# m4drat/wtf

Measured on AMD Instinct MI355X. Metric: execs/sec + emulated instr/s per node (tlv_server, HEVD) at 1/2/4/8 GPUs, higher is better.
Workload: dtype u64

## Files before the change

### wtf_amd/host/gpu_backend.cc

```cpp
#include "gpu_backend.h"
#include "module_instances.h"

#include <algorithm>
#include <chrono>
#include <cstdio>
#include <cstring>

#include "host_pool.h"

#include "blake3_lite.h"

namespace wtfgpu_host {

thread_local uint32_t GpuBackend_t::cur_ = 0;
thread_local uint64_t GpuBackend_t::servicing_bp_ = ~0ull;
thread_local uint64_t GpuBackend_t::servicing_sp_ = ~0ull;
thread_local bool GpuBackend_t::scouting_ = false;

namespace {
constexpr uint64_t kFeedRegion = 16384;
using Clock = std::chrono::steady_clock;
double ms_since(Clock::time_point t0) {
  return std::chrono::duration<double, std::milli>(Clock::now() - t0).count();
}

int gpr_index(Registers_t r) {
  switch (r) {
    case Registers_t::Rax: return WTFGPU_RAX;
    case Registers_t::Rbx: return WTFGPU_RBX;
    case Registers_t::Rcx: return WTFGPU_RCX;
    case Registers_t::Rdx: return WTFGPU_RDX;
    case Registers_t::Rsi: return WTFGPU_RSI;
    case Registers_t::Rdi: return WTFGPU_RDI;
    case Registers_t::Rsp: return WTFGPU_RSP;
    case Registers_t::Rbp: return WTFGPU_RBP;
    case Registers_t::R8: return WTFGPU_R8;
    case Registers_t::R9: return WTFGPU_R9;
    case Registers_t::R10: return WTFGPU_R10;
    case Registers_t::R11: return WTFGPU_R11;
    case Registers_t::R12: return WTFGPU_R12;
    case Registers_t::R13: return WTFGPU_R13;
    case Registers_t::R14: return WTFGPU_R14;
    case Registers_t::R15: return WTFGPU_R15;
    case Registers_t::Rip: return 16;
    case Registers_t::Rflags: return 17;
    default: return -1;
  }
}

}

GpuBackend_t::GpuBackend_t() = default;
GpuBackend_t::~GpuBackend_t() {
  for (Part &P : parts_)
    for (void *p : {(void *)P.pin, (void *)P.ex, (void *)P.nb, (void *)P.dc, (void *)P.sargs, (void *)P.cov_hdr})
      if (p) wtfgpu_host_free(ctx_, p);
  if (wpin_) wtfgpu_host_free(ctx_, wpin_);
  if (ctx_) wtfgpu_destroy(ctx_);
}

bool GpuBackend_t::LoadDump(const std::string &dump_path) { return dump_.Parse(dump_path); }

bool GpuBackend_t::Initialize(const Options_t &Opts, const CpuState_t &CpuState) {
  if (dump_.PageCount() == 0 && !Opts.DumpPath.empty() && !LoadDump(Opts.DumpPath.string())) {
    printf("Failed to parse the dump %s\n", Opts.DumpPath.string().c_str());
    return false;
  }
  if (wtfgpu_create(Opts.GpuDevice, &ctx_) != WTFGPU_OK) {
    printf("wtfgpu_create(%d) failed\n", Opts.GpuDevice);
    return false;
  }
  const auto pages = dump_.Pages();
  std::vector<uint64_t> gpfns(pages.size());
  std::vector<uint8_t> blob(pages.size() * Page::Size);
  for (size_t i = 0; i < pages.size(); i++) {
    gpfns[i] = pages[i].first;
    memcpy(blob.data() + i * Page::Size, pages[i].second, Page::Size);
  }
  if (wtfgpu_load_pool(ctx_, gpfns.data(), blob.data(), gpfns.size())) return false;
  nlanes_ = std::max<uint32_t>(Opts.GpuLanes, 1);
  overlay_pages_ = std::max<uint32_t>(Opts.GpuOverlayPages, 1);
  if (wtfgpu_alloc_lanes(ctx_, nlanes_, overlay_pages_, Opts.GpuCoverageSet)) return false;
  views_.clear();
  views_.resize(nlanes_);
  touched_.assign(nlanes_, 0);
  pf_.assign(nlanes_, PrepFeed{});
  arenas_.resize(HostPool::Get().Threads() + 1);
  if (Opts.Limit) SetLimit(Opts.Limit);
  if (Opts.Edges && wtfgpu_set_edges(ctx_, 1) != WTFGPU_OK) return false;
  if (!Restore(CpuState)) return false;
  return set_code_pages();
}

bool GpuBackend_t::Restore(const CpuState_t &CpuState) {
  initial_ = CpuState;
  initial_regs_ = RegsFromCpuState(CpuState);
  if (wtfgpu_set_initial_state(ctx_, &initial_regs_)) return false;
  if (wtfgpu_restore(ctx_, 0, nlanes_)) return false;
  for (uint32_t l = 0; l < nlanes_; l++) reset_view(l);
  cur_ = 0;
  return true;
}

void GpuBackend_t::reset_view(uint32_t lane) {
  LaneView &v = views_[lane];
  memcpy(v.gpr, initial_regs_.gpr, sizeof(initial_regs_.gpr));
  v.gpr[16] = initial_regs_.rip;
  v.gpr[17] = initial_regs_.rflags;
  v.regs_dirty = false;
  v.cr[0] = initial_regs_.cr2;
  v.cr[1] = initial_regs_.cr3;
  v.cr_known = 3;
  v.cr_dirty = 0;
  v.result.reset();
  v.handler_fault = false;
  v.seed = initial_.Seed;
  v.has_feed = false;
  v.feed.clear();
  v.dirty_known = true;
  v.dirty.clear();
  v.wlog.clear();
  v.wdata.clear();
  v.win_len = 0;
  drop_staged(v);
  touched_[lane] = 0;
}

void GpuBackend_t::Stop(const TestcaseResult_t &Res) { cur().result = Res; }

void GpuBackend_t::SetLimit(const uint64_t Limit) {
  limit_ = Limit;
  if (ctx_) wtfgpu_set_limit(ctx_, Limit);
}

uint64_t GpuBackend_t::GetReg(const Registers_t Reg) {
  const int i = gpr_index(Reg);
  if (i >= 0) return cur().gpr[i];
  if (Reg == Registers_t::Cr2 || Reg == Registers_t::Cr3) {
    const int k = Reg == Registers_t::Cr2 ? 0 : 1;
    LaneView &v = cur();
    if (!(v.cr_known & (1 << k))) {
      std::lock_guard<std::mutex> g(engine_mu_);
      if (wtfgpu_lane_get_cr(ctx_, cur_, k ? 3 : 2, &v.cr[k]) != WTFGPU_OK) std::abort();
      v.cr_known |= uint8_t(1 << k);
    }
    return v.cr[k];
  }
  return 0;
}

uint64_t GpuBackend_t::SetReg(const Registers_t Reg, const uint64_t Value) {
  const int i = gpr_index(Reg);
  if (i >= 0) {
    cur().gpr[i] = Value;
    cur().regs_dirty = true;
  } else if (Reg == Registers_t::Cr2 || Reg == Registers_t::Cr3) {
    const int k = Reg == Registers_t::Cr2 ? 0 : 1;
    cur().cr[k] = Value;
    cur().cr_known |= uint8_t(1 << k);
    cur().cr_dirty |= uint8_t(1 << k);
  }
  return Value;
}

uint64_t GpuBackend_t::Rdrand() { return wtf_rdrand(cur().seed); }

void GpuBackend_t::PrintRunStats() {
  PrintTestcaseRunStats(last_run_, aggregate_.size());
  printf("  Breakpoint services: %llu in %llu rounds\n", (unsigned long long)stats_.breakpoint_hits,
         (unsigned long long)stats_.rounds);
  printf("       Kernel time ms: %.2f\n", stats_.kernel_ms);
}

bool GpuBackend_t::SetBreakpoint(const Gva_t Gva, const BreakpointHandler_t Handler) {
  if (ModuleInstances *I = ModuleInstances::Registering()) {
    I->AddHandler(Gva.U64(), Handler);
    if (I->RegisteringIndex() > 0) return breakpoints_.count(Gva.U64()) != 0;
  }
  if (breakpoints_.count(Gva.U64())) {
    printf("/!\\ There is already a breakpoint at %#llx\n", (unsigned long long)Gva.U64());
    return false;
  }
  breakpoints_.emplace(Gva.U64(), Handler);
  std::vector<uint64_t> v;
  for (auto &kv : breakpoints_) v.push_back(kv.first);
  return wtfgpu_set_breakpoints(ctx_, v.data(), (uint32_t)v.size()) == WTFGPU_OK;
}

bool GpuBackend_t::SetBreakpoint(const Gva_t Gva, const BreakpointHandler_t Handler,
                                 const BreakpointAction_t &Action) {
  if (!SetBreakpoint(Gva, Handler)) return false;
  if (ModuleInstances::Registering() && ModuleInstances::Registering()->RegisteringIndex() > 0) return true;
  const char *Env = getenv("WTFGPU_DEVICE_BP_ACTIONS");
  if (Action.Kind == BreakpointAction_t::Kind_t::Host || (Env && Env[0] == '0')) return true;
  wtfgpu_bp_action_t A;
  memset(&A, 0, sizeof(A));
  A.gva = Gva.U64();
  if (Action.Kind == BreakpointAction_t::Kind_t::SimulateReturn) {
    A.kind = WTFGPU_BPACT_RETURN;
    A.value = Action.Return;
    if (Action.StringReg >= 0) {
      const int g = gpr_index((Registers_t)Action.StringReg);
      if (g < 0) return false;
      A.gprs[0] = (uint64_t)g + 1;
      A.gprs[1] = Action.StringMax;
    }
  } else if (Action.Kind == BreakpointAction_t::Kind_t::Feed) {
    A.kind = WTFGPU_BPACT_FEED;
    A.value = Action.Return;
    A.gprs[0] = (uint64_t)gpr_index((Registers_t)Action.Gprs[0]);
    A.gprs[1] = (uint64_t)gpr_index((Registers_t)Action.Gprs[1]);
    feed_action_ = true;
  } else if (Action.Kind == BreakpointAction_t::Kind_t::StopOk) {
    A.kind = WTFGPU_BPACT_STOP_OK;
  } else if (Action.Kind == BreakpointAction_t::Kind_t::Rdrand) {
    A.kind = WTFGPU_BPACT_RDRAND;
    A.gprs[0] = (uint64_t)gpr_index((Registers_t)Action.Gprs[0]);
  } else if (Action.Kind == BreakpointAction_t::Kind_t::StopWithArgs) {
    if (!Action.ArgsResult || Action.Return > 6) return false;
    A.kind = WTFGPU_BPACT_STOP_ARGS;
    A.value = Action.Return;
    args_results_[Gva.U64()] = Action.ArgsResult;
  } else {
    A.kind = WTFGPU_BPACT_SET_GPRS;
    memcpy(A.gprs, Action.Gprs, sizeof(A.gprs));
  }
  bp_actions_.push_back(A);
  return wtfgpu_set_breakpoint_actions(ctx_, bp_actions_.data(), (uint32_t)bp_actions_.size()) == WTFGPU_OK;
}

bool GpuBackend_t::SetFeed(const uint8_t *Data, const uint64_t Size) {
  if (!feed_action_ || Size > kFeedRegion) return false;
  LaneView &v = cur();
  v.has_feed = true;
  v.feed.assign(Data, Data + Size);
  return true;
}

bool GpuBackend_t::DeclareInsert(const InsertAction_t &Action) {
  if (ModuleInstances::Registering() && ModuleInstances::Registering()->RegisteringIndex() > 0) return insert_action_;
  const char *Env = getenv("WTFGPU_DEVICE_BP_ACTIONS");
  if (Env && Env[0] == '0') return false;
  const int h = gpr_index(Action.HeadReg), p = gpr_index(Action.PtrReg), l = gpr_index(Action.LenReg);
  if (h < 0 || p < 0 || l < 0 || Action.LenArg > 64) return false;
  const wtfgpu_insert_t I = {(uint32_t)h, (uint32_t)p, (uint32_t)l, Action.LenArg};
  if (wtfgpu_set_insert(ctx_, &I) != WTFGPU_OK) return false;
  insert_action_ = true;
  return true;
}

bool GpuBackend_t::SetInsert(const uint8_t *Data, const uint64_t Size) {
  if (!insert_action_ || Size + 4 > kFeedRegion) return false;
  LaneView &v = cur();
  v.has_feed = true;
  v.feed.resize(Size + 4);
  const uint32_t n = (uint32_t)Size;
  memcpy(v.feed.data(), &n, 4);
  if (Size) memcpy(v.feed.data() + 4, Data, Size);
  return true;
}

int GpuBackend_t::upload_feed(uint32_t n) {
  if (!(feed_action_ || insert_action_) || n == 0) return WTFGPU_OK;
  std::vector<uint64_t> off(n + 1);
  std::vector<uint8_t> has(n);
  uint64_t total = 0;
  for (uint32_t l = 0; l < n; l++) total += view(l).feed.size();
  std::vector<uint8_t> bytes;
  bytes.reserve(total);
  for (uint32_t l = 0; l < n; l++) {
    off[l] = bytes.size();
    has[l] = view(l).has_feed;
    bytes.insert(bytes.end(), view(l).feed.begin(), view(l).feed.end());
  }
  off[n] = bytes.size();
  return wtfgpu_set_feed(ctx_, 0, n, off.data(), has.data(), bytes.data(), bytes.size());
}

bool GpuBackend_t::DirtyGpa(const Gpa_t) { return true; }

namespace {
constexpr size_t kArenaBlock = 16u << 20;
const uint8_t kZeroPage[Page::Size] = {};
}

size_t GpuBackend_t::alloc_slots(size_t n, uint8_t **orig, uint8_t **data) const {
  const bool in_loop = HostPool::InLoop();
  std::shared_lock<std::shared_mutex> recycling(recycle_mu_);
  std::unique_lock<std::mutex> spare(spare_mu_, std::defer_lock);
  if (!in_loop) spare.lock();
  Arena &A = arenas_[in_loop ? HostPool::ThreadIndex() : arenas_.size() - 1];
  while (A.cur < A.blocks.size() && A.blocks[A.cur].cap - A.blocks[A.cur].used < n) A.cur++;
  if (A.cur == A.blocks.size()) {
    Block b;
    b.cap = std::max<size_t>(n, kArenaBlock / Page::Size);
    void *p = nullptr;
    int rc;
    {
      std::lock_guard<std::mutex> g(engine_mu_);
      rc = wtfgpu_host_alloc(ctx_, b.cap * Page::Size, &p);
    }
    if (rc != WTFGPU_OK) {
      printf("wtfgpu_host_alloc failed\n");
      std::abort();
    }
    b.orig = (uint8_t *)p;
    b.data.reset(new uint8_t[b.cap * Page::Size]);
    A.blocks.push_back(std::move(b));
  }
  Block &b = A.blocks[A.cur];
  *orig = b.orig + b.used * Page::Size;
  *data = b.data.get() + b.used * Page::Size;
  const size_t first = b.used;
  b.used += n;
  live_staged_ += n;
  return first;
}

void GpuBackend_t::release_slots(size_t n) const { live_staged_ -= n; }

bool GpuBackend_t::parallel_service(const ModuleSlots *slots) const {
  return slots && slots->ThreadSafe() && HostPool::Get().Threads() > 1;
}

uint8_t *GpuBackend_t::stage(uint32_t lane, uint64_t gpfn, const uint8_t *orig, uint8_t *data) const {
  LaneView &v = view(lane);
  v.pages.push_back(Staged{gpfn, data, orig});
  for (LaneView::Logged &w : v.wlog)
    if (w.len && (w.gpa >> 12) == gpfn) {
      memcpy(data + (w.gpa & 0xfff), v.wdata.data() + w.off, w.len);
      w.len = 0;
    }
  return data;
}

bool GpuBackend_t::PhysWriteDirect(const Gpa_t Gpa, const uint8_t *Buffer, const uint64_t Size) {
  const uint32_t lane = cur_;
  if (Staged *p = find_staged(lane, Gpa.U64() >> 12)) {
    memcpy(p->data + (Gpa.U64() & 0xfff), Buffer, Size);
    return true;
  }
  LaneView &v = view(lane);
  if (v.win_len && Gpa.U64() < v.win_gpa + v.win_len && Gpa.U64() + Size > v.win_gpa) {
    const uint64_t lo = std::max(Gpa.U64(), v.win_gpa), hi = std::min(Gpa.U64() + Size, v.win_gpa + v.win_len);
    memcpy(v.win + (lo - v.win_gpa), Buffer + (lo - Gpa.U64()), hi - lo);
  }
  if (!v.wlog.empty()) {
    LaneView::Logged &last = v.wlog.back();
    if (last.len && last.off + last.len == v.wdata.size() && last.gpa + last.len == Gpa.U64() &&
        ((last.gpa ^ Gpa.U64()) >> 12) == 0) {
      last.len += (uint32_t)Size;
      v.wdata.insert(v.wdata.end(), Buffer, Buffer + Size);
      return true;
    }
  }
  v.wlog.push_back(LaneView::Logged{Gpa.U64(), (uint32_t)Size, (uint32_t)v.wdata.size()});
  v.wdata.insert(v.wdata.end(), Buffer, Buffer + Size);
  return true;
}

bool GpuBackend_t::PhysReadDirect(const Gpa_t Gpa, uint8_t *Buffer, const uint64_t Size) const {
  const uint32_t lane = cur_;
  const uint64_t gpfn = Gpa.U64() >> 12;
  if (Staged *p = find_staged(lane, gpfn)) {
    memcpy(Buffer, p->data + (Gpa.U64() & 0xfff), Size);
    return true;
  }
  const LaneView &v = view(lane);
  if (v.win_len && Gpa.U64() >= v.win_gpa && Gpa.U64() + Size <= v.win_gpa + v.win_len) {
    memcpy(Buffer, v.win + (Gpa.U64() - v.win_gpa), Size);
    return true;
  }
  if (!v.dirty_known || in_overlay(v, gpfn)) return false;
  for (const LaneView::Logged &w : v.wlog)
    if (w.len && (w.gpa >> 12) == gpfn) return false;
  const uint8_t *p = dump_.GetPhysicalPage(gpfn << 12);
  memcpy(Buffer, (p ? p : kZeroPage) + (Gpa.U64() & 0xfff), Size);
  return true;
}

uint8_t *GpuBackend_t::stage_copy(uint32_t lane, uint64_t gpfn, const uint8_t *orig) const {
  uint8_t *o, *d;
  alloc_slots(1, &o, &d);
  memcpy(d, orig, Page::Size);
  return stage(lane, gpfn, orig, d);
}

void GpuBackend_t::drop_staged(LaneView &v) const {
  if (v.pages.empty()) return;
  live_staged_ -= v.pages.size();
  v.pages.clear();
  if (!HostPool::InLoop()) recycle_arenas();
}

void GpuBackend_t::recycle_arenas() const {
  if (live_staged_ != 0 || HostPool::InLoop()) return;
  std::unique_lock<std::shared_mutex> recycling(recycle_mu_);
  if (live_staged_ != 0) return;
  std::lock_guard<std::mutex> spare(spare_mu_);
  for (Arena &A : arenas_) {
    for (Block &b : A.blocks) b.used = 0;
    A.cur = 0;
  }
}

GpuBackend_t::Staged *GpuBackend_t::find_staged(uint32_t lane, uint64_t gpfn) const {
  for (Staged &p : view(lane).pages)
    if (p.gpfn == gpfn) return &p;
  return nullptr;
}

bool GpuBackend_t::in_overlay(const LaneView &v, uint64_t gpfn) const {
  return std::find(v.dirty.begin(), v.dirty.end(), (uint32_t)gpfn) != v.dirty.end();
}

uint8_t *GpuBackend_t::lane_page(uint32_t lane, uint64_t gpfn) const {
  if (Staged *p = find_staged(lane, gpfn)) return p->data;
  LaneView &v = view(lane);
  if (!v.dirty_known) {
    std::vector<uint32_t> buf(overlay_pages_ + 1);
    std::lock_guard<std::mutex> g(engine_mu_);
    wtfgpu_read_dirty_list(ctx_, &lane, 1, buf.data());
    v.dirty.assign(buf.begin() + 1, buf.begin() + 1 + std::min<uint32_t>(buf[0], overlay_pages_));
    v.dirty_known = true;
  }
  if (in_overlay(v, gpfn)) {
    const auto t0 = Clock::now();
    uint8_t *o, *d;
    alloc_slots(1, &o, &d);
    const uint64_t gpa = gpfn << 12;
    std::lock_guard<std::mutex> g(engine_mu_);
    wtfgpu_gather_pages(ctx_, &lane, &gpa, 1, o);
    memcpy(d, o, Page::Size);
    stats_.page_fetches++;
    stats_.fetch_ms += ms_since(t0);
    fetch_by_bp_[servicing_bp_]++;
    learn(gpfn);
    return stage(lane, gpfn, o, d);
  }
  if (scouting_) learn(gpfn);
  const uint8_t *p = dump_.GetPhysicalPage(gpfn << 12);
  return stage_copy(lane, gpfn, p ? p : kZeroPage);
}

void GpuBackend_t::learn(uint64_t gpfn) const {
  if (servicing_bp_ == ~0ull) return;
  if (gpfn == servicing_sp_) {
    bp_stack_.insert(servicing_bp_);
    return;
  }
  auto &l = bp_pages_[servicing_bp_];
  if (l.size() < 8 && std::find(l.begin(), l.end(), gpfn) == l.end()) l.push_back(gpfn);
}

const uint8_t *GpuBackend_t::lane_page_ro(uint32_t lane, uint64_t gpfn) const {
  if (Staged *p = find_staged(lane, gpfn)) return p->data;
  const LaneView &v = view(lane);
  if (!v.dirty_known || in_overlay(v, gpfn)) return lane_page(lane, gpfn);
  const uint8_t *p = dump_.GetPhysicalPage(gpfn << 12);
  return p ? p : kZeroPage;
}

namespace {
struct WalkMemo {
  uint64_t vpn = ~0ull, base = 0, mask = 0;
  uint64_t tables[4] = {};
  uint32_t ntables = 0;
};
thread_local WalkMemo t_walk_memo[64];
}

bool GpuBackend_t::VirtTranslate(const Gva_t Gva, Gpa_t &Gpa, const MemoryValidate_t) const {
  const uint64_t va = Gva.U64(), vpn = va >> 12;
  const LaneView &v = view(cur_);
  WalkMemo &m = t_walk_memo[vpn & 63];
  if (m.vpn == vpn && v.dirty_known && (!(v.cr_known & 2) || v.cr[1] == initial_.Cr3)) {
    bool clean = true;
    for (uint32_t k = 0; k < m.ntables && clean; k++)
      clean = !in_overlay(v, m.tables[k]) && !find_staged(cur_, m.tables[k]);
    if (clean) {
      Gpa = Gpa_t(m.base | (va & m.mask));
      return true;
    }
  }
  uint64_t table = initial_.Cr3 & 0x000ffffffffff000ull;
  WalkMemo w;
  bool from_dump = v.dirty_known;
  if ((v.cr_known & 2) && v.cr[1] != initial_.Cr3) {
    table = v.cr[1] & 0x000ffffffffff000ull;
    from_dump = false;
  }
  for (int level = 3; level >= 0; level--) {
    const uint64_t tf = table >> 12;
    w.tables[w.ntables++] = tf;
    from_dump = from_dump && !in_overlay(v, tf) && !find_staged(cur_, tf);
    const uint8_t *pg = lane_page_ro(cur_, tf);
    uint64_t e;
    memcpy(&e, pg + ((va >> (12 + 9 * level)) & 0x1ff) * 8, 8);
    if (!(e & 1)) return false;
    const uint64_t frame = e & 0x000ffffffffff000ull;
    if ((level == 2 || level == 1) && (e & 0x80)) {
      w.mask = level == 2 ? 0x3fffffffull : 0x1fffffull;
      w.base = frame & ~w.mask;
      break;
    }
    if (level == 0) {
      w.mask = 0xfff;
      w.base = frame;
    }
    table = frame;
  }
  Gpa = Gpa_t(w.base | (va & w.mask));
  if (from_dump) {
    w.vpn = vpn;
    m = w;
  }
  return true;
}

uint8_t *GpuBackend_t::PhysTranslate(const Gpa_t Gpa) const {
  return lane_page(cur_, Gpa.U64() >> 12) + (Gpa.U64() & 0xfff);
}

bool GpuBackend_t::PageFaultsMemoryIfNeeded(const Gva_t Gva, const uint64_t Size) {
  for (uint64_t a = Gva.U64() & ~0xfffull; a < Gva.U64() + Size; a += Page::Size) {
    Gpa_t G;
    if (!VirtTranslate(Gva_t(a), G, MemoryValidate_t::ValidateRead)) {
      cur().inject = a;
      return true;
    }
  }
  return false;
}

const std::unordered_set<Gva_t> &GpuBackend_t::LastNewCoverage() const { return last_new_coverage_; }

bool GpuBackend_t::RevokeLastNewCoverage() {
  for (const Gva_t &g : last_new_coverage_) aggregate_.erase(g.U64());
  last_new_coverage_.clear();
  return true;
}

int GpuBackend_t::flush_lanes(const std::vector<uint32_t> &lanes) {
  const auto tp = Clock::now();
  const size_t nl = lanes.size();
  const bool par = nl >= 1024;
  std::vector<uint64_t> rcnt(nl + 1, 0), pcnt(nl + 1, 0), roff(nl + 1, 0), boff(nl + 1, 0);
  std::atomic<bool> any_cr{false};
  HostPool::Get().For(nl, 256, [&](size_t i) {
    const LaneView &v = view(lanes[i]);
    rcnt[i + 1] = v.regs_dirty ? 1 : 0;
    pcnt[i + 1] = v.pages.size();
    uint64_t r = 0, b = 0;
    for (const LaneView::Logged &w : v.wlog)
      if (w.len) {
        r++;
        b += w.len;
      }
    roff[i + 1] = r;
    boff[i + 1] = b;
    if (v.cr_dirty) any_cr.store(true, std::memory_order_relaxed);
  }, par);
  for (size_t i = 0; i < nl; i++) {
    rcnt[i + 1] += rcnt[i];
    pcnt[i + 1] += pcnt[i];
    roff[i + 1] += roff[i];
    boff[i + 1] += boff[i];
  }
  if (any_cr)
    for (uint32_t l : lanes) {
      LaneView &v = view(l);
      for (int k = 0; k < 2; k++)
        if (v.cr_dirty & (1 << k)) {
          std::lock_guard<std::mutex> g(engine_mu_);
          if (wtfgpu_lane_set_cr(ctx_, l, k ? 3 : 2, v.cr[k]) != WTFGPU_OK) return WTFGPU_ERR_INVALID;
        }
      v.cr_dirty = 0;
    }
  std::vector<uint32_t> rl(rcnt[nl]);
  std::vector<uint64_t> regs(rcnt[nl] * 18);
  struct Cand {
    uint32_t lane;
    const Staged *p;
    uint32_t lo, hi;
  };
  std::vector<Cand> cand(pcnt[nl]);
  HostPool::Get().For(nl, 256, [&](size_t i) {
    const uint32_t l = lanes[i];
    LaneView &v = view(l);
    if (v.regs_dirty) {
      rl[rcnt[i]] = l;
      memcpy(&regs[rcnt[i] * 18], v.gpr, 18 * 8);
      v.regs_dirty = false;
    }
    uint64_t k = pcnt[i];
    for (const Staged &p : v.pages) cand[k++] = Cand{l, &p, 0, 0};
  }, par);
  HostPool::Get().For(cand.size(), 64, [&](size_t i) {
    const uint8_t *d = cand[i].p->data, *o = cand[i].p->orig;
    if (!memcmp(d, o, Page::Size)) return;
    size_t lo = 0, hi = Page::Size;
    while (lo + 8 <= hi && !memcmp(d + lo, o + lo, 8)) lo += 8;
    while (lo < hi && d[lo] == o[lo]) lo++;
    while (hi >= lo + 8 && !memcmp(d + hi - 8, o + hi - 8, 8)) hi -= 8;
    while (hi > lo && d[hi - 1] == o[hi - 1]) hi--;
    cand[i].lo = (uint32_t)lo;
    cand[i].hi = (uint32_t)hi;
  });
  uint64_t cbytes = 0, crecs = 0;
  for (const Cand &c : cand)
    if (c.lo != c.hi) {
      crecs++;
      cbytes += c.hi - c.lo;
    }
  std::vector<wtfgpu_write_t> writes(roff[nl] + crecs);
  const uint64_t total = boff[nl] + cbytes;
  if (total > wpin_cap_) {
    if (wpin_) wtfgpu_host_free(ctx_, wpin_);
    wpin_ = nullptr;
    wpin_cap_ = std::max<uint64_t>(total * 2, 1 << 20);
    void *p = nullptr;
    if (wtfgpu_host_alloc(ctx_, wpin_cap_, &p)) return WTFGPU_ERR_OOM;
    wpin_ = (uint8_t *)p;
  }
  HostPool::Get().For(nl, 256, [&](size_t i) {
    const uint32_t l = lanes[i];
    LaneView &v = view(l);
    uint64_t r = roff[i], b = boff[i];
    for (const LaneView::Logged &w : v.wlog) {
      if (!w.len) continue;
      writes[r++] = wtfgpu_write_t{l, w.len, w.gpa, b};
      memcpy(wpin_ + b, v.wdata.data() + w.off, w.len);
      b += w.len;
      v.dirty_known = false;
    }
    v.wlog.clear();
    v.wdata.clear();
  }, par);
  {
    uint64_t r = roff[nl], b = boff[nl];
    for (const Cand &c : cand) {
      if (c.lo == c.hi) continue;
      wtfgpu_write_t w{};
      w.lane = c.lane;
      w.len = c.hi - c.lo;
      w.gva = (c.p->gpfn << 12) | c.lo;
      w.data_off = b;
      memcpy(wpin_ + b, c.p->data + c.lo, w.len);
      b += w.len;
      writes[r++] = w;
      view(c.lane).dirty_known = false;
    }
  }
  stats_.staged_pages += cand.size();
  if (!cand.empty())
    for (uint32_t l : lanes) drop_staged(view(l));
  int rc = WTFGPU_OK;
  const auto tr = Clock::now();
  stats_.up_prep_ms += std::chrono::duration<double, std::milli>(tr - tp).count();
  if (!rl.empty()) rc = wtfgpu_write_gprs_list(ctx_, rl.data(), (uint32_t)rl.size(), regs.data());
  const auto ta = Clock::now();
  stats_.up_regs_ms += std::chrono::duration<double, std::milli>(ta - tr).count();
  if (!rc && !writes.empty())
    rc = wtfgpu_apply_phys_writes(ctx_, writes.data(), (uint32_t)writes.size(), wpin_, total, nullptr);
  stats_.up_apply_ms += ms_since(ta);
  return rc;
}

bool GpuBackend_t::classify(const std::vector<uint32_t> &pending, uint32_t first, const wtfgpu_exit_t *ex,
                            std::vector<uint8_t> &done, std::vector<LaneResult> *out, std::vector<uint32_t> &hits,
                            const uint64_t *stop_args) {
  std::vector<uint8_t> hit(pending.size(), 0);
  HostPool::Get().For(pending.size(), 1024, [&](size_t pi) {
    const uint32_t l = pending[pi];
    if (done[l - first]) return;
    const wtfgpu_exit_t &e = ex[l - first];
    LaneView &v = views_[l];
    const auto mark = [&]() -> LaneView & {
      touched_[l] = 1;
      return v;
    };
    switch (e.status) {
      case WTFGPU_EXIT_BREAKPOINT: hit[pi] = 1; return;
      case WTFGPU_RUNNING: return;
      case WTFGPU_EXIT_TIMEOUT: mark().result = Timedout_t(); break;
      case WTFGPU_EXIT_INT3:
      case WTFGPU_EXIT_HLT: mark().result = Crash_t(); break;
      case WTFGPU_EXIT_CR3: mark().result = Cr3Change_t(); break;
      case WTFGPU_EXIT_FAULT: mark().result = FaultToResult(e.vector, e.error, e.rip, e.addr, e.opcode); break;
      case WTFGPU_EXIT_STOPPED: break;
      case WTFGPU_EXIT_STOP_OK:
        if (touched_[l]) v.result = Ok_t();
        break;
      case WTFGPU_EXIT_STOP_ARGS: hit[pi] = 2; return;
      case WTFGPU_EXIT_FEED_FAULT: mark().handler_fault = true; break;
      default:
        if (out) (*out)[l].error = true;
        if (!v.result) mark().result = Crash_t();
        if (e.status == WTFGPU_EXIT_UNIMPLEMENTED) {
          stats_.err_unimpl++;
          stats_.unimpl_ops.add(e.opcode);
          stats_.last_unimpl_op = e.opcode;
          stats_.last_unimpl_rip = e.rip;
        } else if (e.status == WTFGPU_EXIT_OVERLAY_FULL) {
          stats_.err_overlay++;
        } else {
          stats_.err_other++;
        }
        break;
    }
    done[l - first] = 1;
  }, pending.size() >= 2048);
  std::vector<uint32_t> named;
  for (size_t pi = 0; pi < pending.size(); pi++) {
    if (hit[pi] == 1) hits.push_back(pending[pi]);
    if (hit[pi] == 2) named.push_back(pending[pi]);
  }
  if (named.empty()) return true;
  std::vector<uint64_t> args(named.size() * 6);
  bool ok = true;
  if (stop_args) {
    HostPool::Get().For(named.size(), 2048, [&](size_t k) {
      memcpy(&args[k * 6], stop_args + (uint64_t)(named[k] - first) * 6, 48);
    }, named.size() >= 8192);
  } else {
    ok = wtfgpu_read_stop_args(ctx_, named.data(), (uint32_t)named.size(), args.data()) == WTFGPU_OK;
  }
  std::atomic<uint64_t> bad{0};
  HostPool::Get().For(named.size(), 512, [&](size_t k) {
    const uint32_t l = named[k];
    LaneView &v = view(l);
    const auto it = args_results_.find(ex[l - first].rip);
    if (ok && it != args_results_.end()) {
      v.result = it->second(&args[k * 6]);
    } else {
      if (out) (*out)[l].error = true;
      if (!v.result) v.result = Crash_t();
      bad++;
    }
    done[l - first] = 1;
  }, named.size() >= 2048);
  stats_.err_other += bad;
  return true;
}

bool GpuBackend_t::fill_results(const std::vector<uint32_t> &lanes, uint32_t first,
                                const wtfgpu_exit_t *ex, const std::vector<uint8_t> &done,
                                std::vector<LaneResult> *out, std::vector<uint32_t> *finished) {
  const auto tg = Clock::now();
  std::vector<uint32_t> fin;
  for (uint32_t l : lanes)
    if (done[l - first]) fin.push_back(l);
  if (finished) finished->insert(finished->end(), fin.begin(), fin.end());
  if (!out) return true;
  std::vector<uint64_t> regs;
  uint32_t lo = 0, hi = 0;
  std::vector<uint64_t> nb;
  std::vector<uint32_t> dc, ec;
  if (want_gprs_) {
    regs.resize(fin.size() * 18);
    if (!fin.empty() && wtfgpu_read_gprs_list(ctx_, fin.data(), (uint32_t)fin.size(), regs.data())) return false;
    if (!fin.empty()) {
      lo = *std::min_element(fin.begin(), fin.end());
      hi = *std::max_element(fin.begin(), fin.end()) + 1;
      nb.resize(hi - lo);
      dc.resize(hi - lo);
      ec.resize(2 * (hi - lo));
      if (wtfgpu_read_bytes(ctx_, lo, hi - lo, nb.data()) || wtfgpu_read_dirty_counts(ctx_, lo, hi - lo, dc.data()) ||
          wtfgpu_read_edge_counts(ctx_, lo, hi - lo, ec.data()))
        return false;
    }
  }
  HostPool::Get().For(fin.size(), 1024, [&](size_t i) {
    LaneResult &r = (*out)[fin[i]];
    const LaneView &v = views_[fin[i]];
    const bool t = touched_[fin[i]] != 0;
    r.result = t && v.result ? std::move(*v.result) : TestcaseResult_t(Ok_t());
    if (t && v.handler_fault) {
      r.result = Crash_t();
      r.error = true;
      r.handler_fault = true;
      stats_.err_handler++;
    }
    if (want_gprs_) {
      memcpy(r.gprs, &regs[i * 18], 18 * 8);
      r.rip = r.gprs[16];
      const uint32_t k = fin[i] - lo;
      r.bytes = nb[k];
      r.dirty = std::min(dc[k], overlay_pages_);
      r.edges = ec[2 * k];
      r.edges_new = ec[2 * k + 1];
    } else {
      r.rip = ex[fin[i] - first].rip;
    }
    r.icount = ex[fin[i] - first].icount;
    r.exit_status = ex[fin[i] - first].status;
  }, fin.size() >= 2048);
  stats_.regs_ms += ms_since(tg);
  return true;
}

bool GpuBackend_t::stop_prestopped(const std::vector<uint32_t> &lanes) {
  std::vector<uint8_t> has(lanes.size());
  HostPool::Get().For(lanes.size(), 1024, [&](size_t i) { has[i] = touched_[lanes[i]] && views_[lanes[i]].result.has_value(); },
                      lanes.size() >= 4096);
  std::vector<uint32_t> pre;
  for (size_t i = 0; i < lanes.size(); i++)
    if (has[i]) pre.push_back(lanes[i]);
  return pre.empty() || wtfgpu_stop(ctx_, pre.data(), (uint32_t)pre.size(), WTFGPU_EXIT_STOPPED) == WTFGPU_OK;
}

bool GpuBackend_t::run_lanes(const std::vector<uint32_t> &lanes, std::vector<LaneResult> *out, ModuleSlots *slots,
                             bool per_lane_state) {
  if (lanes.empty()) return true;
  const uint32_t first = lanes.front() & ~63u, count = lanes.back() + 1 - first;
  std::vector<wtfgpu_exit_t> ex(count);
  std::vector<uint8_t> done(count, 0);
  std::vector<uint32_t> pending = lanes;
  if (!stop_prestopped(lanes)) return false;
  for (;;) {
    wtfgpu_run_stats_t rs{};
    const auto tk = Clock::now();
    if (wtfgpu_run(ctx_, first, count, ~0ull, &rs)) return false;
    const auto te = Clock::now();
    stats_.run_ms += std::chrono::duration<double, std::milli>(te - tk).count();
    account_run(rs);
    if (wtfgpu_read_exits(ctx_, first, count, ex.data())) return false;
    std::vector<uint32_t> hits;
    if (!classify(pending, first, ex.data(), done, out, hits)) return false;
    stats_.exits_ms += ms_since(te);
    if (hits.empty()) break;
    if (!service_hits(hits, first, done, slots, per_lane_state)) return false;
    pending.clear();
    for (uint32_t l : hits)
      if (!done[l - first]) pending.push_back(l);
  }
  return fill_results(lanes, first, ex.data(), done, out, nullptr);
}

void GpuBackend_t::account_run(const wtfgpu_run_stats_t &rs) {
  stats_.kernel_launches += rs.kernel_launches;
  stats_.kernel_ms += rs.kernel_ms;
  stats_.retired += rs.lane_retired;
  stats_.group_steps += rs.group_steps;
  stats_.rounds++;
}

bool GpuBackend_t::service_hits(const std::vector<uint32_t> &hits, uint32_t first, std::vector<uint8_t> &done,
                                ModuleSlots *slots, bool per_lane_state) {
  const auto t0 = Clock::now();
  {
    std::vector<uint64_t> regs(hits.size() * 18);
    if (wtfgpu_read_gprs_list(ctx_, hits.data(), (uint32_t)hits.size(), regs.data())) return false;
    std::vector<uint64_t> seeds(hits.size());
    if (wtfgpu_lane_seeds(ctx_, hits.data(), (uint32_t)hits.size(), seeds.data(), 0)) return false;
    const uint32_t stride = overlay_pages_ + 1;
    std::vector<uint32_t> dl(hits.size() * stride);
    if (wtfgpu_read_dirty_list(ctx_, hits.data(), (uint32_t)hits.size(), dl.data())) return false;
    const auto t1 = Clock::now();
    stats_.bulk_ms += std::chrono::duration<double, std::milli>(t1 - t0).count();
    std::vector<uint64_t> sp_gpfn(hits.size(), ~0ull), sp_gpa(hits.size(), ~0ull);
    HostPool::Get().For(hits.size(), 256, [&](size_t i) {
      LaneView &v = view(hits[i]);
      memcpy(v.gpr, &regs[i * 18], 18 * 8);
      v.seed = seeds[i];
      v.regs_dirty = false;
      v.cr_known = 0;
      v.win_len = 0;
      drop_staged(v);
      const uint32_t cnt = std::min(dl[i * stride], overlay_pages_);
      v.dirty.assign(dl.begin() + i * stride + 1, dl.begin() + i * stride + 1 + cnt);
      v.dirty_known = true;
      const uint64_t rip = v.gpr[16];
      if (!bp_seen_.count(rip) || bp_stack_.count(rip)) {
        cur_ = hits[i];
        Gpa_t sp;
        if (VirtTranslate(Gva_t(v.gpr[WTFGPU_RSP]), sp, MemoryValidate_t::ValidateRead)) {
          sp_gpa[i] = sp.U64();
          sp_gpfn[i] = sp.U64() >> 12;
        }
      }
    });
    recycle_arenas();
    std::vector<uint8_t> action(hits.size());
    auto service = [&](size_t h) {
      const uint32_t l = hits[h];
      LaneView &v = view(l);
      cur_ = l;
      const uint64_t rip0 = v.gpr[16];
      servicing_sp_ = sp_gpfn[h];
      BreakpointHandler_t handler = nullptr;
      if (slots && slots->Instances()) {
        handler = slots->Instances()->HandlerOf(l, rip0);
      } else {
        const auto it = breakpoints_.find(rip0);
        if (it != breakpoints_.end()) handler = it->second;
      }
      if (per_lane_state && slots) slots->SwapIn(l);
      servicing_bp_ = rip0;
      v.inject = ~0ull;
      try {
        if (handler) handler(this);
      } catch (const HandlerFault_t &) {
        v.handler_fault = true;
        v.result = Crash_t();
      }
      servicing_bp_ = ~0ull;
      if (per_lane_state && slots) slots->SwapOut(l);
      action[h] = v.result ? 0 : (v.gpr[16] == rip0 ? 2 : 1);
    };
    Backend_t *saved = g_Backend;
    g_Backend = this;
    std::vector<uint8_t> scouted(hits.size(), 0);
    for (size_t i = 0; i < hits.size(); i++) {
      if (!bp_seen_.insert(view(hits[i]).gpr[16]).second) continue;
      scouting_ = true;
      service(i);
      scouting_ = false;
      scouted[i] = 1;
    }
    std::vector<uint32_t> pf_lanes, win_lanes;
    std::vector<uint64_t> pf_gpas, win_gpas;
    std::vector<uint8_t> use_win(hits.size(), 0);
    HostPool::Get().For(hits.size(), 256, [&](size_t i) {
      if (scouted[i] || sp_gpfn[i] == ~0ull) return;
      const LaneView &v = view(hits[i]);
      if (bp_stack_.count(v.gpr[16]) && in_overlay(v, sp_gpfn[i]))
        use_win[i] = (sp_gpa[i] & 0xfff) + LaneView::kWin <= Page::Size ? 1 : 2;
    });
    for (size_t i = 0; i < hits.size(); i++) {
      if (scouted[i]) continue;
      const LaneView &v = view(hits[i]);
      auto want = [&](uint64_t gpfn) {
        if (!in_overlay(v, gpfn)) return;
        for (size_t k = pf_gpas.size(); k-- > 0 && pf_lanes[k] == hits[i];)
          if (pf_gpas[k] == gpfn << 12) return;
        pf_lanes.push_back(hits[i]);
        pf_gpas.push_back(gpfn << 12);
      };
      if (use_win[i] == 1) {
        win_lanes.push_back(hits[i]);
        win_gpas.push_back(sp_gpa[i]);
      } else if (use_win[i] == 2) {
        want(sp_gpfn[i]);
      }
      if (!bp_pages_.empty()) {
        auto lp = bp_pages_.find(v.gpr[16]);
        if (lp != bp_pages_.end())
          for (uint64_t g : lp->second) want(g);
      }
    }
    if (!win_lanes.empty()) {
      const size_t nw = win_lanes.size();
      std::vector<uint8_t> buf(nw * LaneView::kWin);
      if (wtfgpu_gather_bytes(ctx_, win_lanes.data(), win_gpas.data(), (uint32_t)nw, LaneView::kWin, buf.data()))
        return false;
      HostPool::Get().For(nw, 256, [&](size_t i) {
        LaneView &v = view(win_lanes[i]);
        v.win_gpa = win_gpas[i];
        v.win_len = LaneView::kWin;
        memcpy(v.win, buf.data() + i * LaneView::kWin, LaneView::kWin);
      });
      stats_.stack_windows += nw;
    }
    if (!pf_lanes.empty()) {
      const size_t np = pf_lanes.size();
      uint8_t *o, *d;
      alloc_slots(np, &o, &d);
      if (wtfgpu_gather_pages(ctx_, pf_lanes.data(), pf_gpas.data(), (uint32_t)np, o)) {
        release_slots(np);
        return false;
      }
      HostPool::Get().For(np, 256, [&](size_t i) { memcpy(d + i * Page::Size, o + i * Page::Size, Page::Size); });
      for (size_t i = 0; i < np; i++)
        stage(pf_lanes[i], pf_gpas[i] >> 12, o + i * Page::Size, d + i * Page::Size);
      stats_.prefetched_pages += np;
    }
    const auto t2 = Clock::now();
    stats_.prefetch_ms += std::chrono::duration<double, std::milli>(t2 - t1).count();
    if (per_lane_state && parallel_service(slots)) {
      HostPool::Get().For(hits.size(), 64, [&](size_t h) {
        g_Backend = this;
        if (!scouted[h]) service(h);
      });
    } else {
      for (size_t h = 0; h < hits.size(); h++)
        if (!scouted[h]) service(h);
    }
    g_Backend = saved;
    stats_.breakpoint_hits += hits.size();
    const auto t3 = Clock::now();
    stats_.handler_ms += std::chrono::duration<double, std::milli>(t3 - t2).count();
    if (flush_lanes(hits)) return false;
    for (size_t i = 0; i < hits.size(); i++) seeds[i] = view(hits[i]).seed;
    if (wtfgpu_lane_seeds(ctx_, hits.data(), (uint32_t)hits.size(), seeds.data(), 1)) return false;
    {
      std::vector<uint32_t> il;
      std::vector<uint64_t> ia;
      std::vector<size_t> ih;
      for (size_t h = 0; h < hits.size(); h++)
        if (action[h] != 0 && view(hits[h]).inject != ~0ull) {
          il.push_back(hits[h]);
          ia.push_back(view(hits[h]).inject);
          ih.push_back(h);
        }
      if (!il.empty()) {
        std::vector<int32_t> ok(il.size());
        if (wtfgpu_inject_fault(ctx_, il.data(), (uint32_t)il.size(), WTFGPU_VEC_PF, ErrorWrite | ErrorUser, ia.data(),
                                ok.data()))
          return false;
        for (size_t k = 0; k < il.size(); k++) {
          if (ok[k]) {
            action[ih[k]] = 1;
          } else {
            view(il[k]).result = Crash_t();
            action[ih[k]] = 0;
          }
        }
      }
    }
    std::vector<uint32_t> resume, stop;
    std::vector<uint8_t> skip;
    for (size_t h = 0; h < hits.size(); h++) {
      if (action[h] == 0) {
        stop.push_back(hits[h]);
        done[hits[h] - first] = 1;
      } else {
        resume.push_back(hits[h]);
        skip.push_back(action[h] == 2);
      }
    }
    if (!stop.empty() && wtfgpu_stop(ctx_, stop.data(), (uint32_t)stop.size(), WTFGPU_EXIT_STOPPED)) return false;
    if (!resume.empty() && wtfgpu_resume(ctx_, resume.data(), (uint32_t)resume.size(), skip.data())) return false;
    stats_.flush_ms += ms_since(t3);
    stats_.service_ms += ms_since(t0);
  }
  return true;
}

void GpuBackend_t::finish_coverage(uint32_t n, std::vector<LaneResult> *out, std::vector<uint32_t> *timedout) {
  uint64_t total = 0;
  uint32_t ovf = 0, dl = 0;
  uint64_t dr = 0;
  wtfgpu_read_coverage(ctx_, 0, n, &dl, &dr, 0, &total, &ovf);
  std::vector<uint32_t> lanes(total);
  std::vector<uint64_t> rips(total);
  if (total) wtfgpu_read_coverage(ctx_, 0, n, lanes.data(), rips.data(), total, &total, &ovf);
  std::vector<std::vector<uint64_t>> per(n);
  for (uint64_t i = 0; i < total; i++) per[lanes[i]].push_back(rips[i]);
  std::vector<uint64_t> fresh;
  last_new_coverage_.clear();
  for (uint32_t l = 0; l < n; l++) {
    std::sort(per[l].begin(), per[l].end());
    per[l].erase(std::unique(per[l].begin(), per[l].end()), per[l].end());
    if (full_coverage_) {
      if (out) (*out)[l].new_coverage = per[l];
      if (n == 1)
        for (uint64_t rip : per[l]) last_new_coverage_.insert(Gva_t(rip));
      continue;
    }
    const bool revoke = timedout && std::find(timedout->begin(), timedout->end(), l) != timedout->end();
    for (uint64_t rip : per[l]) {
      if (aggregate_.count(rip)) continue;
      if (out) (*out)[l].new_coverage.push_back(rip);
      if (revoke) continue;
      aggregate_.insert(rip);
      fresh.push_back(rip);
      if (n == 1) last_new_coverage_.insert(Gva_t(rip));
    }
  }
  if (full_coverage_) {
    wtfgpu_reset_coverage(ctx_);
    return;
  }
  commit_fresh(fresh);
}

std::optional<TestcaseResult_t> GpuBackend_t::Run(const uint8_t *, const uint64_t) {
  const auto t0 = Clock::now();
  cur_ = 0;
  if (flush_lanes({0}) || upload_feed(1)) return std::nullopt;
  std::vector<LaneResult> out(1);
  if (!run_lanes({0}, &out, nullptr, false)) return std::nullopt;
  LaneView &v = view(0);
  if (wtfgpu_read_gprs_list(ctx_, &cur_, 1, v.gpr)) return std::nullopt;
  v.regs_dirty = false;
  v.cr_known = 0;
  last_icount_ = out[0].icount;
  last_error_ = out[0].error;
  {
    uint64_t nbytes = 0;
    uint32_t dcount = 0, ecount[2] = {0, 0};
    wtfgpu_read_bytes(ctx_, 0, 1, &nbytes);
    wtfgpu_read_dirty_counts(ctx_, 0, 1, &dcount);
    wtfgpu_read_edge_counts(ctx_, 0, 1, ecount);
    last_run_ = out[0];
    last_run_.bytes = nbytes;
    last_run_.dirty = std::min(dcount, overlay_pages_);
    last_run_.edges = ecount[0];
    last_run_.edges_new = ecount[1];
  }
  finish_coverage(1, nullptr, nullptr);
  stats_.total_ms += ms_since(t0);
  cur_ = 0;
  return out[0].result;
}

bool GpuBackend_t::LaneTrace(uint32_t Lane, std::vector<uint64_t> &Rips, bool &Truncated) {
  uint64_t N = 0;
  Rips.clear();
  if (wtfgpu_read_trace(ctx_, Lane, nullptr, 0, &N) != WTFGPU_OK) return false;
  Truncated = N > trace_cap_;
  Rips.resize(std::min<uint64_t>(N, trace_cap_));
  return wtfgpu_read_trace(ctx_, Lane, Rips.data(), Rips.size(), &N) == WTFGPU_OK;
}

bool GpuBackend_t::LaneTenet(uint32_t Lane, std::vector<uint8_t> &Bytes, bool &Truncated) {
  uint64_t N = 0;
  Bytes.clear();
  if (wtfgpu_read_tenet(ctx_, Lane, nullptr, 0, &N) != WTFGPU_OK) return false;
  Truncated = N > tenet_cap_;
  Bytes.resize(std::min<uint64_t>(N, tenet_cap_));
  return wtfgpu_read_tenet(ctx_, Lane, Bytes.data(), Bytes.size(), &N) == WTFGPU_OK;
}

bool GpuBackend_t::RunBatch(const Target_t &Target, const std::vector<std::pair<const uint8_t *, size_t>> &Testcases,
                            std::vector<LaneResult> &Out, ModuleSlots *Slots) {
  const auto t0 = Clock::now();
  const uint32_t n = (uint32_t)Testcases.size();
  if (n == 0 || n > nlanes_) return false;
  Out.assign(n, LaneResult{});
  if (wtfgpu_restore(ctx_, 0, n)) return false;
  for (uint32_t l = 0; l < n; l++) reset_view(l);
  const auto tm = Clock::now();
  stats_.restore_ms += std::chrono::duration<double, std::milli>(tm - t0).count();
  std::vector<uint32_t> lanes(n);
  for (uint32_t l = 0; l < n; l++) lanes[l] = l;
  std::vector<uint8_t> insert_ok;
  insert_lanes(Target, lanes, Testcases, Slots, insert_ok);
  for (uint32_t l = 0; l < n; l++)
    if (!insert_ok[l]) view(l).result = Crash_t("insert-testcase-failed");
  const auto tu = Clock::now();
  stats_.module_ms += std::chrono::duration<double, std::milli>(tu - tm).count();
  if (flush_lanes(lanes) || upload_feed(n)) return false;
  stats_.upload_ms += ms_since(tu);
  stats_.insert_ms += ms_since(t0);
  if (!run_lanes(lanes, &Out, Slots, Slots != nullptr)) return false;
  {
    std::vector<uint64_t> nb(n);
    std::vector<uint32_t> dc(n);
    if (wtfgpu_read_bytes(ctx_, 0, n, nb.data()) == WTFGPU_OK &&
        wtfgpu_read_dirty_counts(ctx_, 0, n, dc.data()) == WTFGPU_OK)
      for (uint32_t l = 0; l < n; l++) stats_.alg_bytes += nb[l] + 2ull * 4096 * dc[l] + Testcases[l].second;
  }
  const auto tc = Clock::now();
  std::vector<uint32_t> timedout;
  for (uint32_t l = 0; l < n; l++)
    if (std::holds_alternative<Timedout_t>(Out[l].result)) timedout.push_back(l);
  finish_coverage(n, &Out, &timedout);
  const auto tr = Clock::now();
  stats_.coverage_ms += std::chrono::duration<double, std::milli>(tr - tc).count();
  target_restore(Target, lanes, Slots);
  stats_.target_restore_ms += ms_since(tr);
  stats_.total_ms += ms_since(t0);
  stats_.batches++;
  stats_.testcases += n;
  return true;
}

void GpuBackend_t::insert_lanes(const Target_t &Target, const std::vector<uint32_t> &lanes,
                                const std::vector<std::pair<const uint8_t *, size_t>> &tcs, ModuleSlots *Slots,
                                std::vector<uint8_t> &ok) {
  Backend_t *saved = g_Backend;
  ok.assign(lanes.size(), 1);
  auto insert = [&](size_t i) {
    const uint32_t l = lanes[i];
    cur_ = l;
    if (Slots) {
      Slots->ResetLane(l);
      Slots->SwapIn(l);
    }
    const Target_t &T = Slots && Slots->Instances() ? Slots->Instances()->TargetOf(l) : Target;
    try {
      ok[i] = T.InsertTestcase(tcs[i].first, tcs[i].second);
    } catch (const HandlerFault_t &) {
      view(l).handler_fault = true;
      ok[i] = 0;
    }
    if (Slots) Slots->SwapOut(l);
  };
  if (parallel_service(Slots)) {
    HostPool::Get().For(lanes.size(), 256, [&](size_t i) {
      g_Backend = this;
      insert(i);
    });
  } else {
    g_Backend = this;
    for (size_t i = 0; i < lanes.size(); i++) insert(i);
  }
  g_Backend = saved;
}

void GpuBackend_t::target_restore(const Target_t &Target, const std::vector<uint32_t> &lanes, ModuleSlots *Slots) {
  Backend_t *saved = g_Backend;
  auto restore = [&](uint32_t l) {
    cur_ = l;
    if (Slots) Slots->SwapIn(l);
    (Slots && Slots->Instances() ? Slots->Instances()->TargetOf(l) : Target).Restore();
    if (Slots) Slots->SwapOut(l);
  };
  if (parallel_service(Slots)) {
    HostPool::Get().For(lanes.size(), 256, [&](size_t i) {
      g_Backend = this;
      restore(lanes[i]);
    });
  } else {
    g_Backend = this;
    for (uint32_t l : lanes) restore(l);
  }
  g_Backend = saved;
  cur_ = 0;
}

void GpuBackend_t::collect_coverage(const std::vector<uint32_t> &lanes, std::vector<LaneResult> &res,
                                    const uint64_t *pf_hdr) {
  const auto t0 = Clock::now();
  uint64_t total = 0;
  uint32_t ovf = 0;
  constexpr uint64_t kPrefetchCap = 1ull << 22;
  bool pf = pf_hdr && pf_hdr[0] <= kPrefetchCap;
  if (pf) {
    total = pf_hdr[0];
    ovf = (uint32_t)pf_hdr[1] & 1;
    if (cov_lanes_.size() < total) {
      cov_lanes_.resize(total);
      cov_rips_.resize(total);
    }
    pf = wtfgpu_prefetched_coverage(ctx_, cov_lanes_.data(), cov_rips_.data(), total) == WTFGPU_OK &&
         wtfgpu_clear_coverage_lanes(ctx_, lanes.data(), (uint32_t)lanes.size()) == WTFGPU_OK;
    if (pf && total) {
      if (cov_want_.size() < nlanes_) cov_want_.assign(nlanes_, 0);
      for (uint32_t l : lanes) cov_want_[l] = 1;
      uint64_t k = 0;
      for (uint64_t i = 0; i < total; i++)
        if (cov_want_[cov_lanes_[i]]) {
          cov_lanes_[k] = cov_lanes_[i];
          cov_rips_[k++] = cov_rips_[i];
        }
      for (uint32_t l : lanes) cov_want_[l] = 0;
      total = k;
    }
  }
  if (!pf) {
    total = 0;
    ovf = 0;
    if (cov_lanes_.size() < (1u << 16)) {
      cov_lanes_.resize(1u << 16);
      cov_rips_.resize(1u << 16);
    }
    wtfgpu_collect_coverage_lanes(ctx_, lanes.data(), (uint32_t)lanes.size(), cov_lanes_.data(), cov_rips_.data(),
                                  cov_lanes_.size(), &total, &ovf);
    if (total > cov_lanes_.size()) {
      cov_lanes_.resize(total);
      cov_rips_.resize(total);
      wtfgpu_collect_coverage_lanes(ctx_, lanes.data(), (uint32_t)lanes.size(), cov_lanes_.data(), cov_rips_.data(),
                                    cov_lanes_.size(), &total, &ovf);
    }
  }
  const std::vector<uint32_t> &cl = cov_lanes_;
  const std::vector<uint64_t> &cr = cov_rips_;
  const auto t1 = Clock::now();
  stats_.covlog_ms += std::chrono::duration<double, std::milli>(t1 - t0).count();
  stats_.cov_entries += total;
  if (ovf && !cov_ovf_warned_) {
    cov_ovf_warned_ = true;
    fprintf(stderr, "wtfgpu: a lane's new-coverage set filled up (rips lost); raise the set size\n");
  }
  std::vector<std::pair<uint32_t, uint64_t>> &ent = cov_sorted_;
  ent.resize(total);
  for (uint64_t i = 0; i < total; i++) ent[i] = {cl[i], cr[i]};
  std::sort(ent.begin(), ent.end());
  ent.erase(std::unique(ent.begin(), ent.end()), ent.end());
  if (getenv("WTFGPU_COVLOG_TOP")) {
    for (uint64_t i = 0; i < total; i++) covlog_count_[cr[i]]++;
    if (++covlog_calls_ % 64 == 0) {
      std::vector<std::pair<uint64_t, uint64_t>> v(covlog_count_.begin(), covlog_count_.end());
      std::sort(v.begin(), v.end(), [](auto &a, auto &b) { return a.second > b.second; });
      fprintf(stderr, "covlog top:");
      for (size_t i = 0; i < v.size() && i < 24; i++)
        fprintf(stderr, " %llx:%llu%s", (unsigned long long)v[i].first, (unsigned long long)v[i].second,
                aggregate_.count(v[i].first) ? "*" : "");
      fprintf(stderr, " (%zu values)\n", v.size());
    }
  }
  std::vector<uint64_t> fresh;
  last_new_coverage_.clear();
  auto attribute = [&](uint32_t l, size_t at) {
    const bool revoke = std::holds_alternative<Timedout_t>(res[l].result);
    for (; at < ent.size() && ent[at].first == l; at++) {
      const uint64_t rip = ent[at].second;
      if (full_coverage_) {
        res[l].new_coverage.push_back(rip);
        continue;
      }
      if (aggregate_.count(rip)) continue;
      res[l].new_coverage.push_back(rip);
      if (revoke) continue;
      aggregate_.insert(rip);
      fresh.push_back(rip);
    }
    return at;
  };
  if (std::is_sorted(lanes.begin(), lanes.end())) {
    for (size_t at = 0; at < ent.size();) at = attribute(ent[at].first, at);
  } else {
    for (uint32_t l : lanes) {
      const auto it = std::lower_bound(ent.begin(), ent.end(), std::pair<uint32_t, uint64_t>{l, 0});
      if (it != ent.end() && it->first == l) attribute(l, (size_t)(it - ent.begin()));
    }
  }
  commit_fresh(fresh);
  stats_.attrib_ms += ms_since(t1);
}

uint32_t GpuBackend_t::FreeLanes() const {
  if (busy_.empty()) return parts_n() > 1 ? nlanes_ / 2 : nlanes_;
  const Part &P = parts_[next_part_];
  if (P.launched) return P.hi - P.lo;
  return (uint32_t)P.free.size();
}

uint32_t GpuBackend_t::parts_n() const {
  if (!parts_.empty()) return (uint32_t)parts_.size();
  const char *e = getenv("WTFGPU_STREAM_PARTS");
  const uint32_t want = e ? (uint32_t)atoi(e) : 2;
  return (want >= 2 && nlanes_ >= 256 && nlanes_ % 128 == 0) ? 2 : 1;
}

bool GpuBackend_t::StreamStep(const Target_t &Target, const std::vector<StreamTestcase_t> &In, uint64_t Slice,
                              std::vector<StreamResult_t> &Out, ModuleSlots *Slots, size_t *Taken) {
  const auto t0 = Clock::now();
  if (Taken) *Taken = 0;
  if (busy_.empty()) {
    busy_.assign(nlanes_, 0);
    tag_.assign(nlanes_, 0);
    tc_bytes_.assign(nlanes_, 0);
    lres_.assign(nlanes_, LaneResult{});
    lres_stale_.assign(nlanes_, 0);
    const uint32_t n = parts_n();
    parts_.assign(n, Part{});
    for (uint32_t p = 0; p < n; p++) {
      Part &Q = parts_[p];
      Q.lo = (uint32_t)((uint64_t)nlanes_ * p / n);
      Q.hi = (uint32_t)((uint64_t)nlanes_ * (p + 1) / n);
      Q.free.resize(Q.hi - Q.lo);
      for (uint32_t l = Q.lo; l < Q.hi; l++) Q.free[l - Q.lo] = l;
    }
    std::vector<uint32_t> all(nlanes_);
    for (uint32_t l = 0; l < nlanes_; l++) all[l] = l;
    if (wtfgpu_stop(ctx_, all.data(), nlanes_, WTFGPU_EXIT_IDLE)) return false;
  }
  const bool pipelined = parts_.size() > 1;
  const uint32_t pi = next_part_;
  next_part_ = (next_part_ + 1) % (uint32_t)parts_.size();
  Part &P = parts_[pi];
  if (pipelined && wtfgpu_select_queue(ctx_, pi)) return false;
  if (pipelined && P.launched && !harvest_part(P, Target, Out, Slots)) return false;
  const auto ti = Clock::now();
  stats_.harvest_ms += std::chrono::duration<double, std::milli>(ti - t0).count();
  std::vector<uint32_t> fresh;
  std::vector<std::pair<const uint8_t *, size_t>> tcs;
  fresh.reserve(std::min<size_t>(In.size(), P.hi - P.lo));
  tcs.reserve(fresh.capacity());
  {
    const size_t take = std::min(In.size(), P.free.size());
    fresh.assign(P.free.begin(), P.free.begin() + (std::ptrdiff_t)take);
    P.free.erase(P.free.begin(), P.free.begin() + (std::ptrdiff_t)take);
    tcs.resize(take);
    for (size_t i = 0; i < take; i++) tcs[i] = {In[i].data, In[i].size};
  }
  if (Taken) *Taken = fresh.size();
  stats_.fresh_ms += ms_since(ti);
  if (!fresh.empty()) {
    if (wtfgpu_restore_lanes(ctx_, fresh.data(), (uint32_t)fresh.size())) return false;
    stats_.restore_dev_ms += ms_since(ti);
    std::vector<uint8_t> prepared(fresh.size(), 0);
    HostPool::Get().For(fresh.size(), 256, [&](size_t i) {
      const uint32_t l = fresh[i];
      if (touched_[l]) reset_view(l);
      pf_[l] = PrepFeed{};
      busy_[l] = 1;
      tag_[l] = In[i].tag;
      tc_bytes_[l] = In[i].size;
      lres_stale_[l] = 1;
      const StreamTestcase_t &T = In[i];
      switch (T.prep) {
        case PreparedInsert_t::Call: return;
        case PreparedInsert_t::Failed: view(l).result = Crash_t("insert-testcase-failed"); break;
        case PreparedInsert_t::Nothing: break;
        case PreparedInsert_t::Feed:
          if (!feed_action_ || T.prep_size > kFeedRegion) return;
          pf_[l] = PrepFeed{T.prep_data, (uint32_t)T.prep_size, 1, 0};
          break;
        case PreparedInsert_t::Insert:
          if (!insert_action_ || T.size + 4 > kFeedRegion) return;
          pf_[l] = PrepFeed{T.data, (uint32_t)T.size, 1, 1};
          break;
      }
      if (Slots) Slots->ResetLane(l);
      prepared[i] = 1;
    });
    recycle_arenas();
    const auto tm = Clock::now();
    stats_.restore_ms += std::chrono::duration<double, std::milli>(tm - ti).count();
    std::vector<uint32_t> call;
    std::vector<std::pair<const uint8_t *, size_t>> call_tcs;
    for (size_t i = 0; i < fresh.size(); i++)
      if (!prepared[i]) {
        call.push_back(fresh[i]);
        call_tcs.push_back(tcs[i]);
      }
    stats_.prepared += fresh.size() - call.size();
    if (!call.empty()) {
      std::vector<uint8_t> ok;
      insert_lanes(Target, call, call_tcs, Slots, ok);
      for (size_t i = 0; i < call.size(); i++)
        if (!ok[i]) view(call[i]).result = Crash_t("insert-testcase-failed");
    }
    const auto tu = Clock::now();
    stats_.module_ms += std::chrono::duration<double, std::milli>(tu - tm).count();
    if (flush_lanes(call)) return false;
    if (feed_action_ || insert_action_) {
      const auto tf = Clock::now();
      const size_t n = fresh.size();
      std::vector<uint64_t> off(n + 1, 0);
      std::vector<uint8_t> has(n);
      HostPool::Get().For(n, 1024, [&](size_t i) {
        const uint32_t l = fresh[i];
        const PrepFeed &f = pf_[l];
        const bool t = !f.has && touched_[l];
        off[i + 1] = f.has ? f.len + (f.ins ? 4 : 0) : t ? views_[l].feed.size() : 0;
        has[i] = f.has || (t && views_[l].has_feed);
      });
      for (size_t i = 0; i < n; i++) off[i + 1] += off[i];
      if (off[n] > P.pin_cap) {
        if (P.pin) wtfgpu_host_free(ctx_, P.pin);
        P.pin = nullptr;
        P.pin_cap = std::max<uint64_t>(off[n] * 2, 1 << 20);
        void *p = nullptr;
        if (wtfgpu_host_alloc(ctx_, P.pin_cap, &p)) return false;
        P.pin = (uint8_t *)p;
      }
      HostPool::Get().For(n, 256, [&](size_t i) {
        const uint32_t l = fresh[i];
        const PrepFeed &f = pf_[l];
        uint8_t *o = P.pin + off[i];
        if (f.has) {
          if (f.ins) {
            memcpy(o, &f.len, 4);
            o += 4;
          }
          if (f.len) memcpy(o, f.p, f.len);
        } else if (touched_[l] && !views_[l].feed.empty()) {
          memcpy(o, views_[l].feed.data(), views_[l].feed.size());
        }
      });
      if (wtfgpu_set_feed_lanes(ctx_, fresh.data(), (uint32_t)n, off.data(), has.data(), P.pin, off[n]))
        return false;
      stats_.up_feed_ms += ms_since(tf);
    }
    if (!stop_prestopped(fresh)) return false;
    stats_.upload_ms += ms_since(tu);
    stats_.testcases += fresh.size();
  }
  stats_.insert_ms += ms_since(ti);
  const auto to = Clock::now();
  if (!fresh.empty()) {
    std::vector<uint32_t> occ(P.occ.size() + fresh.size());
    std::merge(P.occ.begin(), P.occ.end(), fresh.begin(), fresh.end(), occ.begin());
    P.occ.swap(occ);
  }
  stats_.occ_ms += ms_since(to);
  if (!P.occ.empty()) {
    const auto tk = Clock::now();
    if (wtfgpu_run_async(ctx_, P.lo, P.hi - P.lo, Slice ? Slice : 4096)) return false;
    P.pf = pipelined && prefetch_part(P);
    stats_.run_ms += ms_since(tk);
    P.launched = true;
    if (!pipelined && !harvest_part(P, Target, Out, Slots)) return false;
  }
  stats_.total_ms += ms_since(t0);
  return true;
}

bool GpuBackend_t::prefetch_part(Part &P) {
  const uint32_t count = P.hi - P.lo;
  auto grow = [&](auto *&p, uint64_t bytes) {
    if (p) return true;
    void *q = nullptr;
    if (wtfgpu_host_alloc(ctx_, bytes, &q)) return false;
    p = (std::remove_reference_t<decltype(p)>)q;
    return true;
  };
  if (P.ex_cap < count) {
    if (P.ex) wtfgpu_host_free(ctx_, P.ex);
    P.ex = nullptr;
    P.ex_cap = 0;
    if (!grow(P.ex, (uint64_t)count * sizeof(wtfgpu_exit_t))) return false;
    P.ex_cap = count;
  }
  const bool args = !args_results_.empty();
  if (!grow(P.nb, (uint64_t)count * 8) || !grow(P.dc, (uint64_t)count * 4) || !grow(P.cov_hdr, 16) ||
      (args && !grow(P.sargs, (uint64_t)count * 48)))
    return false;
  if (wtfgpu_prefetch_results(ctx_, P.lo, count, P.ex, P.nb, P.dc, args ? P.sargs : nullptr) != WTFGPU_OK)
    return false;
  P.pf_cov = !full_coverage_ && wtfgpu_prefetch_coverage(ctx_, P.lo, count, P.cov_hdr) == WTFGPU_OK;
  return true;
}

bool GpuBackend_t::harvest_part(Part &P, const Target_t &Target, std::vector<StreamResult_t> &Out,
                                ModuleSlots *Slots) {
  const auto tw = Clock::now();
  wtfgpu_run_stats_t rs{};
  if (wtfgpu_run_wait(ctx_, &rs)) return false;
  const auto te = Clock::now();
  stats_.run_ms += std::chrono::duration<double, std::milli>(te - tw).count();
  account_run(rs);
  P.launched = false;
  const uint32_t first = P.lo, count = P.hi - P.lo;
  HostPool::Get().For(P.occ.size(), 1024, [&](size_t i) {
    const uint32_t l = P.occ[i];
    if (!lres_stale_[l]) return;
    lres_stale_[l] = 0;
    LaneResult &r = lres_[l];
    r.result = Ok_t();
    r.error = false;
    r.handler_fault = false;
    r.exit_status = 0;
    r.icount = 0;
    r.rip = 0;
    r.new_coverage.clear();
  }, P.occ.size() >= 8192);
  const bool pf = P.pf;
  P.pf = false;
  if (!pf) {
    if (P.ex_cap < count) {
      if (P.ex) wtfgpu_host_free(ctx_, P.ex);
      P.ex = nullptr;
      P.ex_cap = 0;
      void *p = nullptr;
      if (wtfgpu_host_alloc(ctx_, (uint64_t)count * sizeof(wtfgpu_exit_t), &p)) return false;
      P.ex = (wtfgpu_exit_t *)p;
      P.ex_cap = count;
    }
    if (wtfgpu_read_exits(ctx_, first, count, P.ex)) return false;
  }
  std::vector<uint8_t> done(count, 0);
  std::vector<uint32_t> hits;
  if (!classify(P.occ, first, P.ex, done, &lres_, hits, pf ? P.sargs : nullptr)) return false;
  stats_.exits_ms += ms_since(te);
  if (!hits.empty() && !service_hits(hits, first, done, Slots, Slots != nullptr)) return false;
  std::vector<uint32_t> finished;
  if (!fill_results(P.occ, first, P.ex, done, &lres_, &finished)) return false;
  if (finished.empty()) return true;
  const auto tc = Clock::now();
  if (pf) {
    uint64_t b = 0;
    for (uint32_t l : finished) b += P.nb[l - first] + 2ull * 4096 * P.dc[l - first] + tc_bytes_[l];
    stats_.alg_bytes += b;
  } else {
    uint32_t lo = finished.front() & ~63u, hi = finished.back() + 1;
    std::vector<uint64_t> nb(hi - lo);
    std::vector<uint32_t> dc(hi - lo);
    if (wtfgpu_read_bytes(ctx_, lo, hi - lo, nb.data()) == WTFGPU_OK &&
        wtfgpu_read_dirty_counts(ctx_, lo, hi - lo, dc.data()) == WTFGPU_OK)
      for (uint32_t l : finished) stats_.alg_bytes += nb[l - lo] + 2ull * 4096 * dc[l - lo] + tc_bytes_[l];
  }
  stats_.bytes_ms += ms_since(tc);
  collect_coverage(finished, lres_, pf && P.pf_cov ? P.cov_hdr : nullptr);
  const auto tr = Clock::now();
  stats_.coverage_ms += std::chrono::duration<double, std::milli>(tr - tc).count();
  target_restore(Target, finished, Slots);
  stats_.target_restore_ms += ms_since(tr);
  const auto tout = Clock::now();
  const size_t base = Out.size();
  Out.resize(base + finished.size());
  for (size_t i = 0; i < finished.size(); i++) {
    const uint32_t l = finished[i];
    Out[base + i] = StreamResult_t{tag_[l], &lres_[l]};
    busy_[l] = 0;
  }
  {
    std::vector<uint32_t> occ(P.occ.size()), fr(P.free.size() + finished.size());
    occ.resize(std::set_difference(P.occ.begin(), P.occ.end(), finished.begin(), finished.end(), occ.begin()) -
               occ.begin());
    std::merge(P.free.begin(), P.free.end(), finished.begin(), finished.end(), fr.begin());
    P.occ.swap(occ);
    P.free.swap(fr);
  }
  stats_.out_ms += ms_since(tout);
  stats_.batches++;
  return true;
}

void GpuBackend_t::ResetCoverage() {
  aggregate_.clear();
  last_new_coverage_.clear();
  wtfgpu_reset_coverage(ctx_);
}

std::string GpuBackend_t::StatsJson() const {
  char b[2048];
  snprintf(b, sizeof(b),
           "{\"kind\":\"gpu\",\"group_steps\":%llu,\"rounds\":%llu,\"breakpoint_hits\":%llu,\"kernel_launches\":%llu,"
           "\"kernel_ms\":%.3f,\"service_ms\":%.3f,\"total_ms\":%.3f,\"page_fetches\":%llu,"
           "\"prefetched_pages\":%llu,\"stack_windows\":%llu,\"staged_pages\":%llu,\"bulk_ms\":%.3f,\"prefetch_ms\":%.3f,"
           "\"handler_ms\":%.3f,\"fetch_ms\":%.3f,\"flush_ms\":%.3f,\"insert_ms\":%.3f,\"coverage_ms\":%.3f,"
           "\"target_restore_ms\":%.3f,\"alg_bytes\":%llu,\"restore_ms\":%.3f,\"module_ms\":%.3f,"
           "\"upload_ms\":%.3f,\"bytes_ms\":%.3f,\"covlog_ms\":%.3f,\"attrib_ms\":%.3f,\"cov_entries\":%llu,"
           "\"run_ms\":%.3f,\"exits_ms\":%.3f,\"regs_ms\":%.3f,\"err_unimpl\":%llu,\"err_overlay\":%llu,"
           "\"err_other\":%llu,\"err_handler\":%llu,\"last_unimpl_op\":%llu,\"last_unimpl_rip\":%llu}",
           (unsigned long long)stats_.group_steps, (unsigned long long)stats_.rounds,
           (unsigned long long)stats_.breakpoint_hits, (unsigned long long)stats_.kernel_launches, stats_.kernel_ms,
           stats_.service_ms, stats_.total_ms, (unsigned long long)stats_.page_fetches,
           (unsigned long long)stats_.prefetched_pages, (unsigned long long)stats_.stack_windows,
           (unsigned long long)stats_.staged_pages, stats_.bulk_ms, stats_.prefetch_ms, stats_.handler_ms,
           stats_.fetch_ms, stats_.flush_ms, stats_.insert_ms, stats_.coverage_ms, stats_.target_restore_ms,
           (unsigned long long)stats_.alg_bytes, stats_.restore_ms, stats_.module_ms, stats_.upload_ms,
           stats_.bytes_ms, stats_.covlog_ms, stats_.attrib_ms, (unsigned long long)stats_.cov_entries,
           stats_.run_ms, stats_.exits_ms, stats_.regs_ms, (unsigned long long)stats_.err_unimpl.load(),
           (unsigned long long)stats_.err_overlay.load(), (unsigned long long)stats_.err_other.load(),
           (unsigned long long)stats_.err_handler.load(), (unsigned long long)stats_.last_unimpl_op.load(), (unsigned long long)stats_.last_unimpl_rip.load());
  std::string r(b);
  r.pop_back();
  snprintf(b, sizeof(b), ",\"up_prep_ms\":%.3f,\"up_regs_ms\":%.3f,\"up_apply_ms\":%.3f,\"up_feed_ms\":%.3f,"
           "\"restore_dev_ms\":%.3f,\"out_ms\":%.3f,\"fresh_ms\":%.3f,\"occ_ms\":%.3f,\"harvest_ms\":%.3f,"
           "\"prepared\":%llu",
           stats_.up_prep_ms, stats_.up_regs_ms, stats_.up_apply_ms, stats_.up_feed_ms, stats_.restore_dev_ms,
           stats_.out_ms, stats_.fresh_ms, stats_.occ_ms, stats_.harvest_ms, (unsigned long long)stats_.prepared);
  r += b;
  r += ",\"unimpl_ops\":" + stats_.unimpl_ops.json();
  r += ",\"unimpl_raw\":" + stats_.unimpl_ops.raw_json();
  b[0] = 0;
  r += b;
  r += ",\"fetch_by_bp\":{";
  bool first = true;
  for (const auto &[bp, n] : fetch_by_bp_) {
    char e[64];
    snprintf(e, sizeof(e), "%s\"%#llx\":%llu", first ? "" : ",", (unsigned long long)bp, (unsigned long long)n);
    r += e;
    first = false;
  }
  return r + "}}";
}

bool GpuBackend_t::set_code_pages() {
  const std::vector<uint64_t> vpns = ExecutablePages(dump_, initial_.Cr3);
  code_vpns_.clear();
  code_vpns_.insert(vpns.begin(), vpns.end());
  if (vpns.empty()) return true;
  return wtfgpu_set_code_pages(ctx_, vpns.data(), (uint32_t)vpns.size()) == WTFGPU_OK;
}

bool GpuBackend_t::CoverageMap(uint8_t **Map, uint64_t *Bytes, bool *Device) {
  void *p = nullptr;
  if (wtfgpu_coverage_device_map(ctx_, &p, Bytes) != WTFGPU_OK) return false;
  *Map = (uint8_t *)p;
  *Device = true;
  return true;
}

size_t GpuBackend_t::AbsorbCoverageMap() {
  uint64_t n = 0;
  if (wtfgpu_coverage_absorb(ctx_, nullptr, 0, &n) != WTFGPU_OK || n == 0) return 0;
  std::vector<uint64_t> rips(n);
  if (wtfgpu_coverage_absorb(ctx_, rips.data(), n, &n) != WTFGPU_OK) return 0;
  size_t added = 0;
  for (uint64_t i = 0; i < n && i < rips.size(); i++) added += aggregate_.insert(rips[i]).second;
  return added;
}

void GpuBackend_t::commit_fresh(const std::vector<uint64_t> &fresh) {
  if (fresh.empty()) return;
  for (uint64_t v : fresh)
    if (!code_vpns_.count(v >> 12)) extra_new_.push_back(v);
  wtfgpu_commit_coverage(ctx_, fresh.data(), fresh.size());
}

void GpuBackend_t::TakeNewExtra(std::vector<uint64_t> &Out) {
  Out.swap(extra_new_);
  extra_new_.clear();
}

size_t GpuBackend_t::AbsorbExtra(const std::vector<uint64_t> &All) {
  std::vector<uint64_t> add;
  for (uint64_t v : All)
    if (aggregate_.insert(v).second) add.push_back(v);
  if (!add.empty()) wtfgpu_commit_coverage(ctx_, add.data(), add.size());
  return add.size();
}

}
```

### wtf_amd/host/gpu_backend.h

```cpp
#pragma once
#include "unimpl_hist.h"
#include <atomic>
#include <memory>
#include <mutex>
#include <shared_mutex>
#include <string>
#include <unordered_map>
#include <vector>

#include "../../include/wtfgpu.h"
#include "kdmp.h"
#include "module_slots.h"
#include "runner.h"
#include "wtf_api.h"

namespace wtfgpu_host {

struct BatchStats {
  uint64_t rounds = 0, breakpoint_hits = 0, kernel_launches = 0, retired = 0, group_steps = 0;
  uint64_t page_fetches = 0, prefetched_pages = 0, batches = 0, testcases = 0, staged_pages = 0, stack_windows = 0;
  uint64_t prepared = 0;
  double kernel_ms = 0, service_ms = 0, total_ms = 0;
  double bulk_ms = 0, prefetch_ms = 0, handler_ms = 0, fetch_ms = 0, flush_ms = 0;
  double insert_ms = 0, coverage_ms = 0, target_restore_ms = 0;
  uint64_t alg_bytes = 0;
  double restore_ms = 0, module_ms = 0, upload_ms = 0;
  double up_prep_ms = 0, up_regs_ms = 0, up_apply_ms = 0, up_feed_ms = 0, restore_dev_ms = 0;
  double out_ms = 0, fresh_ms = 0, occ_ms = 0, harvest_ms = 0;
  double bytes_ms = 0, covlog_ms = 0, attrib_ms = 0;
  uint64_t cov_entries = 0;
  double run_ms = 0, exits_ms = 0, regs_ms = 0;
  std::atomic<uint64_t> err_unimpl{0}, err_overlay{0}, err_other{0}, err_handler{0};
  UnimplHist unimpl_ops;
  std::atomic<uint64_t> last_unimpl_op{0}, last_unimpl_rip{0};
};

class GpuBackend_t final : public Backend_t, public Executor_t {
 public:
  GpuBackend_t();
  ~GpuBackend_t() override;

  bool LoadDump(const std::string &dump_path);

  bool Initialize(const Options_t &Opts, const CpuState_t &CpuState) override;
  std::optional<TestcaseResult_t> Run(const uint8_t *Buffer, const uint64_t BufferSize) override;
  bool Restore(const CpuState_t &CpuState) override;
  void Stop(const TestcaseResult_t &Res) override;
  void SetLimit(const uint64_t Limit) override;
  uint64_t GetReg(const Registers_t Reg) override;
  uint64_t SetReg(const Registers_t Reg, const uint64_t Value) override;
  uint64_t Rdrand() override;
  void PrintRunStats() override;
  bool SetBreakpoint(const Gva_t Gva, const BreakpointHandler_t Handler) override;
  bool SetBreakpoint(const Gva_t Gva, const BreakpointHandler_t Handler, const BreakpointAction_t &Action) override;
  bool DirtyGpa(const Gpa_t Gpa) override;
  bool VirtTranslate(const Gva_t Gva, Gpa_t &Gpa, const MemoryValidate_t Validate) const override;
  uint8_t *PhysTranslate(const Gpa_t Gpa) const override;
  bool PageFaultsMemoryIfNeeded(const Gva_t Gva, const uint64_t Size) override;
  bool PhysWriteDirect(const Gpa_t Gpa, const uint8_t *Buffer, const uint64_t Size) override;
  bool PhysReadDirect(const Gpa_t Gpa, uint8_t *Buffer, const uint64_t Size) const override;
  bool SetFeed(const uint8_t *Data, const uint64_t Size) override;
  bool DeclareInsert(const InsertAction_t &Action) override;
  bool SetInsert(const uint8_t *Data, const uint64_t Size) override;
  const std::unordered_set<Gva_t> &LastNewCoverage() const override;
  bool RevokeLastNewCoverage() override;
  using Backend_t::SetBreakpoint;

  bool RunBatch(const Target_t &Target, const std::vector<std::pair<const uint8_t *, size_t>> &Testcases,
                std::vector<LaneResult> &Out, ModuleSlots *Slots) override;
  Backend_t *AsBackend() override { return this; }
  bool CanStream() const override { return true; }
  bool TakesPrepared() const override { return feed_action_ || insert_action_; }
  uint32_t FreeLanes() const override;
  bool StreamStep(const Target_t &Target, const std::vector<StreamTestcase_t> &In, uint64_t Slice,
                  std::vector<StreamResult_t> &Out, ModuleSlots *Slots, size_t *Taken) override;
  void ResetCoverage() override;
  void SetFullCoverage(bool On) override { full_coverage_ = On; }
  void SetWantRegisters(bool On) override { want_gprs_ = On; }
  uint64_t LastIcount() const override { return last_icount_; }
  bool LastError() const override { return last_error_; }
  bool LastHandlerFault() const override { return last_run_.handler_fault; }
  void LastRunStats(LaneResult &L) const override {
    L.bytes = last_run_.bytes;
    L.dirty = last_run_.dirty;
    L.edges = last_run_.edges;
    L.edges_new = last_run_.edges_new;
  }
  size_t CoverageSize() const override { return aggregate_.size(); }
  void TakeNewExtra(std::vector<uint64_t> &Out) override;
  size_t AbsorbExtra(const std::vector<uint64_t> &All) override;
  std::string StatsJson() const override;
  bool CoverageMap(uint8_t **Map, uint64_t *Bytes, bool *Device) override;
  size_t AbsorbCoverageMap() override;
  size_t MergeCoverageMap(const uint8_t *Merged, uint64_t Bytes, bool Device) override {
    if (!Device || wtfgpu_coverage_merge_in(ctx_, Merged, Bytes) != WTFGPU_OK) return 0;
    return AbsorbCoverageMap();
  }
  bool EnableTrace(uint32_t PerLane) override {
    trace_cap_ = PerLane;
    return ctx_ && wtfgpu_set_trace(ctx_, PerLane) == WTFGPU_OK;
  }
  bool LaneTrace(uint32_t Lane, std::vector<uint64_t> &Rips, bool &Truncated) override;
  bool EnableTenet(uint64_t BytesPerLane) override {
    tenet_cap_ = BytesPerLane;
    return ctx_ && wtfgpu_set_tenet(ctx_, BytesPerLane) == WTFGPU_OK;
  }
  bool LaneTenet(uint32_t Lane, std::vector<uint8_t> &Bytes, bool &Truncated) override;
  const BatchStats &Stats() const { return stats_; }
  uint32_t Lanes() const override { return nlanes_; }
  wtfgpu_ctx *Engine() const { return ctx_; }
  const std::unordered_set<uint64_t> &AggregateCoverage() const { return aggregate_; }

 private:
  struct Staged {
    uint64_t gpfn;
    uint8_t *data;
    const uint8_t *orig;
  };
  struct LaneView {
    uint64_t gpr[18] = {};
    bool regs_dirty = false;
    uint64_t cr[2] = {};
    uint8_t cr_known = 0, cr_dirty = 0;
    std::optional<TestcaseResult_t> result;
    bool handler_fault = false;
    uint64_t seed = 0;
    uint64_t inject = ~0ull;
    bool has_feed = false;
    std::vector<uint8_t> feed;
    bool dirty_known = false;
    std::vector<uint32_t> dirty;
    std::vector<Staged> pages;
    struct Logged {
      uint64_t gpa;
      uint32_t len, off;
    };
    std::vector<Logged> wlog;
    std::vector<uint8_t> wdata;
    static constexpr uint32_t kWin = 128;
    uint64_t win_gpa = 0;
    uint32_t win_len = 0;
    uint8_t win[kWin];
  };

  LaneView &view(uint32_t lane) const {
    touched_[lane] = 1;
    return views_[lane];
  }
  LaneView &cur() const { return view(cur_); }
  void reset_view(uint32_t lane);
  uint8_t *lane_page(uint32_t lane, uint64_t gpfn) const;
  const uint8_t *lane_page_ro(uint32_t lane, uint64_t gpfn) const;
  Staged *find_staged(uint32_t lane, uint64_t gpfn) const;
  size_t alloc_slots(size_t n, uint8_t **orig, uint8_t **data) const;
  uint8_t *stage(uint32_t lane, uint64_t gpfn, const uint8_t *orig, uint8_t *data) const;
  uint8_t *stage_copy(uint32_t lane, uint64_t gpfn, const uint8_t *orig) const;
  void drop_staged(LaneView &v) const;
  bool in_overlay(const LaneView &v, uint64_t gpfn) const;
  int flush_lanes(const std::vector<uint32_t> &lanes);
  bool run_lanes(const std::vector<uint32_t> &lanes, std::vector<LaneResult> *out, ModuleSlots *slots,
                 bool per_lane_state);
  bool classify(const std::vector<uint32_t> &pending, uint32_t first, const wtfgpu_exit_t *ex,
                std::vector<uint8_t> &done, std::vector<LaneResult> *out, std::vector<uint32_t> &hits,
                const uint64_t *stop_args = nullptr);
  bool fill_results(const std::vector<uint32_t> &lanes, uint32_t first, const wtfgpu_exit_t *ex,
                    const std::vector<uint8_t> &done, std::vector<LaneResult> *out, std::vector<uint32_t> *finished);
  bool stop_prestopped(const std::vector<uint32_t> &lanes);
  void account_run(const wtfgpu_run_stats_t &rs);
  bool service_hits(const std::vector<uint32_t> &hits, uint32_t first, std::vector<uint8_t> &done, ModuleSlots *slots,
                    bool per_lane_state);
  void insert_lanes(const Target_t &Target, const std::vector<uint32_t> &lanes,
                    const std::vector<std::pair<const uint8_t *, size_t>> &tcs, ModuleSlots *Slots,
                    std::vector<uint8_t> &ok);
  void target_restore(const Target_t &Target, const std::vector<uint32_t> &lanes, ModuleSlots *Slots);
  void collect_coverage(const std::vector<uint32_t> &lanes, std::vector<LaneResult> &res,
                        const uint64_t *pf_hdr = nullptr);
  std::vector<uint8_t> busy_;
  std::vector<uint64_t> tag_;
  std::vector<uint64_t> tc_bytes_;
  std::vector<LaneResult> lres_;
  std::vector<uint8_t> lres_stale_;
  std::vector<uint32_t> cov_lanes_;
  std::vector<uint64_t> cov_rips_;
  std::vector<uint8_t> cov_want_;
  std::vector<std::pair<uint32_t, uint64_t>> cov_sorted_;
  bool cov_ovf_warned_ = false;
  bool want_gprs_ = true;
  uint64_t last_icount_ = 0;
  LaneResult last_run_;
  bool last_error_ = false;
  struct Part {
    uint32_t lo = 0, hi = 0;
    bool launched = false;
    std::vector<uint32_t> occ, free;
    wtfgpu_exit_t *ex = nullptr;
    uint64_t ex_cap = 0;
    uint8_t *pin = nullptr;
    uint64_t pin_cap = 0;
    bool pf = false, pf_cov = false;
    uint64_t *nb = nullptr, *sargs = nullptr, *cov_hdr = nullptr;
    uint32_t *dc = nullptr;
  };
  bool prefetch_part(Part &P);
  std::vector<Part> parts_;
  uint8_t *wpin_ = nullptr;
  uint64_t wpin_cap_ = 0;
  uint32_t next_part_ = 0;
  uint32_t parts_n() const;
  bool harvest_part(Part &P, const Target_t &Target, std::vector<StreamResult_t> &Out, ModuleSlots *Slots);
  void finish_coverage(uint32_t n, std::vector<LaneResult> *out, std::vector<uint32_t> *timedout);
  bool set_code_pages();

  wtfgpu_ctx *ctx_ = nullptr;
  KernelDump dump_;
  CpuState_t initial_{};
  wtfgpu_regs_t initial_regs_{};
  uint32_t nlanes_ = 0, overlay_pages_ = 0;
  uint64_t limit_ = 0;
  mutable std::vector<LaneView> views_;
  mutable std::vector<uint8_t> touched_;
  struct PrepFeed {
    const uint8_t *p = nullptr;
    uint32_t len = 0;
    uint8_t has = 0, ins = 0;
  };
  std::vector<PrepFeed> pf_;
  static thread_local uint32_t cur_;
  std::unordered_map<uint64_t, BreakpointHandler_t> breakpoints_;
  std::vector<wtfgpu_bp_action_t> bp_actions_;
  uint32_t trace_cap_ = 0;
  uint64_t tenet_cap_ = 0;
  std::unordered_map<uint64_t, BreakpointAction_t::ArgsResult_t> args_results_;
  bool feed_action_ = false;
  bool insert_action_ = false;
  int upload_feed(uint32_t n);
  std::unordered_set<uint64_t> aggregate_;
  std::unordered_set<uint64_t> code_vpns_;
  std::vector<uint64_t> extra_new_;
  void commit_fresh(const std::vector<uint64_t> &fresh);
  std::unordered_set<Gva_t> last_new_coverage_;
  mutable BatchStats stats_;
  struct Block {
    uint8_t *orig = nullptr;
    std::unique_ptr<uint8_t[]> data;
    size_t cap = 0, used = 0;
  };
  struct Arena {
    std::vector<Block> blocks;
    size_t cur = 0;
  };
  mutable std::vector<Arena> arenas_;
  mutable std::mutex spare_mu_;
  mutable std::shared_mutex recycle_mu_;
  void release_slots(size_t n) const;
  std::unordered_map<uint64_t, uint64_t> covlog_count_;
  uint64_t covlog_calls_ = 0;
  void recycle_arenas() const;
  mutable std::atomic<size_t> live_staged_{0};
  mutable std::mutex engine_mu_;
  bool parallel_service(const ModuleSlots *slots) const;
  mutable std::unordered_map<uint64_t, std::vector<uint64_t>> bp_pages_;
  mutable std::unordered_map<uint64_t, uint64_t> fetch_by_bp_;
  mutable std::unordered_set<uint64_t> bp_stack_;
  std::unordered_set<uint64_t> bp_seen_;
  static thread_local uint64_t servicing_bp_, servicing_sp_;
  static thread_local bool scouting_;
  void learn(uint64_t gpfn) const;
  bool full_coverage_ = false;
};


}
```

### wtf_amd/host/runner.cc

```cpp
#include "runner.h"
#include "remote.h"
#include "host_pool.h"
#include "module_instances.h"

#include <sys/resource.h>

#include <algorithm>
#include <atomic>
#include <chrono>
#include <cstdio>
#include <future>
#include <cstdlib>
#include <cstring>
#include <fstream>
#include <thread>

#include "../../include/wtfgpu.h"

namespace wtfgpu_host {

namespace {

constexpr size_t kParMutateMin = 8192, kMutateChunk = 2048;
uint64_t ThreadCpuNs() {
  timespec t{};
  clock_gettime(CLOCK_THREAD_CPUTIME_ID, &t);
  return (uint64_t)t.tv_sec * 1000000000ull + (uint64_t)t.tv_nsec;
}


using Clock = std::chrono::steady_clock;
double secs_since(Clock::time_point t0) { return std::chrono::duration<double>(Clock::now() - t0).count(); }

std::string crash_name(const TestcaseResult_t &R) {
  if (const Crash_t *C = std::get_if<Crash_t>(&R)) return C->CrashName;
  return "";
}

std::string json_escape(const std::string &S) {
  std::string O;
  for (char c : S) {
    if (c == '"' || c == '\\') O += '\\';
    O += c;
  }
  return O;
}

std::vector<fs::path> list_inputs(const fs::path &P) {
  std::vector<fs::path> V;
  if (fs::is_directory(P)) {
    for (const auto &E : fs::directory_iterator(P))
      if (E.is_regular_file()) V.push_back(E.path());
    std::sort(V.begin(), V.end());
  } else if (fs::exists(P)) {
    V.push_back(P);
  }
  return V;
}
  void seg(wtfgpu_seg_t &d, const Seg_t &s) {
  d.base = s.Base;
  d.limit = s.Limit;
  d.selector = s.Selector;
  d.attr = s.Attr;
  d.present = s.Present;
}
}

void FormatTenet(const uint8_t *S, size_t Bytes, FILE *F) {
  static const int Order[16] = {0, 3, 1, 2, 5, 4, 6, 7, 8, 9, 10, 11, 12, 13, 14, 15};
  static const char *Name[17] = {"rax", "rcx", "rdx", "rbx", "rsp", "rbp", "rsi", "rdi", "r8",
                                 "r9",  "r10", "r11", "r12", "r13", "r14", "r15", "rip"};
  static const char *Type[4] = {"", "mr", "mw", "mrw"};
  static const char Hex[] = "0123456789ABCDEF";
  uint64_t Prev[17] = {};
  bool First = true;
  std::string Line, Mem;
  auto word = [&](size_t q) {
    uint64_t v;
    memcpy(&v, S + q, 8);
    return v;
  };
  size_t q = 0;
  while (q + 16 <= Bytes) {
    const uint64_t w0 = word(q), w1 = word(q + 8);
    if (w0 == 2ull << 56) {
      if (q + 8 + 17 * 8 > Bytes) break;
      uint64_t Cur[17];
      memcpy(Cur, S + q + 8, sizeof(Cur));
      Line.clear();
      char Buf[48];
      for (int k = 0; k < 17; k++) {
        const int r = k < 16 ? Order[k] : 16;
        if (!First && Cur[r] == Prev[r]) continue;
        snprintf(Buf, sizeof(Buf), "%s=0x%llx%s", Name[r], (unsigned long long)Cur[r], k < 16 ? "," : "");
        Line += Buf;
      }
      Line += Mem;
      if (!Line.empty()) {
        Line += '\n';
        fwrite(Line.data(), 1, Line.size(), F);
      }
      Mem.clear();
      memcpy(Prev, Cur, sizeof(Prev));
      First = false;
      q += 8 + 17 * 8;
      continue;
    }
    const uint32_t Ty = (uint32_t)(w1 >> 32) & 0xff, Len = (uint32_t)w1;
    if (w1 >> 56 != 1 || Ty == 0 || Ty > 3) break;
    const size_t n = 16 + ((size_t)Len + 7) / 8 * 8;
    if (q + n > Bytes) break;
    char Buf[40];
    snprintf(Buf, sizeof(Buf), ",%s=0x%llx:", Type[Ty], (unsigned long long)w0);
    Mem += Buf;
    for (uint32_t i = 0; i < Len; i++) {
      Mem += Hex[S[q + 16 + i] >> 4];
      Mem += Hex[S[q + 16 + i] & 15];
    }
    q += n;
  }
  if (!Mem.empty()) {
    Mem += '\n';
    fwrite(Mem.data(), 1, Mem.size(), F);
  }
}

wtfgpu_regs_t RegsFromCpuState(const CpuState_t &S) {
  wtfgpu_regs_t r{};
  const uint64_t g[16] = {S.Rax, S.Rcx, S.Rdx, S.Rbx, S.Rsp, S.Rbp, S.Rsi, S.Rdi,
                          S.R8, S.R9, S.R10, S.R11, S.R12, S.R13, S.R14, S.R15};
  memcpy(r.gpr, g, sizeof(g));
  r.rip = S.Rip;
  r.rflags = S.Rflags;
  r.cr0 = S.Cr0.Flags, r.cr2 = S.Cr2, r.cr3 = S.Cr3, r.cr4 = S.Cr4.Flags, r.cr8 = S.Cr8;
  r.efer = S.Efer.Flags, r.xcr0 = S.Xcr0, r.kernel_gs_base = S.KernelGsBase;
  r.star = S.Star, r.lstar = S.Lstar, r.cstar = S.Cstar, r.sfmask = S.Sfmask;
  r.tsc = S.Tsc, r.tsc_aux = S.TscAux, r.apic_base = S.ApicBase, r.pat = S.Pat;
  r.sysenter_cs = S.SysenterCs, r.sysenter_eip = S.SysenterEip, r.sysenter_esp = S.SysenterEsp;
  seg(r.seg[WTFGPU_ES], S.Es), seg(r.seg[WTFGPU_CS], S.Cs), seg(r.seg[WTFGPU_SS], S.Ss);
  seg(r.seg[WTFGPU_DS], S.Ds), seg(r.seg[WTFGPU_FS], S.Fs), seg(r.seg[WTFGPU_GS], S.Gs);
  seg(r.seg[WTFGPU_TR], S.Tr), seg(r.seg[WTFGPU_LDTR], S.Ldtr);
  r.gdtr_base = S.Gdtr.Base, r.gdtr_limit = S.Gdtr.Limit, r.idtr_base = S.Idtr.Base, r.idtr_limit = S.Idtr.Limit;
  r.mxcsr = S.Mxcsr, r.mxcsr_mask = S.MxcsrMask;
  r.fpcw = S.Fpcw, r.fpsw = S.Fpsw, r.fptw = S.Fptw, r.fpop = S.Fpop;
  memcpy(r.fpst, S.Fpst, sizeof(r.fpst));
  for (int i = 0; i < 16; i++) {
    r.xmm[i][0] = S.Zmm[i].Q[0], r.xmm[i][1] = S.Zmm[i].Q[1];
    r.ymmh[i][0] = S.Zmm[i].Q[2], r.ymmh[i][1] = S.Zmm[i].Q[3];
    for (int q = 0; q < 4; q++) r.zmmh[i][q] = S.Zmm[i].Q[4 + q];
    for (int q = 0; q < 8; q++) r.zmm_hi[i][q] = S.Zmm[16 + i].Q[q];
  }
  return r;
}

TestcaseResult_t FaultToResult(uint32_t vector, uint32_t error, uint64_t rip, uint64_t addr, uint32_t cpl) {
  uint32_t code = EXCEPTION_ACCESS_VIOLATION_READ;
  switch (vector) {
    case WTFGPU_VEC_DE: code = EXCEPTION_INT_DIVIDE_BY_ZERO; break;
    case WTFGPU_VEC_UD: code = EXCEPTION_ILLEGAL_INSTRUCTION; break;
    case WTFGPU_VEC_GP: code = EXCEPTION_ACCESS_VIOLATION_READ; break;
    case WTFGPU_VEC_PF:
      code = (error & ErrorInstructionFetch) ? EXCEPTION_ACCESS_VIOLATION_EXECUTE
             : (error & ErrorWrite)          ? EXCEPTION_ACCESS_VIOLATION_WRITE
                                             : EXCEPTION_ACCESS_VIOLATION_READ;
      break;
    default: break;
  }
  char name[160];
  if (cpl == 3)
    snprintf(name, sizeof(name), "crash-%s-%#llx", std::string(ExceptionCodeToStr(code)).c_str(),
             (unsigned long long)rip);
  else if (vector == WTFGPU_VEC_PF)
    snprintf(name, sizeof(name), "crash-0x50-0x%llx-0x%x-0x%llx-0x0-0x0", (unsigned long long)addr,
             (error & ErrorInstructionFetch) ? 0x10u : (error & ErrorWrite) ? 2u : 0u, (unsigned long long)rip);
  else
    snprintf(name, sizeof(name), "crash-0x1e-0x%x-0x%llx-0x0-0x0-0x0",
             vector == WTFGPU_VEC_DE ? 0xc0000094u : vector == WTFGPU_VEC_UD ? 0xc000001du : 0xc0000005u,
             (unsigned long long)rip);
  return Crash_t(name);
}

static std::string bytes_to_human(uint64_t B) {
  const char *Unit = "b";
  double V = double(B);
  const double K = 1024, M = K * K, G = M * K;
  if (V >= G) Unit = "gb", V /= G;
  else if (V >= M) Unit = "mb", V /= M;
  else if (V >= K) Unit = "kb", V /= K;
  char b[64];
  snprintf(b, sizeof(b), "%.1f%s", V, Unit);
  return b;
}
static std::string number_to_human(uint64_t N) {
  const char *Unit = "";
  double V = double(N);
  if (V > 1e6) Unit = "m", V /= 1e6;
  else if (V > 1e3) Unit = "k", V /= 1e3;
  char b[64];
  snprintf(b, sizeof(b), "%.1f%s", V, Unit);
  return b;
}

void PrintTestcaseRunStats(const LaneResult &L, size_t AggregateCoverage) {
  printf("--------------------------------------------------\n");
  printf("Run stats:\n");
  printf("Instructions executed: %s (%s unique)\n", number_to_human(L.icount).c_str(),
         number_to_human(AggregateCoverage).c_str());
  printf("          Dirty pages: %s\n", bytes_to_human((uint64_t)L.dirty * Page::Size).c_str());
  printf("      Memory accesses: %s\n", bytes_to_human(L.bytes).c_str());
  printf("       Edges executed: %s (%s unique)\n", number_to_human(L.edges).c_str(),
         number_to_human(L.edges_new).c_str());
}

bool ParseRunnerArgs(int argc, char **argv, RunnerOptions &O) {
  for (int i = 1; i < argc; i++) {
    const std::string a = argv[i];
    auto next = [&](const char *what) -> const char * {
      if (i + 1 >= argc) {
        fprintf(stderr, "%s needs a value\n", what);
        exit(2);
      }
      return argv[++i];
    };
    if (a == "run" || a == "fuzz" || a == "master") O.mode = a;
    else if (a == "--name") O.name = next("--name");
    else if (a == "--target") O.target = next("--target");
    else if (a == "--input") O.input = next("--input");
    else if (a == "--results") O.results = next("--results");
    else if (a == "--limit") O.limit = strtoull(next("--limit"), nullptr, 0);
    else if (a == "--lanes") O.lanes = (uint32_t)strtoul(next("--lanes"), nullptr, 0);
    else if (a == "--overlay-pages") O.overlay_pages = (uint32_t)strtoul(next("--overlay-pages"), nullptr, 0);
    else if (a == "--runs") O.runs = strtoull(next("--runs"), nullptr, 0);
    else if (a == "--seconds") O.seconds = atof(next("--seconds"));
    else if (a == "--seed") O.seed = strtoull(next("--seed"), nullptr, 0);
    else if (a == "--max_len") O.max_len = strtoull(next("--max_len"), nullptr, 0);
    else if (a == "--device") O.device = atoi(next("--device"));
    else if (a == "--full-coverage") O.full_coverage = true;
    else if (a == "--edges") O.edges = true;
    else if (a == "--trace-path") O.trace_path = next("--trace-path");
    else if (a == "--trace-type") O.trace_type = next("--trace-type");
    else if (a == "--trace-cap") O.trace_cap = (uint32_t)strtoul(next("--trace-cap"), nullptr, 0);
    else if (a == "--tenet-cap") O.tenet_cap = strtoull(next("--tenet-cap"), nullptr, 0) & ~7ull;
    else if (a == "--quiet") O.quiet = true;
    else if (a == "--serial-mutation") O.serial_mutation = true;
    else if (a == "--slice-steps") O.slice = strtoull(next("--slice-steps"), nullptr, 0);
    else if (a == "--regroup-steps") O.regroup = strtoull(next("--regroup-steps"), nullptr, 0);
    else if (a == "--stream-run") O.stream_run = true;
    else if (a == "--serial") O.serial = true;
    else if (a == "--module-so") O.module_so = next("--module-so");
    else if (a == "--rank") O.rank = atoi(next("--rank"));
    else if (a == "--world") O.world = atoi(next("--world"));
    else if (a == "--exchange") O.exchange = next("--exchange");
    else if (a == "--nccl-id-file") O.nccl_id_file = next("--nccl-id-file");
    else if (a == "--rccl-force") O.rccl_force = true;
    else if (a == "--address") O.address = next("--address");
    else if (a == "--nodes") O.nodes = atoi(next("--nodes"));
    else if (a == "--batched") O.batched = true;
    else if (a == "--sample") O.sample = next("--sample");
    else if (a == "--sample-every") O.sample_every = strtoull(next("--sample-every"), nullptr, 0);
    else {
      fprintf(stderr, "unknown argument %s\n", a.c_str());
      return false;
    }
  }
  if (const char *e = getenv("WTF_RCCL_FORCE")) O.rccl_force = O.rccl_force || atoi(e) != 0;
  if (O.world < 1 || O.rank < 0 || O.rank >= O.world) {
    fprintf(stderr, "--rank must be in [0, --world)\n");
    return false;
  }
  if (O.mode == "master" && (O.address.empty() || O.nodes < 1)) {
    fprintf(stderr, "master needs --address and --nodes >= 1\n");
    return false;
  }
  if (O.name.empty() || O.target.empty()) {
    fprintf(stderr, "usage: [run|fuzz|master] --name <target> --target <dir> [--input p] [--results f] [--limit n]\n"
                    "       [--lanes n] [--overlay-pages k] [--runs n] [--seconds s] [--seed s] [--full-coverage]\n"
                    "       [--serial-mutation] [--slice-steps s] [--regroup-steps r] [--rank r --world n [--exchange host:port | --nccl-id-file f]]\n"
                    "       [--address tcp://ip:port|unix://path [--batched] [--nodes k]] [--edges]\n"
                    "       [--trace-path dir [--trace-type rip|cov|tenet] [--trace-cap n] [--tenet-cap bytes]] [--module-so m.so] [--serial]\n");
    return false;
  }
  return true;
}

bool LoadTarget(const RunnerOptions &O, Options_t &Opts, CpuState_t &State) {
  const fs::path T(O.target);
  Opts.TargetName = O.name;
  Opts.StatePath = T / "state";
  Opts.DumpPath = Opts.StatePath / "mem.dmp";
  Opts.CpuStatePath = Opts.StatePath / "regs.json";
  Opts.SymbolFilePath = Opts.StatePath / "symbol-store.json";
  Opts.Limit = O.limit;
  Opts.Edges = O.edges;
  Opts.GpuDevice = O.device;
  Opts.GpuLanes = O.lanes;
  Opts.GpuOverlayPages = O.overlay_pages;
  if (O.full_coverage) Opts.GpuCoverageSet = 8192;
  Opts.Fuzz.Seed = (uint32_t)O.seed;
  if (!LoadCpuStateFromJSON(State, Opts.CpuStatePath)) {
    printf("Failed to load the CPU state from %s\n", Opts.CpuStatePath.string().c_str());
    return false;
  }
  if (!SanitizeCpuState(State)) return false;
  Opts.CpuState = State;
  if (!g_Dbg.Init(Opts.DumpPath, Opts.SymbolFilePath)) return false;
  return true;
}

int RunnerMain(const RunnerOptions &O, Executor_t &Exec, const Options_t &Opts, const CpuState_t &State,
               CoverageExchange_t *X) {
  std::unique_ptr<ModuleInstances> Inst;
  Target_t *Target = nullptr;
  std::unique_ptr<Target_t> Copy0;
  if (!O.module_so.empty()) {
    Inst = std::make_unique<ModuleInstances>();
    if (!Inst->Load(O.module_so, O.name, Exec.Lanes())) return 1;
    Copy0 = std::make_unique<Target_t>(Inst->TargetOf(0));
    Target = Copy0.get();
  } else {
    Target = Targets_t::Instance().Get(O.name);
  }
  if (!Target) {
    printf("Target %s not found\n", O.name.c_str());
    Targets_t::Instance().DisplayRegisteredTargets();
    return 1;
  }
  g_Backend = Exec.AsBackend();
  if (Inst ? !Inst->InitAll(Opts, State) : !Target->Init(Opts, State)) {
    printf("Failed to initialize the target\n");
    return 1;
  }
  const uint32_t N = Exec.Lanes();
  ModuleSlots Slots;
  Slots.Capture(N);
  Slots.AttachInstances(Inst.get());
  Exec.SetFullCoverage(O.full_coverage);

  if (O.mode == "run") {
    auto Inputs = list_inputs(O.input.empty() ? fs::path(O.target) / "inputs" : fs::path(O.input));
    const uint64_t Runs = O.runs ? O.runs : 1;
    const bool Stats = Inputs.size() == 1 && Runs == 1 && !O.quiet;
    LaneResult Last;
    const bool Trace = !O.trace_path.empty();
    std::unordered_set<uint64_t> TraceSeen;
    if (Trace) {
      if (O.trace_type != "rip" && O.trace_type != "cov" && O.trace_type != "tenet") {
        printf("--trace-type %s is not supported by this backend (rip, cov, tenet)\n", O.trace_type.c_str());
        return 1;
      }
      if (O.trace_type == "tenet") {
        const uint64_t Cap = O.tenet_cap ? O.tenet_cap : std::min<uint64_t>(1ull << 24, (32ull << 30) / N) & ~7ull;
        if (!Exec.EnableTenet(Cap)) {
          printf("EnableTenet failed (%u lanes x %llu bytes)\n", N, (unsigned long long)Cap);
          return 1;
        }
      } else if (!Exec.EnableTrace(O.trace_cap)) {
        printf("EnableTrace failed\n");
        return 1;
      }
      fs::create_directories(O.trace_path);
      std::vector<fs::path> Keep;
      for (const fs::path &In : Inputs) {
        if (fs::exists(fs::path(O.trace_path) / (In.filename().string() + ".trace")))
          printf("Skipping %s as it already exists.\n", In.string().c_str());
        else Keep.push_back(In);
      }
      Inputs = Keep;
    }
    std::vector<uint64_t> RepOf(Inputs.size(), 0);
    if (Runs > 1) {
      std::vector<fs::path> Rep;
      Rep.reserve(Inputs.size() * Runs);
      RepOf.clear();
      for (const fs::path &In : Inputs)
        for (uint64_t k = 0; k < Runs; k++) {
          Rep.push_back(In);
          RepOf.push_back(k);
        }
      Inputs.swap(Rep);
    }
    auto write_trace = [&](const fs::path &In, uint32_t Lane, uint64_t Rep) -> bool {
      if (Rep) {
        if (O.trace_type != "cov") return true;
        std::vector<uint64_t> Rips;
        bool Truncated = false;
        if (!Exec.LaneTrace(Lane, Rips, Truncated)) return false;
        TraceSeen.insert(Rips.begin(), Rips.end());
        return true;
      }
      if (O.trace_type == "tenet") {
        std::vector<uint8_t> Bytes;
        bool Truncated = false;
        if (!Exec.LaneTenet(Lane, Bytes, Truncated)) return false;
        FILE *F = fopen((fs::path(O.trace_path) / (In.filename().string() + ".trace")).c_str(), "w");
        if (!F) return false;
        FormatTenet(Bytes.data(), Bytes.size(), F);
        fclose(F);
        if (Truncated) printf("tenet trace of %s truncated at %zu bytes (--tenet-cap)\n", In.string().c_str(), Bytes.size());
        return true;
      }
      std::vector<uint64_t> Rips;
      bool Truncated = false;
      if (!Exec.LaneTrace(Lane, Rips, Truncated)) return false;
      FILE *F = fopen((fs::path(O.trace_path) / (In.filename().string() + ".trace")).c_str(), "w");
      if (!F) return false;
      for (uint64_t R : Rips)
        if (O.trace_type == "rip" || TraceSeen.insert(R).second) fprintf(F, "%#llx\n", (unsigned long long)R);
      TraceSeen.clear();
      fclose(F);
      if (Truncated) printf("trace of %s truncated at %zu rips (--trace-cap)\n", In.string().c_str(), Rips.size());
      return true;
    };
    FILE *Out = O.results.empty() ? stdout : fopen(O.results.c_str(), "w");
    if (!Out) return 1;
    const auto t0 = Clock::now();
    uint64_t Retired = 0;
    auto print = [&](const fs::path &In, const LaneResult &L) {
      std::vector<uint64_t> Cov = L.new_coverage;
      std::sort(Cov.begin(), Cov.end());
      fprintf(Out, "{\"input\":\"%s\",\"result\":\"%s\",\"crash\":\"%s\",\"error\":%d,\"exit\":%u,\"icount\":%llu,",
              json_escape(In.filename().string()).c_str(), TestcaseResultName(L.result).c_str(),
              json_escape(crash_name(L.result)).c_str(), (int)L.error, L.exit_status, (unsigned long long)L.icount);
      fprintf(Out, "\"gprs\":[");
      for (int g = 0; g < 18; g++) fprintf(Out, "%s%llu", g ? "," : "", (unsigned long long)L.gprs[g]);
      fprintf(Out, "],\"coverage\":[");
      for (size_t c = 0; c < Cov.size(); c++) fprintf(Out, "%s%llu", c ? "," : "", (unsigned long long)Cov[c]);
      fprintf(Out, "],\"bytes\":%llu,\"dirty\":%u,\"edges\":%llu,\"edges_new\":%llu,\"handler_fault\":%d}\n",
              (unsigned long long)L.bytes, L.dirty, (unsigned long long)L.edges, (unsigned long long)L.edges_new,
              (int)L.handler_fault);
      Last = L;
    };
    if (O.serial && !Trace) {
      Backend_t *B = Exec.AsBackend();
      static const Registers_t Order[18] = {
          Registers_t::Rax, Registers_t::Rcx, Registers_t::Rdx, Registers_t::Rbx, Registers_t::Rsp, Registers_t::Rbp,
          Registers_t::Rsi, Registers_t::Rdi, Registers_t::R8,  Registers_t::R9,  Registers_t::R10, Registers_t::R11,
          Registers_t::R12, Registers_t::R13, Registers_t::R14, Registers_t::R15, Registers_t::Rip, Registers_t::Rflags};
      for (const fs::path &In : Inputs) {
        g_Backend = B;
        const std::vector<uint8_t> Buf = ReadFile(In);
        LaneResult L;
        bool Inserted = false;
        try {
          Inserted = Target->InsertTestcase(Buf.data(), Buf.size());
        } catch (const HandlerFault_t &) {
          L.error = true;
          L.handler_fault = true;
        }
        if (!Inserted) {
          L.result = L.error ? Crash_t() : Crash_t("insert-testcase-failed");
        } else {
          const std::optional<TestcaseResult_t> Res = B->Run(Buf.data(), Buf.size());
          if (!Res) {
            printf("Run failed\n");
            return 1;
          }
          L.result = *Res;
          for (const Gva_t &G : B->LastNewCoverage()) L.new_coverage.push_back(G.U64());
          if (std::holds_alternative<Timedout_t>(*Res)) B->RevokeLastNewCoverage();
          L.icount = Exec.LastIcount();
          L.error = Exec.LastError();
          L.handler_fault = Exec.LastHandlerFault();
          Exec.LastRunStats(L);
        }
        for (int g = 0; g < 18; g++) L.gprs[g] = B->GetReg(Order[g]);
        L.rip = L.gprs[16];
        if (!Target->Restore() || !B->Restore(State)) {
          printf("Restore failed\n");
          return 1;
        }
        Retired += L.icount;
        print(In, L);
      }
    }
    if (O.stream_run && Exec.CanStream() && !Trace) {
      std::vector<std::vector<uint8_t>> Bufs(Inputs.size());
      std::vector<LaneResult> Res(Inputs.size());
      std::vector<uint8_t> Got(Inputs.size(), 0);
      size_t next = 0, got = 0;
      while (got < Inputs.size()) {
        std::vector<StreamTestcase_t> In;
        for (uint32_t f = Exec.FreeLanes(); f && next < Inputs.size(); f--, next++) {
          Bufs[next] = ReadFile(Inputs[next]);
          In.push_back(StreamTestcase_t{Bufs[next].data(), Bufs[next].size(), next});
        }
        std::vector<StreamResult_t> R;
        size_t Taken = 0;
        if (!Exec.StreamStep(*Target, In, O.slice ? O.slice : 4096, R, &Slots, &Taken)) {
          printf("StreamStep failed\n");
          return 1;
        }
        next -= In.size() - Taken;
        for (StreamResult_t &F : R) {
          Res[F.tag] = std::move(*F.r);
          Got[F.tag] = 1;
          got++;
        }
      }
      for (size_t i = 0; i < Inputs.size(); i++) {
        Retired += Res[i].icount;
        print(Inputs[i], Res[i]);
      }
    }
    for (size_t b = (O.stream_run && Exec.CanStream() && !Trace) || (O.serial && !Trace) ? Inputs.size() : 0;
         b < Inputs.size(); b += N) {
      const size_t n = std::min<size_t>(N, Inputs.size() - b);
      std::vector<std::vector<uint8_t>> Bufs(n);
      std::vector<std::pair<const uint8_t *, size_t>> Tc(n);
      for (size_t i = 0; i < n; i++) {
        Bufs[i] = ReadFile(Inputs[b + i]);
        Tc[i] = {Bufs[i].data(), Bufs[i].size()};
      }
      if (O.full_coverage) Exec.ResetCoverage();
      std::vector<LaneResult> R;
      if (!Exec.RunBatch(*Target, Tc, R, &Slots)) {
        printf("RunBatch failed\n");
        return 1;
      }
      for (size_t i = 0; i < n; i++) {
        Retired += R[i].icount;
        print(Inputs[b + i], R[i]);
        if (Trace && !write_trace(Inputs[b + i], (uint32_t)i, RepOf[b + i])) {
          printf("trace of %s failed\n", Inputs[b + i].string().c_str());
          return 1;
        }
      }
    }
    if (Out != stdout) fclose(Out);
    if (Stats) PrintTestcaseRunStats(Last, Exec.CoverageSize());
    if (!O.quiet)
      fprintf(stderr, "run: %zu testcases, %llu instructions, %.3f s\n", Inputs.size(), (unsigned long long)Retired,
              secs_since(t0));
    return 0;
  }

  if (!O.address.empty()) return NodeMain(O, Exec, *Target, Slots);

  if (X && X->Exchanging() && O.full_coverage) {
    printf("--full-coverage is a single-node parity mode (not with --world > 1)\n");
    return 1;
  }
  FuzzSession F(O, Exec, *Target, Slots, X);
  if (!F.Start()) {
    printf("Nothing to run: empty corpus and no inputs\n");
    return 1;
  }
  const bool Shards = X && X->Exchanging();
  for (;;) {
    if (Shards ? F.AllDone() : F.Done()) break;
    if (!F.Step()) {
      printf("RunBatch failed\n");
      return 1;
    }
  }
  if (Shards && !F.FinishMerge()) return 1;
  F.FlushFiles();
  printf("%s\n", F.SummaryJson().c_str());
  return 0;
}

FileWriter::FileWriter() : Th_([this] { Loop(); }) {}

FileWriter::~FileWriter() {
  {
    std::lock_guard<std::mutex> g(Mu_);
    Stop_ = true;
  }
  Cv_.notify_all();
  Th_.join();
}

void FileWriter::Save(std::filesystem::path Path, const uint8_t *Data, size_t Size) {
  {
    std::lock_guard<std::mutex> g(Mu_);
    Q_.emplace_back(std::move(Path), std::vector<uint8_t>(Data, Data + Size));
  }
  Cv_.notify_one();
}

void FileWriter::Flush() {
  std::unique_lock<std::mutex> g(Mu_);
  Idle_.wait(g, [this] { return Q_.empty() && !Busy_; });
}

void FileWriter::Loop() {
  std::unique_lock<std::mutex> g(Mu_);
  for (;;) {
    Cv_.wait(g, [this] { return Stop_ || !Q_.empty(); });
    if (Q_.empty()) return;
    auto F = std::move(Q_.front());
    Q_.pop_front();
    Busy_ = true;
    g.unlock();
    SaveFile(F.first, F.second.data(), F.second.size());
    g.lock();
    Busy_ = false;
    if (Q_.empty()) Idle_.notify_all();
  }
}

FuzzSession::FuzzSession(const RunnerOptions &O, Executor_t &Exec, Target_t &Target, ModuleSlots &Slots,
                         CoverageExchange_t *X)
    : O_(O), Exec_(Exec), Target_(Target), Slots_(Slots), X_(X),
      Rng_(O.seed + (X ? (uint64_t)X->Rank() : 0)), T_(O.target), Corpus_(T_ / "outputs", Rng_) {}

FuzzSession::~FuzzSession() {
  if (Next_.valid()) Next_.wait();
  Writer_.Flush();
  if (Sample_) fclose(Sample_);
}

void FuzzSession::WriteSample(const uint8_t *Tc, size_t Size, const LaneResult &L) {
  static const char *hex = "0123456789abcdef";
  std::string H(2 * Size, '0');
  for (size_t i = 0; i < Size; i++) {
    H[2 * i] = hex[Tc[i] >> 4];
    H[2 * i + 1] = hex[Tc[i] & 15];
  }
  std::vector<uint64_t> Cov = L.new_coverage;
  std::sort(Cov.begin(), Cov.end());
  fprintf(Sample_, "{\"tc\":\"%s\",\"result\":\"%s\",\"crash\":\"%s\",\"error\":%d,\"icount\":%llu,\"gprs\":[",
          H.c_str(), TestcaseResultName(L.result).c_str(), json_escape(crash_name(L.result)).c_str(), (int)L.error,
          (unsigned long long)L.icount);
  for (int g = 0; g < 18; g++) fprintf(Sample_, "%s%llu", g ? "," : "", (unsigned long long)L.gprs[g]);
  fprintf(Sample_, "],\"coverage\":[");
  for (size_t c = 0; c < Cov.size(); c++) fprintf(Sample_, "%s%llu", c ? "," : "", (unsigned long long)Cov[c]);
  fprintf(Sample_, "]}\n");
}

bool FuzzSession::Start() {
  Exec_.SetWantRegisters(!O_.sample.empty());
  if (!O_.sample.empty()) {
    Sample_ = fopen(O_.sample.c_str(), "w");
    if (!Sample_) return false;
  }
  fs::create_directories(T_ / "outputs");
  fs::create_directories(T_ / "crashes");
  if (Target_.CreateMutator) Mutator_ = Target_.CreateMutator(Rng_, O_.max_len);
  if (!Mutator_) {
    printf("Target %s has no mutator\n", O_.name.c_str());
    return false;
  }
  for (const auto &P : list_inputs(T_ / "inputs")) {
    const auto B = ReadFile(P);
    Pending_.emplace_back(B.begin(), B.end());
  }
  t0_ = Clock::now();
  stream_ = O_.slice && Exec_.CanStream();
  if (stream_ && Exec_.TakesPrepared() && !Slots_.Instances() && !getenv("WTF_NO_PREPARED_INSERT"))
    Prepare_ = Target_.PrepareInsert;
  if (stream_) {
    Adopt(MakeBatch(Budget(Exec_.Lanes())));
    return !Ready_.empty();
  }
  Batch_ = MakeBatch(Budget(Exec_.Lanes()));
  return !Batch_.empty();
}

void FuzzSession::Adopt(TcBatch &&B) {
  for (std::unique_ptr<TcArena> &A : B) {
    if (!A || A->Count() == 0) continue;
    A->Live = A->Count();
    for (size_t i = 0; i < A->Count(); i++) Ready_.push_back(TcRef{A.get(), (uint32_t)i});
    TcArena *K = A.get();
    Arenas_.emplace(K, std::move(A));
  }
}

uint64_t FuzzSession::Budget(uint64_t n) const {
  if (!O_.runs) return n;
  const uint64_t made = S_.execs + (stream_ ? InFlight_ + Ready_.size() : 0);
  return made >= O_.runs ? 0 : std::min<uint64_t>(n, O_.runs - made);
}

bool FuzzSession::Done() const {
  if (!stream_) return Batch_.empty();
  if (O_.seconds > 0 && secs_since(t0_) >= O_.seconds) return true;
  return Ready_.empty() && InFlight_ == 0 && !Next_.valid() &&
         (Budget(1) == 0 || !More(S_.execs) || Corpus_.Size() == 0);
}

bool FuzzSession::More(uint64_t done) const {
  return (O_.runs == 0 || done < O_.runs) && (O_.seconds <= 0 || secs_since(t0_) < O_.seconds);
}

double FuzzSession::WallSeconds() const { return secs_since(t0_); }

TcBatch FuzzSession::MakeBatch(uint64_t n) {
  TcBatch Batch;
  size_t Made = 0;
  auto Tail = [&]() -> TcArena & {
    if (Batch.empty()) Batch.push_back(NewArena());
    return *Batch.back();
  };
  while (Made < n && !Pending_.empty()) {
    Tail().Add(Pending_.back().data(), Pending_.back().size());
    Pending_.pop_back();
    Made++;
  }
  const size_t Need = n - Made;
  if (Corpus_.Size() && Need >= kParMutateMin && !O_.serial_mutation) {
    const size_t Chunks = (Need + kMutateChunk - 1) / kMutateChunk;
    std::vector<uint64_t> Seeds(Chunks);
    for (uint64_t &S : Seeds) S = Rng_();
    std::vector<std::unique_ptr<TcArena>> Out(Chunks);
    std::atomic<size_t> NextChunk{0};
    std::atomic<uint64_t> CpuNs{0};
    auto Work = [&]() {
      const uint64_t c0 = ThreadCpuNs();
      for (size_t c; (c = NextChunk.fetch_add(1)) < Chunks;) {
        std::mt19937_64 R(Seeds[c]);
        Corpus_t View(Corpus_, R);
        std::unique_ptr<Mutator_t> M = Target_.CreateMutator(R, O_.max_len);
        if (HaveNewCov_) M->OnNewCoverage(Testcase_t((const uint8_t *)LastNewCov_.data(), LastNewCov_.size()));
        auto A = NewArena();
        const size_t End = std::min(Need, (c + 1) * kMutateChunk);
        A->Off.reserve(End - c * kMutateChunk + 1);
        std::vector<uint8_t> Scratch;
        for (size_t i = c * kMutateChunk; i < End; i++) {
          const std::string S = M->GetNewTestcase(View);
          A->Add(S.data(), std::min<size_t>(S.size(), O_.max_len));
          if (Prepare_) A->Prepare(Prepare_, Scratch);
        }
        Out[c] = std::move(A);
      }
      CpuNs += ThreadCpuNs() - c0;
    };
    std::vector<std::thread> Pool;
    static const unsigned MutThreads = [] {
      const char *e = getenv("WTF_MUTATE_THREADS");
      return e && atoi(e) > 0 ? (unsigned)atoi(e) : host_threads();
    }();
    for (unsigned t = 1; t < MutThreads; t++) Pool.emplace_back(Work);
    Work();
    for (std::thread &Th : Pool) Th.join();
    MutateCpuNs_ += CpuNs.load();
    for (std::unique_ptr<TcArena> &A : Out) Batch.push_back(std::move(A));
    Made += Need;
    Batch.push_back(NewArena());
  }
  while (Made < n) {
    if (Corpus_.Size() == 0 && Made == 0) break;
    if (Corpus_.Size()) {
      const std::string S = Mutator_->GetNewTestcase(Corpus_);
      Tail().Add(S.data(), std::min<size_t>(S.size(), O_.max_len));
    } else {
      size_t k = Rng_() % Made;
      const TcArena *F = nullptr;
      for (const std::unique_ptr<TcArena> &A : Batch) {
        if (k < A->Count()) {
          F = A.get();
          break;
        }
        k -= A->Count();
      }
      const std::vector<uint8_t> Copy(F->Ptr(k), F->Ptr(k) + F->Len(k));
      Tail().Add(Copy.data(), Copy.size());
    }
    Made++;
  }
  Batch.erase(std::remove_if(Batch.begin(), Batch.end(), [](const std::unique_ptr<TcArena> &A) { return A->Count() == 0; }),
              Batch.end());
  return Batch;
}

bool FuzzSession::Step() {
  const bool done = Done();
  if (X_ && X_->Exchanging() && done) return MergeCoverage(true);
  if (stream_) {
    const auto tc = Clock::now();
    const bool ok = StreamStep(done);
    S_.call_ms += secs_since(tc) * 1e3;
    return ok;
  }
  BatchRefs_.clear();
  for (const std::unique_ptr<TcArena> &A : Batch_)
    for (size_t i = 0; i < A->Count(); i++) BatchRefs_.push_back(TcRef{A.get(), (uint32_t)i});
  if (BatchRefs_.empty()) return true;
  std::vector<std::pair<const uint8_t *, size_t>> Tc(BatchRefs_.size());
  for (size_t i = 0; i < BatchRefs_.size(); i++) Tc[i] = {BatchRefs_[i].data(), BatchRefs_[i].size()};
  std::vector<LaneResult> R;
  const auto tb = Clock::now();
  const uint64_t after = S_.execs + BatchRefs_.size();
  if (More(after) && Corpus_.Size()) {
    const uint64_t n = O_.runs ? std::min<uint64_t>(Exec_.Lanes(), O_.runs - after) : Exec_.Lanes();
    Next_ = std::async(std::launch::async, &FuzzSession::MakeBatch, this, n);
  }
  if (!Exec_.RunBatch(Target_, Tc, R, &Slots_)) return false;
  S_.run_s += secs_since(tb);
  S_.batches++;
  TcBatch NextBatch;
  if (Next_.valid()) NextBatch = Next_.get();
  for (size_t i = 0; i < BatchRefs_.size(); i++) Account(BatchRefs_[i].data(), BatchRefs_[i].size(), R[i]);
  if (X_ && X_->Exchanging() && !MergeCoverage(false)) return false;
  if (!NextBatch.empty() || !More(S_.execs))
    Batch_ = std::move(NextBatch);
  else
    Batch_ = MakeBatch(Budget(Exec_.Lanes()));
  return true;
}

bool FuzzSession::StreamStep(bool Done) {
  if (Done) return true;
  const auto t_step = Clock::now();
  std::vector<StreamTestcase_t> In;
  const bool open = More(S_.execs);
  if (open) {
    const uint32_t free = Exec_.FreeLanes();
    if (Ready_.size() < free && !Next_.valid() && Corpus_.Size()) {
      const auto tm = Clock::now();
      Adopt(MakeBatch(Budget(free - Ready_.size())));
      S_.make_ms += secs_since(tm) * 1e3;
    }
    const size_t take = std::min<size_t>(free, Ready_.size());
    while (FreeSlot_.size() < take) {
      FreeSlot_.push_back(Slot_.size());
      Slot_.emplace_back();
    }
    const size_t base = FreeSlot_.size() - take;
    std::vector<TcRef> Refs(Ready_.begin(), Ready_.begin() + (std::ptrdiff_t)take);
    Ready_.erase(Ready_.begin(), Ready_.begin() + (std::ptrdiff_t)take);
    In.resize(take);
    HostPool::Get().For(take, 1024, [&](size_t i) {
      const uint64_t tag = FreeSlot_[base + i];
      const TcRef R = Refs[i];
      Slot_[tag] = R;
      StreamTestcase_t T{R.data(), R.size(), tag};
      if (R.A->Prep.size() == R.A->Count()) {
        T.prep = R.prep();
        T.prep_data = R.prep_data();
        T.prep_size = R.prep_size();
      }
      In[i] = T;
    }, take >= 4096);
    FreeSlot_.resize(base);
    InFlight_ += take;
    const uint64_t want = Budget(Exec_.Lanes() > Ready_.size() ? Exec_.Lanes() - Ready_.size() : 0);
    if (want && Corpus_.Size() && !Next_.valid())
      Next_ = std::async(std::launch::async, &FuzzSession::MakeBatch, this, want);
  }
  std::vector<StreamResult_t> Out;
  const auto tb = Clock::now();
  S_.fill_ms += std::chrono::duration<double, std::milli>(tb - t_step).count();
  size_t Taken = 0;
  const bool ok = Exec_.StreamStep(Target_, In, O_.slice, Out, &Slots_, &Taken);
  S_.run_s += secs_since(tb);
  for (size_t i = In.size(); i-- > Taken;) {
    Ready_.push_front(Slot_[In[i].tag]);
    Slot_[In[i].tag] = TcRef{};
    FreeSlot_.push_back(In[i].tag);
    InFlight_--;
  }
  const auto tw = Clock::now();
  if (Next_.valid()) Adopt(Next_.get());
  const auto ta = Clock::now();
  S_.produce_wait_ms += std::chrono::duration<double, std::milli>(ta - tw).count();
  if (!ok) return false;
  S_.batches++;
  for (const StreamResult_t &F : Out)
    if (F.tag >= Slot_.size()) return false;
  AccountStep(Out);
  S_.account_ms += secs_since(ta) * 1e3;
  if (X_ && X_->Exchanging() && !MergeCoverage(false)) return false;
  S_.step_ms += secs_since(t_step) * 1e3;
  return true;
}

std::unique_ptr<TcArena> FuzzSession::NewArena() {
  {
    std::lock_guard<std::mutex> g(ArenaPoolMu_);
    if (!ArenaPool_.empty()) {
      std::unique_ptr<TcArena> A = std::move(ArenaPool_.back());
      ArenaPool_.pop_back();
      return A;
    }
  }
  return std::make_unique<TcArena>();
}

void FuzzSession::ReleaseArena(TcArena *A) {
  auto it = Arenas_.find(A);
  if (it == Arenas_.end()) return;
  std::unique_ptr<TcArena> Own = std::move(it->second);
  Arenas_.erase(it);
  Own->Data.clear();
  Own->Off.assign(1, 0);
  Own->Live = 0;
  Own->Prep.clear();
  Own->PrepData.clear();
  Own->PrepOff.assign(1, 0);
  std::lock_guard<std::mutex> g(ArenaPoolMu_);
  if (ArenaPool_.size() < 512) ArenaPool_.push_back(std::move(Own));
}

void FuzzSession::AccountStep(std::vector<StreamResult_t> &Out) {
  const size_t n = Out.size();
  enum : uint8_t { K_SERIAL = 1, K_TIMEOUT = 2, K_CR3 = 4, K_CRASH = 8 };
  std::vector<uint8_t> Kind(n, 0);
  std::vector<TcArena *> Ar(n);
  struct Sum {
    uint64_t retired = 0, timeouts = 0, cr3 = 0, crashes = 0;
  };
  const unsigned T = HostPool::Get().Threads();
  std::vector<Sum> Part(T + 1);
  const bool every = Sample_ != nullptr;
  HostPool::Get().For(n, 1024, [&](size_t i) {
    const LaneResult &L = *Out[i].r;
    const TcRef R = Slot_[Out[i].tag];
    Ar[i] = R.A;
    uint8_t k = 0;
    if (every || L.error) {
      k = K_SERIAL;
    } else {
      if (std::holds_alternative<Timedout_t>(L.result)) k |= K_TIMEOUT;
      if (std::holds_alternative<Cr3Change_t>(L.result)) k |= K_CR3;
      if (const Crash_t *C = std::get_if<Crash_t>(&L.result)) {
        k |= K_CRASH;
        if (!C->CrashName.empty() && !CrashNames_.count(C->CrashName)) k = K_SERIAL;
      }
      if (!L.new_coverage.empty() && !std::holds_alternative<Timedout_t>(L.result)) k = K_SERIAL;
    }
    Kind[i] = k;
    if (k != K_SERIAL) {
      Sum &s = Part[HostPool::ThreadIndex()];
      s.retired += L.icount;
      s.timeouts += (k & K_TIMEOUT) != 0;
      s.cr3 += (k & K_CR3) != 0;
      s.crashes += (k & K_CRASH) != 0;
    }
  }, n >= 4096);
  uint64_t bulk = 0;
  for (size_t i = 0; i < n; i++) {
    if (Kind[i] != K_SERIAL) {
      bulk++;
      continue;
    }
    const TcRef R = Slot_[Out[i].tag];
    Account(R.data(), R.size(), *Out[i].r, false);
  }
  S_.execs += bulk;
  for (const Sum &s : Part) {
    S_.retired += s.retired;
    S_.timeouts += s.timeouts;
    S_.cr3 += s.cr3;
    S_.crashes += s.crashes;
  }
  const size_t fs = FreeSlot_.size();
  FreeSlot_.resize(fs + n);
  HostPool::Get().For(n, 4096, [&](size_t i) {
    Slot_[Out[i].tag] = TcRef{};
    FreeSlot_[fs + i] = Out[i].tag;
  }, n >= 8192);
  InFlight_ -= n;
  for (size_t i = 0; i < n;) {
    size_t j = i + 1;
    while (j < n && Ar[j] == Ar[i]) j++;
    TcArena *A = Ar[i];
    A->Live -= j - i;
    if (A->Live == 0) ReleaseArena(A);
    i = j;
  }
}

void FuzzSession::Account(const uint8_t *Tc, size_t Size, const LaneResult &L, bool KnownCrash) {
  if (Sample_ && S_.execs % std::max<uint64_t>(1, O_.sample_every) == 0) WriteSample(Tc, Size, L);
  S_.execs++;
  S_.retired += L.icount;
  if (L.error) {
    if (S_.errors < 256) {
      std::error_code ec;
      fs::create_directories(T_ / "errors", ec);
      SaveFile(T_ / "errors" / ("engine-error-" + std::to_string(S_.errors)), Tc, Size);
    }
    S_.errors++;
    S_.error_retired += L.icount;
    return;
  }
  if (std::holds_alternative<Timedout_t>(L.result)) S_.timeouts++;
  if (std::holds_alternative<Cr3Change_t>(L.result)) S_.cr3++;
  if (const Crash_t *C = std::get_if<Crash_t>(&L.result)) {
    S_.crashes++;
    if (!KnownCrash && !C->CrashName.empty()) {
      const auto tc = Clock::now();
      if (CrashNames_.insert(C->CrashName).second) Writer_.Save(T_ / "crashes" / C->CrashName, Tc, Size);
      S_.crashsave_ms += secs_since(tc) * 1e3;
    }
  }
  if (!L.new_coverage.empty() && !std::holds_alternative<Timedout_t>(L.result)) {
    const auto tn = Clock::now();
    const size_t Before = Coverage_.size();
    Coverage_.insert(L.new_coverage.begin(), L.new_coverage.end());
    if (Coverage_.size() != Before) {
      Testcase_t Tcase(Tc, Size);
      Mutator_->OnNewCoverage(Tcase);
      LastNewCov_.assign((const char *)Tc, Size);
      HaveNewCov_ = true;
      Corpus_.SaveTestcase(L.result, std::move(Tcase));
    }
    S_.newcov_ms += secs_since(tn) * 1e3;
  }
}

bool FuzzSession::MergeCoverage(bool Done) {
  const auto t = Clock::now();
  if (!AbsorbMerge()) return false;
  uint8_t *Map = nullptr;
  uint64_t Bytes = 0;
  bool Device = false;
  if (!Exec_.CoverageMap(&Map, &Bytes, &Device)) return false;
  std::vector<uint64_t> Mine;
  Exec_.TakeNewExtra(Mine);
  if (!X_->MergeBegin(Map, Bytes, Device, Mine, Done)) return false;
  MergePending_ = true;
  S_.merge_ms += secs_since(t) * 1e3;
  return true;
}

bool FuzzSession::AbsorbMerge() {
  if (!MergePending_) return true;
  MergePending_ = false;
  const uint8_t *Merged = nullptr;
  uint64_t Bytes = 0;
  std::vector<uint64_t> All;
  bool Every = false;
  if (!X_->MergeEnd(&Merged, &Bytes, All, &Every)) return false;
  uint8_t *Map = nullptr;
  uint64_t MapBytes = 0;
  bool Device = false;
  if (!Exec_.CoverageMap(&Map, &MapBytes, &Device)) return false;
  if (Bytes && Bytes == MapBytes) S_.merged_rips += Exec_.MergeCoverageMap(Merged, Bytes, Device);
  S_.merged_rips += Exec_.AbsorbExtra(All);
  S_.merges++;
  S_.merged_map_bytes += Bytes;
  AllDone_ = Every;
  return true;
}

bool FuzzSession::FinishMerge() {
  const auto t = Clock::now();
  const bool ok = AbsorbMerge();
  S_.merge_ms += secs_since(t) * 1e3;
  return ok;
}

bool CoverageExchange_t::MergeBegin(const uint8_t *Map, uint64_t Bytes, bool Device,
                                    const std::vector<uint64_t> &Extras, bool Done) {
  if (Device) return false;
  merged_.assign(Map, Map + Bytes);
  merged_device_ = false;
  if (Bytes && !AllReduceMax(merged_.data(), Bytes, false)) return false;
  std::vector<uint64_t> Block(1 + blocks_.Cap()), Blocks;
  Block.resize(blocks_.Pack(Extras, Done, Block.data()));
  if (!AllGatherV(Block, Blocks)) return false;
  return MergeBlocks::Unpack(Blocks.data(), Blocks.size(), (uint64_t)World(), 0, kMergeCap, merged_extra_,
                             &merged_done_);
}

bool CoverageExchange_t::MergeEnd(const uint8_t **Merged, uint64_t *Bytes, std::vector<uint64_t> &AllExtras,
                                  bool *AllDone) {
  *Merged = merged_.data();
  *Bytes = merged_.size();
  AllExtras.swap(merged_extra_);
  merged_extra_.clear();
  *AllDone = merged_done_;
  return true;
}

static double ProcessCpuSeconds() {
  struct rusage u {};
  getrusage(RUSAGE_SELF, &u);
  return (double)u.ru_utime.tv_sec + u.ru_utime.tv_usec * 1e-6 + (double)u.ru_stime.tv_sec + u.ru_stime.tv_usec * 1e-6;
}

std::string FuzzSession::SummaryJson() const {
  const double Wall = WallSeconds();
  char b[2048];
  snprintf(b, sizeof(b),
           "{\"mode\":\"fuzz\",\"target\":\"%s\",\"lanes\":%u,\"rank\":%d,\"world\":%d,\"batches\":%llu,"
           "\"execs\":%llu,\"retired\":%llu,\"wall_s\":%.6f,\"run_s\":%.6f,\"execs_per_s\":%.3f,"
           "\"instr_per_s\":%.3f,\"coverage\":%zu,\"corpus\":%zu,\"crashes\":%llu,\"unique_crashes\":%zu,"
           "\"timeouts\":%llu,\"cr3\":%llu,\"errors\":%llu,\"error_retired\":%llu,\"merged_rips\":%llu,"
           "\"merges\":%llu,\"merged_map_bytes\":%llu,"
           "\"merge_ms\":%.3f,\"produce_wait_ms\":%.3f,\"account_ms\":%.3f,\"make_ms\":%.3f,\"step_ms\":%.3f,\"fill_ms\":%.3f,"
           "\"newcov_ms\":%.3f,\"crashsave_ms\":%.3f,\"call_ms\":%.3f,\"cpu_s\":%.3f,\"mutate_cpu_ms\":%.3f,"
           "\"backend\":",
           O_.name.c_str(), Exec_.Lanes(), X_ ? X_->Rank() : 0, X_ ? X_->World() : 1,
           (unsigned long long)S_.batches, (unsigned long long)S_.execs, (unsigned long long)S_.retired, Wall,
           S_.run_s, S_.run_s > 0 ? S_.execs / S_.run_s : 0.0, S_.run_s > 0 ? S_.retired / S_.run_s : 0.0,
           Exec_.CoverageSize(), Corpus_.Size(), (unsigned long long)S_.crashes, CrashNames_.size(),
           (unsigned long long)S_.timeouts, (unsigned long long)S_.cr3, (unsigned long long)S_.errors,
           (unsigned long long)S_.error_retired, (unsigned long long)S_.merged_rips,
           (unsigned long long)S_.merges, (unsigned long long)S_.merged_map_bytes, S_.merge_ms, S_.produce_wait_ms,
           S_.account_ms, S_.make_ms, S_.step_ms, S_.fill_ms, S_.newcov_ms, S_.crashsave_ms, S_.call_ms, ProcessCpuSeconds(),
           MutateCpuNs_.load() * 1e-6);
  return std::string(b) + Exec_.StatsJson() + "}";
}

}
```

### wtf_amd/host/runner.h

```cpp
#pragma once
#include <atomic>
#include <chrono>
#include <condition_variable>
#include <filesystem>
#include <mutex>
#include <thread>
#include <cstdint>
#include <deque>
#include <unordered_map>
#include <future>
#include <random>
#include <string>
#include <unordered_set>
#include <utility>
#include <vector>

#include "../../include/wtfgpu.h"
#include "merge_block.h"
#include "wtf_api.h"

namespace wtfgpu_host {

struct LaneResult {
  TestcaseResult_t result;
  bool error = false;
  bool handler_fault = false;
  uint32_t exit_status = 0;
  uint64_t icount = 0;
  uint64_t rip = 0;
  uint64_t gprs[18] = {};
  std::vector<uint64_t> new_coverage;
  uint64_t bytes = 0, edges = 0, edges_new = 0;
  uint32_t dirty = 0;
};

struct StreamTestcase_t {
  const uint8_t *data;
  size_t size;
  uint64_t tag;
  PreparedInsert_t prep = PreparedInsert_t::Call;
  const uint8_t *prep_data = nullptr;
  size_t prep_size = 0;
};
struct StreamResult_t {
  uint64_t tag;
  LaneResult *r;
};

class Executor_t {
 public:
  virtual bool CanStream() const { return false; }
  virtual bool TakesPrepared() const { return false; }
  virtual uint32_t FreeLanes() const { return 0; }
  virtual bool StreamStep(const Target_t &, const std::vector<StreamTestcase_t> &, uint64_t,
                          std::vector<StreamResult_t> &, ModuleSlots *, size_t *Taken) {
    if (Taken) *Taken = 0;
    return false;
  }

  virtual ~Executor_t() = default;
  virtual Backend_t *AsBackend() = 0;
  virtual uint32_t Lanes() const = 0;
  virtual bool RunBatch(const Target_t &Target, const std::vector<std::pair<const uint8_t *, size_t>> &Testcases,
                        std::vector<LaneResult> &Out, ModuleSlots *Slots) = 0;
  virtual void ResetCoverage() = 0;
  virtual void SetFullCoverage(bool On) = 0;
  virtual void SetWantRegisters(bool) {}
  virtual uint64_t LastIcount() const { return 0; }
  virtual bool LastError() const { return false; }
  virtual bool LastHandlerFault() const { return false; }
  virtual void LastRunStats(LaneResult &) const {}
  virtual size_t CoverageSize() const = 0;
  virtual std::string StatsJson() const { return "{}"; }
  virtual bool CoverageMap(uint8_t **Map, uint64_t *Bytes, bool *Device) {
    *Map = nullptr;
    *Bytes = 0;
    *Device = false;
    return true;
  }
  virtual size_t AbsorbCoverageMap() { return 0; }
  virtual size_t MergeCoverageMap(const uint8_t *, uint64_t, bool) { return 0; }
  virtual void TakeNewExtra(std::vector<uint64_t> &Out) { Out.clear(); }
  virtual size_t AbsorbExtra(const std::vector<uint64_t> &) { return 0; }
  virtual bool EnableTrace(uint32_t) { return false; }
  virtual bool LaneTrace(uint32_t, std::vector<uint64_t> &, bool &) { return false; }
  virtual bool EnableTenet(uint64_t) { return false; }
  virtual bool LaneTenet(uint32_t, std::vector<uint8_t> &, bool &) { return false; }
};

class CoverageExchange_t {
 public:
  virtual ~CoverageExchange_t() = default;
  virtual int Rank() const = 0;
  virtual int World() const = 0;
  virtual bool Exchanging() const { return World() > 1; }
  virtual bool AllReduceMax(uint8_t *Map, uint64_t Bytes, bool Device) = 0;
  virtual bool AllDone(bool Mine, bool *All) = 0;
  virtual bool AllGatherV(const std::vector<uint64_t> &Mine, std::vector<uint64_t> &All) = 0;

  virtual bool MergeBegin(const uint8_t *Map, uint64_t Bytes, bool Device, const std::vector<uint64_t> &Extras,
                          bool Done);
  virtual bool MergeEnd(const uint8_t **Merged, uint64_t *Bytes, std::vector<uint64_t> &AllExtras, bool *AllDone);

 protected:
  std::vector<uint8_t> merged_;
  std::vector<uint64_t> merged_extra_;
  bool merged_done_ = false, merged_device_ = false;
  MergeBlocks blocks_{kMergeCap};
};

void PrintTestcaseRunStats(const LaneResult &L, size_t AggregateCoverage);

struct RunnerOptions {
  std::string mode = "run";
  std::string name;
  std::string target;
  std::string input;
  std::string results;
  uint64_t limit = 0;
  uint32_t lanes = 1;
  uint32_t overlay_pages = 32;
  uint64_t runs = 0;
  double seconds = 0;
  uint64_t seed = 1337;
  uint64_t max_len = 0x1000;
  int device = 0;
  bool full_coverage = false;
  bool edges = false;
  std::string trace_path;
  std::string trace_type = "rip";
  uint32_t trace_cap = 1u << 20;
  uint64_t tenet_cap = 0;
  bool quiet = false;
  bool serial_mutation = false;
  uint64_t slice = 4096;
  uint64_t regroup = ~0ull;
  bool stream_run = false;
  bool serial = false;
  std::string module_so;
  int rank = 0, world = 1;
  std::string exchange = "127.0.0.1:31337";
  std::string nccl_id_file;
  bool rccl_force = false;
  std::string address;
  int nodes = 1;
  bool batched = false;
  std::string sample;
  uint64_t sample_every = 0;
};

struct FuzzStats {
  uint64_t execs = 0, retired = 0, crashes = 0, timeouts = 0, cr3 = 0, errors = 0, batches = 0, merged_rips = 0;
  uint64_t merges = 0, merged_map_bytes = 0;
  uint64_t error_retired = 0;
  double run_s = 0, merge_ms = 0;
  double produce_wait_ms = 0, account_ms = 0;
  double make_ms = 0, step_ms = 0;
  double fill_ms = 0;
  double call_ms = 0;
  double newcov_ms = 0, crashsave_ms = 0;
};

struct TcArena {
  std::vector<uint8_t> Data;
  std::vector<uint64_t> Off{0};
  size_t Live = 0;
  std::vector<PreparedInsert_t> Prep;
  std::vector<uint8_t> PrepData;
  std::vector<uint64_t> PrepOff{0};
  void Add(const void *P, size_t N) {
    const uint8_t *B = (const uint8_t *)P;
    Data.insert(Data.end(), B, B + N);
    Off.push_back(Data.size());
  }
  void Prepare(PrepareInsert_t F, std::vector<uint8_t> &Scratch) {
    const size_t I = Count() - 1;
    Scratch.clear();
    const PreparedInsert_t K = F(Ptr(I), Len(I), Scratch);
    Prep.push_back(K);
    if (K == PreparedInsert_t::Feed) PrepData.insert(PrepData.end(), Scratch.begin(), Scratch.end());
    PrepOff.push_back(PrepData.size());
  }
  size_t Count() const { return Off.size() - 1; }
  const uint8_t *Ptr(size_t I) const { return Data.data() + Off[I]; }
  size_t Len(size_t I) const { return Off[I + 1] - Off[I]; }
};
using TcBatch = std::vector<std::unique_ptr<TcArena>>;
struct TcRef {
  TcArena *A = nullptr;
  uint32_t I = 0;
  const uint8_t *data() const { return A->Ptr(I); }
  size_t size() const { return A->Len(I); }
  PreparedInsert_t prep() const { return I < A->Prep.size() ? A->Prep[I] : PreparedInsert_t::Call; }
  const uint8_t *prep_data() const { return A->PrepData.data() + A->PrepOff[I]; }
  size_t prep_size() const { return A->PrepOff[I + 1] - A->PrepOff[I]; }
};

class FileWriter {
 public:
  FileWriter();
  ~FileWriter();
  void Save(std::filesystem::path Path, const uint8_t *Data, size_t Size);
  void Flush();

 private:
  void Loop();
  std::mutex Mu_;
  std::condition_variable Cv_, Idle_;
  std::deque<std::pair<std::filesystem::path, std::vector<uint8_t>>> Q_;
  bool Stop_ = false, Busy_ = false;
  std::thread Th_;
};

class FuzzSession {
 public:
  FuzzSession(const RunnerOptions &O, Executor_t &Exec, Target_t &Target, ModuleSlots &Slots,
              CoverageExchange_t *X);
  ~FuzzSession();
  bool Start();
  bool Step();
  bool Done() const;
  bool AllDone() const { return AllDone_; }
  bool FinishMerge();
  const FuzzStats &Stats() const { return S_; }
  size_t CorpusSize() const { return Corpus_.Size(); }
  double WallSeconds() const;
  std::string SummaryJson() const;
  void FlushFiles() { Writer_.Flush(); }

 private:
  TcBatch MakeBatch(uint64_t n);
  PrepareInsert_t Prepare_ = nullptr;
  std::atomic<uint64_t> MutateCpuNs_{0};
  void Adopt(TcBatch &&B);
  uint64_t Budget(uint64_t n) const;
  bool More(uint64_t done) const;
  bool MergeCoverage(bool Done);
  bool AbsorbMerge();
  bool MergePending_ = false, AllDone_ = false;
  void WriteSample(const uint8_t *Tc, size_t Size, const LaneResult &L);
  FILE *Sample_ = nullptr;
  bool StreamStep(bool Done);
  void Account(const uint8_t *Tc, size_t Size, const LaneResult &L, bool KnownCrash = false);
  void AccountStep(std::vector<StreamResult_t> &Out);
  void ReleaseArena(TcArena *A);
  std::unique_ptr<TcArena> NewArena();
  std::mutex ArenaPoolMu_;
  std::vector<std::unique_ptr<TcArena>> ArenaPool_;

  const RunnerOptions O_;
  Executor_t &Exec_;
  Target_t &Target_;
  ModuleSlots &Slots_;
  CoverageExchange_t *X_;
  std::mt19937_64 Rng_;
  fs::path T_;
  Corpus_t Corpus_;
  std::unique_ptr<Mutator_t> Mutator_;
  std::vector<std::string> Pending_;
  TcBatch Batch_;
  std::vector<TcRef> BatchRefs_;
  std::string LastNewCov_;
  bool HaveNewCov_ = false;
  std::future<TcBatch> Next_;
  FileWriter Writer_;
  std::unordered_set<std::string> CrashNames_;
  std::unordered_set<uint64_t> Coverage_;
  FuzzStats S_;
  std::chrono::steady_clock::time_point t0_;
  bool stream_ = false;
  std::deque<TcRef> Ready_;
  std::unordered_map<TcArena *, std::unique_ptr<TcArena>> Arenas_;
  std::vector<TcRef> Slot_;
  std::vector<uint64_t> FreeSlot_;
  size_t InFlight_ = 0;
};

bool ParseRunnerArgs(int argc, char **argv, RunnerOptions &O);
void FormatTenet(const uint8_t *Stream, size_t Bytes, FILE *F);
int RunnerMain(const RunnerOptions &O, Executor_t &Exec, const Options_t &Opts, const CpuState_t &State,
               CoverageExchange_t *X = nullptr);
bool LoadTarget(const RunnerOptions &O, Options_t &Opts, CpuState_t &State);

TestcaseResult_t FaultToResult(uint32_t vector, uint32_t error, uint64_t rip, uint64_t addr, uint32_t cpl);

wtfgpu_regs_t RegsFromCpuState(const CpuState_t &S);

}
```

Baseline: 13.79 million.

## Chunk host refill, harvest and accounting into reusable per-chunk buffers with fast paths

Restructures the streaming host path so refill, harvest and result accounting each run as one chunked parallel pass with reusable member buffers, replacing several separate passes that allocated fresh vectors on every step. Harvest classifies exits and fills results directly in a single pass, and plain OK lanes skip building a LaneResult by passing only an icount. The ready queue now stores testcase ranges instead of individual refs, and stale-result clearing only visits lanes that were actually used. This aims to cut CPU-side per-step overhead between GPU launches, at the cost of more complex state tracking, such as the plain_ and res_used bookkeeping, where correctness bugs could hide.

```diff
diff --git a/wtf_amd/host/gpu_backend.cc b/wtf_amd/host/gpu_backend.cc
--- a/wtf_amd/host/gpu_backend.cc
+++ b/wtf_amd/host/gpu_backend.cc
@@ -716,7 +716,14 @@
     if (hit[pi] == 1) hits.push_back(pending[pi]);
     if (hit[pi] == 2) named.push_back(pending[pi]);
   }
-  if (named.empty()) return true;
+  name_stop_args(named, first, ex, done, out, stop_args);
+  return true;
+}
+
+void GpuBackend_t::name_stop_args(const std::vector<uint32_t> &named, uint32_t first, const wtfgpu_exit_t *ex,
+                                  std::vector<uint8_t> &done, std::vector<LaneResult> *out,
+                                  const uint64_t *stop_args) {
+  if (named.empty()) return;
   std::vector<uint64_t> args(named.size() * 6);
   bool ok = true;
   if (stop_args) {
@@ -741,18 +748,36 @@
     done[l - first] = 1;
   }, named.size() >= 2048);
   stats_.err_other += bad;
-  return true;
 }
 
 bool GpuBackend_t::fill_results(const std::vector<uint32_t> &lanes, uint32_t first,
                                 const wtfgpu_exit_t *ex, const std::vector<uint8_t> &done,
                                 std::vector<LaneResult> *out, std::vector<uint32_t> *finished) {
-  const auto tg = Clock::now();
   std::vector<uint32_t> fin;
   for (uint32_t l : lanes)
     if (done[l - first]) fin.push_back(l);
   if (finished) finished->insert(finished->end(), fin.begin(), fin.end());
-  if (!out) return true;
+  return !out || fill_lanes(fin, first, ex, *out);
+}
+
+void GpuBackend_t::fill_lane(uint32_t l, const wtfgpu_exit_t &e, LaneResult &r) {
+  const LaneView &v = views_[l];
+  const bool t = touched_[l] != 0;
+  r.result = t && v.result ? std::move(*v.result) : TestcaseResult_t(Ok_t());
+  if (t && v.handler_fault) {
+    r.result = Crash_t();
+    r.error = true;
+    r.handler_fault = true;
+    stats_.err_handler++;
+  }
+  r.rip = e.rip;
+  r.icount = e.icount;
+  r.exit_status = e.status;
+}
+
+bool GpuBackend_t::fill_lanes(const std::vector<uint32_t> &fin, uint32_t first, const wtfgpu_exit_t *ex,
+                              std::vector<LaneResult> &out) {
+  const auto tg = Clock::now();
   std::vector<uint64_t> regs;
   uint32_t lo = 0, hi = 0;
   std::vector<uint64_t> nb;
@@ -772,16 +797,8 @@
     }
   }
   HostPool::Get().For(fin.size(), 1024, [&](size_t i) {
-    LaneResult &r = (*out)[fin[i]];
-    const LaneView &v = views_[fin[i]];
-    const bool t = touched_[fin[i]] != 0;
-    r.result = t && v.result ? std::move(*v.result) : TestcaseResult_t(Ok_t());
-    if (t && v.handler_fault) {
-      r.result = Crash_t();
-      r.error = true;
-      r.handler_fault = true;
-      stats_.err_handler++;
-    }
+    LaneResult &r = out[fin[i]];
+    fill_lane(fin[i], ex[fin[i] - first], r);
     if (want_gprs_) {
       memcpy(r.gprs, &regs[i * 18], 18 * 8);
       r.rip = r.gprs[16];
@@ -790,11 +807,7 @@
       r.dirty = std::min(dc[k], overlay_pages_);
       r.edges = ec[2 * k];
       r.edges_new = ec[2 * k + 1];
-    } else {
-      r.rip = ex[fin[i] - first].rip;
-    }
-    r.icount = ex[fin[i] - first].icount;
-    r.exit_status = ex[fin[i] - first].status;
+    }
   }, fin.size() >= 2048);
   stats_.regs_ms += ms_since(tg);
   return true;
@@ -1346,8 +1359,9 @@
     tag_.assign(nlanes_, 0);
     tc_bytes_.assign(nlanes_, 0);
     lres_.assign(nlanes_, LaneResult{});
-    lres_stale_.assign(nlanes_, 0);
+    plain_.assign(nlanes_, 0);
     const uint32_t n = parts_n();
+    done_.assign((nlanes_ + n - 1) / n + 1, 0);
     parts_.assign(n, Part{});
     for (uint32_t p = 0; p < n; p++) {
       Part &Q = parts_[p];
@@ -1368,117 +1382,170 @@
   if (pipelined && P.launched && !harvest_part(P, Target, Out, Slots)) return false;
   const auto ti = Clock::now();
   stats_.harvest_ms += std::chrono::duration<double, std::milli>(ti - t0).count();
-  std::vector<uint32_t> fresh;
-  std::vector<std::pair<const uint8_t *, size_t>> tcs;
-  fresh.reserve(std::min<size_t>(In.size(), P.hi - P.lo));
-  tcs.reserve(fresh.capacity());
+  std::vector<uint32_t> &fresh = fresh_;
   {
     const size_t take = std::min(In.size(), P.free.size());
     fresh.assign(P.free.begin(), P.free.begin() + (std::ptrdiff_t)take);
     P.free.erase(P.free.begin(), P.free.begin() + (std::ptrdiff_t)take);
-    tcs.resize(take);
-    for (size_t i = 0; i < take; i++) tcs[i] = {In[i].data, In[i].size};
   }
   if (Taken) *Taken = fresh.size();
   stats_.fresh_ms += ms_since(ti);
   if (!fresh.empty()) {
     if (wtfgpu_restore_lanes(ctx_, fresh.data(), (uint32_t)fresh.size())) return false;
     stats_.restore_dev_ms += ms_since(ti);
-    std::vector<uint8_t> prepared(fresh.size(), 0);
-    HostPool::Get().For(fresh.size(), 256, [&](size_t i) {
-      const uint32_t l = fresh[i];
-      if (touched_[l]) reset_view(l);
-      pf_[l] = PrepFeed{};
-      busy_[l] = 1;
-      tag_[l] = In[i].tag;
-      tc_bytes_[l] = In[i].size;
-      lres_stale_[l] = 1;
-      const StreamTestcase_t &T = In[i];
-      switch (T.prep) {
-        case PreparedInsert_t::Call: return;
-        case PreparedInsert_t::Failed: view(l).result = Crash_t("insert-testcase-failed"); break;
-        case PreparedInsert_t::Nothing: break;
-        case PreparedInsert_t::Feed:
-          if (!feed_action_ || T.prep_size > kFeedRegion) return;
-          pf_[l] = PrepFeed{T.prep_data, (uint32_t)T.prep_size, 1, 0};
-          break;
-        case PreparedInsert_t::Insert:
-          if (!insert_action_ || T.size + 4 > kFeedRegion) return;
-          pf_[l] = PrepFeed{T.data, (uint32_t)T.size, 1, 1};
-          break;
+    const size_t n = fresh.size();
+    const bool feeds = feed_action_ || insert_action_;
+    constexpr size_t kChunk = 1024;
+    const size_t chunks = (n + kChunk - 1) / kChunk;
+    if (rchunks_.size() < chunks) rchunks_.resize(chunks);
+    if (flen_.size() < n) {
+      flen_.resize(n);
+      fhas_.resize(n);
+      foff_.resize(n + 1);
+    }
+    HostPool::Get().For(chunks, 1, [&](size_t c) {
+      RefillChunk &C = rchunks_[c];
+      C.call.clear();
+      C.pre.clear();
+      C.bytes = 0;
+      const size_t hi = std::min(n, (c + 1) * kChunk);
+      for (size_t i = c * kChunk; i < hi; i++) {
+        const uint32_t l = fresh[i];
+        if (touched_[l]) reset_view(l);
+        PrepFeed f{};
+        busy_[l] = 1;
+        tag_[l] = In[i].tag;
+        tc_bytes_[l] = In[i].size;
+        const StreamTestcase_t &T = In[i];
+        bool prepared = true;
+        switch (T.prep) {
+          case PreparedInsert_t::Call: prepared = false; break;
+          case PreparedInsert_t::Failed:
+            view(l).result = Crash_t("insert-testcase-failed");
+            C.pre.push_back(l);
+            break;
+          case PreparedInsert_t::Nothing: break;
+          case PreparedInsert_t::Feed:
+            if (!feed_action_ || T.prep_size > kFeedRegion)
+              prepared = false;
+            else
+              f = PrepFeed{T.prep_data, (uint32_t)T.prep_size, 1, 0};
+            break;
+          case PreparedInsert_t::Insert:
+            if (!insert_action_ || T.size + 4 > kFeedRegion)
+              prepared = false;
+            else
+              f = PrepFeed{T.data, (uint32_t)T.size, 1, 1};
+            break;
+        }
+        pf_[l] = f;
+        flen_[i] = f.has ? f.len + (f.ins ? 4 : 0) : 0;
+        fhas_[i] = f.has;
+        C.bytes += flen_[i];
+        if (!prepared) {
+          C.call.push_back((uint32_t)i);
+          continue;
+        }
+        if (Slots) Slots->ResetLane(l);
       }
-      if (Slots) Slots->ResetLane(l);
-      prepared[i] = 1;
-    });
+    }, n >= 512);
     recycle_arenas();
     const auto tm = Clock::now();
     stats_.restore_ms += std::chrono::duration<double, std::milli>(tm - ti).count();
-    std::vector<uint32_t> call;
-    std::vector<std::pair<const uint8_t *, size_t>> call_tcs;
-    for (size_t i = 0; i < fresh.size(); i++)
-      if (!prepared[i]) {
-        call.push_back(fresh[i]);
-        call_tcs.push_back(tcs[i]);
+    call_.clear();
+    pre_.clear();
+    for (size_t c = 0; c < chunks; c++) {
+      call_.insert(call_.end(), rchunks_[c].call.begin(), rchunks_[c].call.end());
+      pre_.insert(pre_.end(), rchunks_[c].pre.begin(), rchunks_[c].pre.end());
+    }
+    stats_.prepared += n - call_.size();
+    std::vector<uint32_t> call(call_.size());
+    if (!call_.empty()) {
+      std::vector<std::pair<const uint8_t *, size_t>> call_tcs(call_.size());
+      for (size_t k = 0; k < call_.size(); k++) {
+        call[k] = fresh[call_[k]];
+        call_tcs[k] = {In[call_[k]].data, In[call_[k]].size};
       }
-    stats_.prepared += fresh.size() - call.size();
-    if (!call.empty()) {
       std::vector<uint8_t> ok;
       insert_lanes(Target, call, call_tcs, Slots, ok);
-      for (size_t i = 0; i < call.size(); i++)
-        if (!ok[i]) view(call[i]).result = Crash_t("insert-testcase-failed");
+      for (size_t k = 0; k < call.size(); k++)
+        if (!ok[k]) view(call[k]).result = Crash_t("insert-testcase-failed");
     }
     const auto tu = Clock::now();
     stats_.module_ms += std::chrono::duration<double, std::milli>(tu - tm).count();
     if (flush_lanes(call)) return false;
-    if (feed_action_ || insert_action_) {
+    if (!call_.empty()) {
+      std::vector<uint32_t> pre_call;
+      for (size_t k = 0; k < call_.size(); k++) {
+        const uint32_t i = call_[k], l = call[k];
+        if (!touched_[l]) continue;
+        const LaneView &v = views_[l];
+        flen_[i] = (uint32_t)v.feed.size();
+        fhas_[i] = v.has_feed;
+        rchunks_[i / kChunk].bytes += flen_[i];
+        if (v.result.has_value()) pre_call.push_back(l);
+      }
+      if (!pre_call.empty()) {
+        tmp_lanes_.resize(pre_.size() + pre_call.size());
+        std::merge(pre_.begin(), pre_.end(), pre_call.begin(), pre_call.end(), tmp_lanes_.begin());
+        pre_.swap(tmp_lanes_);
+      }
+    }
+    if (feeds) {
       const auto tf = Clock::now();
-      const size_t n = fresh.size();
-      std::vector<uint64_t> off(n + 1, 0);
-      std::vector<uint8_t> has(n);
-      HostPool::Get().For(n, 1024, [&](size_t i) {
-        const uint32_t l = fresh[i];
-        const PrepFeed &f = pf_[l];
-        const bool t = !f.has && touched_[l];
-        off[i + 1] = f.has ? f.len + (f.ins ? 4 : 0) : t ? views_[l].feed.size() : 0;
-        has[i] = f.has || (t && views_[l].has_feed);
-      });
-      for (size_t i = 0; i < n; i++) off[i + 1] += off[i];
-      if (off[n] > P.pin_cap) {
+      uint64_t total = 0;
+      for (size_t c = 0; c < chunks; c++) {
+        const uint64_t b = rchunks_[c].bytes;
+        rchunks_[c].bytes = total;
+        total += b;
+      }
+      foff_[n] = total;
+      if (total > P.pin_cap) {
         if (P.pin) wtfgpu_host_free(ctx_, P.pin);
         P.pin = nullptr;
-        P.pin_cap = std::max<uint64_t>(off[n] * 2, 1 << 20);
+        P.pin_cap = std::max<uint64_t>(total * 2, 1 << 20);
         void *p = nullptr;
         if (wtfgpu_host_alloc(ctx_, P.pin_cap, &p)) return false;
         P.pin = (uint8_t *)p;
       }
-      HostPool::Get().For(n, 256, [&](size_t i) {
-        const uint32_t l = fresh[i];
-        const PrepFeed &f = pf_[l];
-        uint8_t *o = P.pin + off[i];
-        if (f.has) {
-          if (f.ins) {
-            memcpy(o, &f.len, 4);
-            o += 4;
+      HostPool::Get().For(chunks, 1, [&](size_t c) {
+        uint64_t at = rchunks_[c].bytes;
+        const size_t hi = std::min(n, (c + 1) * kChunk);
+        for (size_t i = c * kChunk; i < hi; i++) {
+          foff_[i] = at;
+          if (!flen_[i]) continue;
+          const uint32_t l = fresh[i];
+          const PrepFeed &f = pf_[l];
+          uint8_t *o = P.pin + at;
+          if (f.has) {
+            if (f.ins) {
+              memcpy(o, &f.len, 4);
+              o += 4;
+            }
+            if (f.len) memcpy(o, f.p, f.len);
+          } else {
+            memcpy(o, views_[l].feed.data(), flen_[i]);
           }
-          if (f.len) memcpy(o, f.p, f.len);
-        } else if (touched_[l] && !views_[l].feed.empty()) {
-          memcpy(o, views_[l].feed.data(), views_[l].feed.size());
+          at += flen_[i];
         }
-      });
-      if (wtfgpu_set_feed_lanes(ctx_, fresh.data(), (uint32_t)n, off.data(), has.data(), P.pin, off[n]))
+      }, n >= 512);
+      if (wtfgpu_set_feed_lanes(ctx_, fresh.data(), (uint32_t)n, foff_.data(), fhas_.data(), P.pin, total))
         return false;
       stats_.up_feed_ms += ms_since(tf);
     }
-    if (!stop_prestopped(fresh)) return false;
+    if (!pre_.empty() && wtfgpu_stop(ctx_, pre_.data(), (uint32_t)pre_.size(), WTFGPU_EXIT_STOPPED) != WTFGPU_OK)
+      return false;
     stats_.upload_ms += ms_since(tu);
     stats_.testcases += fresh.size();
   }
   stats_.insert_ms += ms_since(ti);
   const auto to = Clock::now();
-  if (!fresh.empty()) {
-    std::vector<uint32_t> occ(P.occ.size() + fresh.size());
-    std::merge(P.occ.begin(), P.occ.end(), fresh.begin(), fresh.end(), occ.begin());
-    P.occ.swap(occ);
+  if (P.occ.empty()) {
+    P.occ.swap(fresh);
+  } else if (!fresh.empty()) {
+    tmp_lanes_.resize(P.occ.size() + fresh.size());
+    std::merge(P.occ.begin(), P.occ.end(), fresh.begin(), fresh.end(), tmp_lanes_.begin());
+    P.occ.swap(tmp_lanes_);
   }
   stats_.occ_ms += ms_since(to);
   if (!P.occ.empty()) {
@@ -1529,11 +1596,8 @@
   account_run(rs);
   P.launched = false;
   const uint32_t first = P.lo, count = P.hi - P.lo;
-  HostPool::Get().For(P.occ.size(), 1024, [&](size_t i) {
-    const uint32_t l = P.occ[i];
-    if (!lres_stale_[l]) return;
-    lres_stale_[l] = 0;
-    LaneResult &r = lres_[l];
+  HostPool::Get().For(P.res_used.size(), 1024, [&](size_t i) {
+    LaneResult &r = lres_[P.res_used[i]];
     r.result = Ok_t();
     r.error = false;
     r.handler_fault = false;
@@ -1541,7 +1605,8 @@
     r.icount = 0;
     r.rip = 0;
     r.new_coverage.clear();
-  }, P.occ.size() >= 8192);
+  }, P.res_used.size() >= 8192);
+  P.res_used.clear();
   const bool pf = P.pf;
   P.pf = false;
   if (!pf) {
@@ -1556,19 +1621,137 @@
     }
     if (wtfgpu_read_exits(ctx_, first, count, P.ex)) return false;
   }
-  std::vector<uint8_t> done(count, 0);
-  std::vector<uint32_t> hits;
-  if (!classify(P.occ, first, P.ex, done, &lres_, hits, pf ? P.sargs : nullptr)) return false;
+  const wtfgpu_exit_t *ex = P.ex;
+  const size_t n = P.occ.size();
+  constexpr size_t kChunk = 2048;
+  const size_t chunks = (n + kChunk - 1) / kChunk;
+  if (hchunks_.size() < chunks) hchunks_.resize(chunks);
+  const bool fill = !want_gprs_;
+  HostPool::Get().For(chunks, 1, [&](size_t c) {
+    HarvestChunk &C = hchunks_[c];
+    C.fin.clear();
+    C.used.clear();
+    C.run.clear();
+    C.hits.clear();
+    C.named.clear();
+    uint64_t bytes = 0;
+    const size_t hi = std::min(n, (c + 1) * kChunk);
+    for (size_t i = c * kChunk; i < hi; i++) {
+      const uint32_t l = P.occ[i];
+      const wtfgpu_exit_t &e = ex[l - first];
+      LaneView &v = views_[l];
+      const auto mark = [&]() -> LaneView & {
+        touched_[l] = 1;
+        return v;
+      };
+      bool plain = false, direct = false;
+      const auto ends = [&](TestcaseResult_t &&R) {
+        if (fill && !touched_[l]) {
+          lres_[l].result = std::move(R);
+          direct = true;
+        } else {
+          mark().result = std::move(R);
+        }
+      };
+      switch (e.status) {
+        case WTFGPU_EXIT_BREAKPOINT: C.hits.push_back(l); continue;
+        case WTFGPU_RUNNING: C.run.push_back(l); continue;
+        case WTFGPU_EXIT_STOP_ARGS: C.named.push_back(l); continue;
+        case WTFGPU_EXIT_TIMEOUT: ends(Timedout_t()); break;
+        case WTFGPU_EXIT_INT3:
+        case WTFGPU_EXIT_HLT: ends(Crash_t()); break;
+        case WTFGPU_EXIT_CR3: ends(Cr3Change_t()); break;
+        case WTFGPU_EXIT_FAULT: ends(FaultToResult(e.vector, e.error, e.rip, e.addr, e.opcode)); break;
+        case WTFGPU_EXIT_STOPPED: break;
+        case WTFGPU_EXIT_STOP_OK:
+          if (touched_[l])
+            v.result = Ok_t();
+          else
+            plain = fill;
+          break;
+        case WTFGPU_EXIT_FEED_FAULT: mark().handler_fault = true; break;
+        default:
+          lres_[l].error = true;
+          if (!v.result) mark().result = Crash_t();
+          if (e.status == WTFGPU_EXIT_UNIMPLEMENTED) {
+            stats_.err_unimpl++;
+            stats_.unimpl_ops.add(e.opcode);
+            stats_.last_unimpl_op = e.opcode;
+            stats_.last_unimpl_rip = e.rip;
+          } else if (e.status == WTFGPU_EXIT_OVERLAY_FULL) {
+            stats_.err_overlay++;
+          } else {
+            stats_.err_other++;
+          }
+          break;
+      }
+      C.fin.push_back(l);
+      if (plain) {
+        plain_[l] = 1;
+      } else {
+        C.used.push_back(l);
+        if (direct) {
+          LaneResult &r = lres_[l];
+          r.rip = e.rip;
+          r.icount = e.icount;
+          r.exit_status = e.status;
+        } else if (fill) {
+          fill_lane(l, e, lres_[l]);
+        }
+      }
+      if (pf) bytes += P.nb[l - first] + 2ull * 4096 * P.dc[l - first] + tc_bytes_[l];
+    }
+    C.bytes = bytes;
+  }, n >= 2048);
+  std::vector<uint32_t> &finished = fin_;
+  finished.clear();
+  run_.clear();
+  hits_.clear();
+  named_.clear();
+  uint64_t b_exec = 0;
+  for (size_t c = 0; c < chunks; c++) {
+    const HarvestChunk &C = hchunks_[c];
+    finished.insert(finished.end(), C.fin.begin(), C.fin.end());
+    P.res_used.insert(P.res_used.end(), C.used.begin(), C.used.end());
+    run_.insert(run_.end(), C.run.begin(), C.run.end());
+    hits_.insert(hits_.end(), C.hits.begin(), C.hits.end());
+    named_.insert(named_.end(), C.named.begin(), C.named.end());
+    b_exec += C.bytes;
+  }
+  name_stop_args(named_, first, ex, done_, &lres_, pf ? P.sargs : nullptr);
   stats_.exits_ms += ms_since(te);
-  if (!hits.empty() && !service_hits(hits, first, done, Slots, Slots != nullptr)) return false;
-  std::vector<uint32_t> finished;
-  if (!fill_results(P.occ, first, P.ex, done, &lres_, &finished)) return false;
+  if (!hits_.empty() && !service_hits(hits_, first, done_, Slots, Slots != nullptr)) return false;
+  if (!hits_.empty() || !named_.empty()) {
+    late_.resize(hits_.size() + named_.size());
+    std::merge(hits_.begin(), hits_.end(), named_.begin(), named_.end(), late_.begin());
+    std::vector<uint32_t> late_fin, late_run;
+    for (uint32_t l : late_) {
+      (done_[l - first] ? late_fin : late_run).push_back(l);
+      done_[l - first] = 0;
+    }
+    if (fill) {
+      HostPool::Get().For(late_fin.size(), 1024, [&](size_t i) {
+        fill_lane(late_fin[i], ex[late_fin[i] - first], lres_[late_fin[i]]);
+      }, late_fin.size() >= 2048);
+    }
+    if (pf)
+      for (uint32_t l : late_fin) b_exec += P.nb[l - first] + 2ull * 4096 * P.dc[l - first] + tc_bytes_[l];
+    const auto join = [&](std::vector<uint32_t> &into, const std::vector<uint32_t> &add) {
+      if (add.empty()) return;
+      tmp_lanes_.resize(into.size() + add.size());
+      std::merge(into.begin(), into.end(), add.begin(), add.end(), tmp_lanes_.begin());
+      into.swap(tmp_lanes_);
+    };
+    join(finished, late_fin);
+    join(P.res_used, late_fin);
+    join(run_, late_run);
+  }
+  P.occ.swap(run_);
   if (finished.empty()) return true;
+  if (!fill && !fill_lanes(finished, first, ex, lres_)) return false;
   const auto tc = Clock::now();
   if (pf) {
-    uint64_t b = 0;
-    for (uint32_t l : finished) b += P.nb[l - first] + 2ull * 4096 * P.dc[l - first] + tc_bytes_[l];
-    stats_.alg_bytes += b;
+    stats_.alg_bytes += b_exec;
   } else {
     uint32_t lo = finished.front() & ~63u, hi = finished.back() + 1;
     std::vector<uint64_t> nb(hi - lo);
@@ -1579,6 +1762,21 @@
   }
   stats_.bytes_ms += ms_since(tc);
   collect_coverage(finished, lres_, pf && P.pf_cov ? P.cov_hdr : nullptr);
+  {
+    uint32_t last = ~0u;
+    size_t added = 0;
+    for (const std::pair<uint32_t, uint64_t> &E : cov_sorted_) {
+      const uint32_t l = E.first;
+      if (l == last) continue;
+      last = l;
+      if (!plain_[l] || lres_[l].new_coverage.empty()) continue;
+      plain_[l] = 0;
+      fill_lane(l, ex[l - first], lres_[l]);
+      P.res_used.push_back(l);
+      added++;
+    }
+    if (added) std::inplace_merge(P.res_used.begin(), P.res_used.end() - (std::ptrdiff_t)added, P.res_used.end());
+  }
   const auto tr = Clock::now();
   stats_.coverage_ms += std::chrono::duration<double, std::milli>(tr - tc).count();
   target_restore(Target, finished, Slots);
@@ -1586,18 +1784,22 @@
   const auto tout = Clock::now();
   const size_t base = Out.size();
   Out.resize(base + finished.size());
-  for (size_t i = 0; i < finished.size(); i++) {
+  HostPool::Get().For(finished.size(), 2048, [&](size_t i) {
     const uint32_t l = finished[i];
-    Out[base + i] = StreamResult_t{tag_[l], &lres_[l]};
+    if (plain_[l]) {
+      plain_[l] = 0;
+      Out[base + i] = StreamResult_t{tag_[l], nullptr, ex[l - first].icount};
+    } else {
+      Out[base + i] = StreamResult_t{tag_[l], &lres_[l]};
+    }
     busy_[l] = 0;
-  }
-  {
-    std::vector<uint32_t> occ(P.occ.size()), fr(P.free.size() + finished.size());
-    occ.resize(std::set_difference(P.occ.begin(), P.occ.end(), finished.begin(), finished.end(), occ.begin()) -
-               occ.begin());
-    std::merge(P.free.begin(), P.free.end(), finished.begin(), finished.end(), fr.begin());
-    P.occ.swap(occ);
-    P.free.swap(fr);
+  }, finished.size() >= 8192);
+  if (P.free.empty()) {
+    P.free.swap(finished);
+  } else {
+    tmp_lanes_.resize(P.free.size() + finished.size());
+    std::merge(P.free.begin(), P.free.end(), finished.begin(), finished.end(), tmp_lanes_.begin());
+    P.free.swap(tmp_lanes_);
   }
   stats_.out_ms += ms_since(tout);
   stats_.batches++;
diff --git a/wtf_amd/host/gpu_backend.h b/wtf_amd/host/gpu_backend.h
--- a/wtf_amd/host/gpu_backend.h
+++ b/wtf_amd/host/gpu_backend.h
@@ -163,8 +163,13 @@
   bool classify(const std::vector<uint32_t> &pending, uint32_t first, const wtfgpu_exit_t *ex,
                 std::vector<uint8_t> &done, std::vector<LaneResult> *out, std::vector<uint32_t> &hits,
                 const uint64_t *stop_args = nullptr);
+  void name_stop_args(const std::vector<uint32_t> &named, uint32_t first, const wtfgpu_exit_t *ex,
+                      std::vector<uint8_t> &done, std::vector<LaneResult> *out, const uint64_t *stop_args);
   bool fill_results(const std::vector<uint32_t> &lanes, uint32_t first, const wtfgpu_exit_t *ex,
                     const std::vector<uint8_t> &done, std::vector<LaneResult> *out, std::vector<uint32_t> *finished);
+  bool fill_lanes(const std::vector<uint32_t> &fin, uint32_t first, const wtfgpu_exit_t *ex,
+                  std::vector<LaneResult> &out);
+  void fill_lane(uint32_t l, const wtfgpu_exit_t &e, LaneResult &r);
   bool stop_prestopped(const std::vector<uint32_t> &lanes);
   void account_run(const wtfgpu_run_stats_t &rs);
   bool service_hits(const std::vector<uint32_t> &hits, uint32_t first, std::vector<uint8_t> &done, ModuleSlots *slots,
@@ -179,7 +184,23 @@
   std::vector<uint64_t> tag_;
   std::vector<uint64_t> tc_bytes_;
   std::vector<LaneResult> lres_;
-  std::vector<uint8_t> lres_stale_;
+  std::vector<uint8_t> plain_;
+  std::vector<uint8_t> done_;
+  struct HarvestChunk {
+    std::vector<uint32_t> fin, used, run, hits, named;
+    uint64_t bytes = 0;
+  };
+  std::vector<HarvestChunk> hchunks_;
+  std::vector<uint32_t> hits_, named_, late_, fin_, run_, tmp_lanes_;
+  struct RefillChunk {
+    std::vector<uint32_t> call, pre;
+    uint64_t bytes = 0;
+  };
+  std::vector<RefillChunk> rchunks_;
+  std::vector<uint32_t> fresh_, call_, pre_;
+  std::vector<uint32_t> flen_;
+  std::vector<uint64_t> foff_;
+  std::vector<uint8_t> fhas_;
   std::vector<uint32_t> cov_lanes_;
   std::vector<uint64_t> cov_rips_;
   std::vector<uint8_t> cov_want_;
@@ -193,6 +214,7 @@
     uint32_t lo = 0, hi = 0;
     bool launched = false;
     std::vector<uint32_t> occ, free;
+    std::vector<uint32_t> res_used;
     wtfgpu_exit_t *ex = nullptr;
     uint64_t ex_cap = 0;
     uint8_t *pin = nullptr;
diff --git a/wtf_amd/host/runner.cc b/wtf_amd/host/runner.cc
--- a/wtf_amd/host/runner.cc
+++ b/wtf_amd/host/runner.cc
@@ -22,6 +22,13 @@
 namespace {
 
 constexpr size_t kParMutateMin = 8192, kMutateChunk = 2048;
+HostPool &MutatePool() {
+  static HostPool P([] {
+    const char *e = getenv("WTF_MUTATE_THREADS");
+    return e && atoi(e) > 0 ? (unsigned)atoi(e) : host_threads();
+  }());
+  return P;
+}
 uint64_t ThreadCpuNs() {
   timespec t{};
   clock_gettime(CLOCK_THREAD_CPUTIME_ID, &t);
@@ -651,7 +658,7 @@
     Prepare_ = Target_.PrepareInsert;
   if (stream_) {
     Adopt(MakeBatch(Budget(Exec_.Lanes())));
-    return !Ready_.empty();
+    return ReadyCount_ != 0;
   }
   Batch_ = MakeBatch(Budget(Exec_.Lanes()));
   return !Batch_.empty();
@@ -661,7 +668,8 @@
   for (std::unique_ptr<TcArena> &A : B) {
     if (!A || A->Count() == 0) continue;
     A->Live = A->Count();
-    for (size_t i = 0; i < A->Count(); i++) Ready_.push_back(TcRef{A.get(), (uint32_t)i});
+    Ready_.push_back(TcRange{A.get(), 0, (uint32_t)A->Count()});
+    ReadyCount_ += A->Count();
     TcArena *K = A.get();
     Arenas_.emplace(K, std::move(A));
   }
@@ -669,14 +677,14 @@
 
 uint64_t FuzzSession::Budget(uint64_t n) const {
   if (!O_.runs) return n;
-  const uint64_t made = S_.execs + (stream_ ? InFlight_ + Ready_.size() : 0);
+  const uint64_t made = S_.execs + (stream_ ? InFlight_ + ReadyCount_ : 0);
   return made >= O_.runs ? 0 : std::min<uint64_t>(n, O_.runs - made);
 }
 
 bool FuzzSession::Done() const {
   if (!stream_) return Batch_.empty();
   if (O_.seconds > 0 && secs_since(t0_) >= O_.seconds) return true;
-  return Ready_.empty() && InFlight_ == 0 && !Next_.valid() &&
+  return ReadyCount_ == 0 && InFlight_ == 0 && !Next_.valid() &&
          (Budget(1) == 0 || !More(S_.execs) || Corpus_.Size() == 0);
 }
 
@@ -704,11 +712,10 @@
     std::vector<uint64_t> Seeds(Chunks);
     for (uint64_t &S : Seeds) S = Rng_();
     std::vector<std::unique_ptr<TcArena>> Out(Chunks);
-    std::atomic<size_t> NextChunk{0};
     std::atomic<uint64_t> CpuNs{0};
-    auto Work = [&]() {
+    MutatePool().For(Chunks, 1, [&](size_t c) {
       const uint64_t c0 = ThreadCpuNs();
-      for (size_t c; (c = NextChunk.fetch_add(1)) < Chunks;) {
+      {
         std::mt19937_64 R(Seeds[c]);
         Corpus_t View(Corpus_, R);
         std::unique_ptr<Mutator_t> M = Target_.CreateMutator(R, O_.max_len);
@@ -725,15 +732,7 @@
         Out[c] = std::move(A);
       }
       CpuNs += ThreadCpuNs() - c0;
-    };
-    std::vector<std::thread> Pool;
-    static const unsigned MutThreads = [] {
-      const char *e = getenv("WTF_MUTATE_THREADS");
-      return e && atoi(e) > 0 ? (unsigned)atoi(e) : host_threads();
-    }();
-    for (unsigned t = 1; t < MutThreads; t++) Pool.emplace_back(Work);
-    Work();
-    for (std::thread &Th : Pool) Th.join();
+    });
     MutateCpuNs_ += CpuNs.load();
     for (std::unique_ptr<TcArena> &A : Out) Batch.push_back(std::move(A));
     Made += Need;
@@ -803,50 +802,78 @@
 bool FuzzSession::StreamStep(bool Done) {
   if (Done) return true;
   const auto t_step = Clock::now();
-  std::vector<StreamTestcase_t> In;
+  std::vector<StreamTestcase_t> &In = In_;
   const bool open = More(S_.execs);
+  if (!open) In.clear();
   if (open) {
     const uint32_t free = Exec_.FreeLanes();
-    if (Ready_.size() < free && !Next_.valid() && Corpus_.Size()) {
+    if (ReadyCount_ < free && !Next_.valid() && Corpus_.Size()) {
       const auto tm = Clock::now();
-      Adopt(MakeBatch(Budget(free - Ready_.size())));
+      Adopt(MakeBatch(Budget(free - ReadyCount_)));
       S_.make_ms += secs_since(tm) * 1e3;
     }
-    const size_t take = std::min<size_t>(free, Ready_.size());
+    const size_t take = std::min<size_t>(free, ReadyCount_);
     while (FreeSlot_.size() < take) {
       FreeSlot_.push_back(Slot_.size());
       Slot_.emplace_back();
     }
     const size_t base = FreeSlot_.size() - take;
-    std::vector<TcRef> Refs(Ready_.begin(), Ready_.begin() + (std::ptrdiff_t)take);
-    Ready_.erase(Ready_.begin(), Ready_.begin() + (std::ptrdiff_t)take);
+    Taken_.clear();
+    for (size_t got = 0; got < take;) {
+      TcRange &F = Ready_.front();
+      const uint32_t k = (uint32_t)std::min<size_t>(F.E - F.B, take - got);
+      Taken_.push_back({TcRange{F.A, F.B, F.B + k}, got});
+      got += k;
+      F.B += k;
+      if (F.B == F.E) Ready_.pop_front();
+    }
+    ReadyCount_ -= take;
     In.resize(take);
-    HostPool::Get().For(take, 1024, [&](size_t i) {
-      const uint64_t tag = FreeSlot_[base + i];
-      const TcRef R = Refs[i];
-      Slot_[tag] = R;
-      StreamTestcase_t T{R.data(), R.size(), tag};
-      if (R.A->Prep.size() == R.A->Count()) {
-        T.prep = R.prep();
-        T.prep_data = R.prep_data();
-        T.prep_size = R.prep_size();
-      }
-      In[i] = T;
+    constexpr size_t kFill = 1024;
+    HostPool::Get().For((take + kFill - 1) / kFill, 1, [&](size_t c) {
+      const size_t lo = c * kFill, hi = std::min(take, lo + kFill);
+      size_t r = (size_t)(std::upper_bound(Taken_.begin(), Taken_.end(), lo,
+                                           [](size_t v, const std::pair<TcRange, size_t> &T) { return v < T.second; }) -
+                          Taken_.begin()) - 1;
+      for (size_t i = lo; i < hi; r++) {
+        const TcRange &G = Taken_[r].first;
+        TcArena *A = G.A;
+        const bool prep = A->Prep.size() == A->Count();
+        const size_t end = std::min<size_t>(hi, Taken_[r].second + (G.E - G.B));
+        for (; i < end; i++) {
+          const uint64_t tag = FreeSlot_[base + i];
+          const TcRef R{A, G.B + (uint32_t)(i - Taken_[r].second)};
+          Slot_[tag] = R;
+          StreamTestcase_t T{R.data(), R.size(), tag};
+          if (prep) {
+            T.prep = R.prep();
+            T.prep_data = R.prep_data();
+            T.prep_size = R.prep_size();
+          }
+          In[i] = T;
+        }
+      }
     }, take >= 4096);
     FreeSlot_.resize(base);
     InFlight_ += take;
-    const uint64_t want = Budget(Exec_.Lanes() > Ready_.size() ? Exec_.Lanes() - Ready_.size() : 0);
+    const uint64_t want = Budget(Exec_.Lanes() > ReadyCount_ ? Exec_.Lanes() - ReadyCount_ : 0);
     if (want && Corpus_.Size() && !Next_.valid())
       Next_ = std::async(std::launch::async, &FuzzSession::MakeBatch, this, want);
   }
-  std::vector<StreamResult_t> Out;
+  std::vector<StreamResult_t> &Out = Out_;
+  Out.clear();
   const auto tb = Clock::now();
   S_.fill_ms += std::chrono::duration<double, std::milli>(tb - t_step).count();
   size_t Taken = 0;
   const bool ok = Exec_.StreamStep(Target_, In, O_.slice, Out, &Slots_, &Taken);
   S_.run_s += secs_since(tb);
   for (size_t i = In.size(); i-- > Taken;) {
-    Ready_.push_front(Slot_[In[i].tag]);
+    const TcRef R = Slot_[In[i].tag];
+    if (!Ready_.empty() && Ready_.front().A == R.A && Ready_.front().B == R.I + 1)
+      Ready_.front().B = R.I;
+    else
+      Ready_.push_front(TcRange{R.A, R.I, R.I + 1});
+    ReadyCount_++;
     Slot_[In[i].tag] = TcRef{};
     FreeSlot_.push_back(In[i].tag);
     InFlight_--;
@@ -857,9 +884,7 @@
   S_.produce_wait_ms += std::chrono::duration<double, std::milli>(ta - tw).count();
   if (!ok) return false;
   S_.batches++;
-  for (const StreamResult_t &F : Out)
-    if (F.tag >= Slot_.size()) return false;
-  AccountStep(Out);
+  if (!AccountStep(Out)) return false;
   S_.account_ms += secs_since(ta) * 1e3;
   if (X_ && X_->Exchanging() && !MergeCoverage(false)) return false;
   S_.step_ms += secs_since(t_step) * 1e3;
@@ -893,73 +918,87 @@
   if (ArenaPool_.size() < 512) ArenaPool_.push_back(std::move(Own));
 }
 
-void FuzzSession::AccountStep(std::vector<StreamResult_t> &Out) {
+bool FuzzSession::AccountStep(std::vector<StreamResult_t> &Out) {
   const size_t n = Out.size();
   enum : uint8_t { K_SERIAL = 1, K_TIMEOUT = 2, K_CR3 = 4, K_CRASH = 8 };
-  std::vector<uint8_t> Kind(n, 0);
-  std::vector<TcArena *> Ar(n);
-  struct Sum {
-    uint64_t retired = 0, timeouts = 0, cr3 = 0, crashes = 0;
-  };
-  const unsigned T = HostPool::Get().Threads();
-  std::vector<Sum> Part(T + 1);
+  constexpr size_t kChunk = 2048;
+  const size_t chunks = (n + kChunk - 1) / kChunk;
+  if (Acct_.size() < chunks) Acct_.resize(chunks);
   const bool every = Sample_ != nullptr;
-  HostPool::Get().For(n, 1024, [&](size_t i) {
-    const LaneResult &L = *Out[i].r;
-    const TcRef R = Slot_[Out[i].tag];
-    Ar[i] = R.A;
-    uint8_t k = 0;
-    if (every || L.error) {
-      k = K_SERIAL;
-    } else {
-      if (std::holds_alternative<Timedout_t>(L.result)) k |= K_TIMEOUT;
-      if (std::holds_alternative<Cr3Change_t>(L.result)) k |= K_CR3;
-      if (const Crash_t *C = std::get_if<Crash_t>(&L.result)) {
-        k |= K_CRASH;
-        if (!C->CrashName.empty() && !CrashNames_.count(C->CrashName)) k = K_SERIAL;
-      }
-      if (!L.new_coverage.empty() && !std::holds_alternative<Timedout_t>(L.result)) k = K_SERIAL;
-    }
-    Kind[i] = k;
-    if (k != K_SERIAL) {
-      Sum &s = Part[HostPool::ThreadIndex()];
-      s.retired += L.icount;
-      s.timeouts += (k & K_TIMEOUT) != 0;
-      s.cr3 += (k & K_CR3) != 0;
-      s.crashes += (k & K_CRASH) != 0;
+  const size_t fs = FreeSlot_.size(), slots = Slot_.size();
+  FreeSlot_.resize(fs + n);
+  std::atomic<bool> bad{false};
+  HostPool::Get().For(chunks, 1, [&](size_t c) {
+    AcctChunk &C = Acct_[c];
+    C.retired = C.timeouts = C.cr3 = C.crashes = 0;
+    C.serial.clear();
+    C.arena.clear();
+    const size_t hi = std::min(n, (c + 1) * kChunk);
+    for (size_t i = c * kChunk; i < hi; i++) {
+      const uint64_t tag = Out[i].tag;
+      if (tag >= slots) {
+        bad = true;
+        FreeSlot_[fs + i] = 0;
+        continue;
+      }
+      const TcRef R = Slot_[tag];
+      Slot_[tag] = TcRef{};
+      FreeSlot_[fs + i] = tag;
+      if (!C.arena.empty() && C.arena.back().first == R.A)
+        C.arena.back().second++;
+      else
+        C.arena.push_back({R.A, 1});
+      const LaneResult *L = Out[i].r;
+      if (!L && !every) {
+        C.retired += Out[i].icount;
+        continue;
+      }
+      uint8_t k = 0;
+      if (every || L->error) {
+        k = K_SERIAL;
+      } else {
+        if (std::holds_alternative<Timedout_t>(L->result)) k |= K_TIMEOUT;
+        if (std::holds_alternative<Cr3Change_t>(L->result)) k |= K_CR3;
+        if (const Crash_t *Cr = std::get_if<Crash_t>(&L->result)) {
+          k |= K_CRASH;
+          if (!Cr->CrashName.empty() && !CrashNames_.count(Cr->CrashName)) k = K_SERIAL;
+        }
+        if (!L->new_coverage.empty() && !std::holds_alternative<Timedout_t>(L->result)) k = K_SERIAL;
+      }
+      if (k == K_SERIAL) {
+        C.serial.push_back({(uint32_t)i, R});
+        continue;
+      }
+      C.retired += L->icount;
+      C.timeouts += (k & K_TIMEOUT) != 0;
+      C.cr3 += (k & K_CR3) != 0;
+      C.crashes += (k & K_CRASH) != 0;
     }
   }, n >= 4096);
-  uint64_t bulk = 0;
-  for (size_t i = 0; i < n; i++) {
-    if (Kind[i] != K_SERIAL) {
-      bulk++;
-      continue;
-    }
-    const TcRef R = Slot_[Out[i].tag];
-    Account(R.data(), R.size(), *Out[i].r, false);
-  }
-  S_.execs += bulk;
-  for (const Sum &s : Part) {
-    S_.retired += s.retired;
-    S_.timeouts += s.timeouts;
-    S_.cr3 += s.cr3;
-    S_.crashes += s.crashes;
-  }
-  const size_t fs = FreeSlot_.size();
-  FreeSlot_.resize(fs + n);
-  HostPool::Get().For(n, 4096, [&](size_t i) {
-    Slot_[Out[i].tag] = TcRef{};
-    FreeSlot_[fs + i] = Out[i].tag;
-  }, n >= 8192);
+  if (bad) return false;
+  uint64_t serial = 0;
+  LaneResult Plain;
+  for (size_t c = 0; c < chunks; c++)
+    for (const std::pair<uint32_t, TcRef> &E : Acct_[c].serial) {
+      const StreamResult_t &F = Out[E.first];
+      serial++;
+      if (!F.r) Plain.icount = F.icount;
+      Account(E.second.data(), E.second.size(), F.r ? *F.r : Plain, false);
+    }
+  S_.execs += n - serial;
   InFlight_ -= n;
-  for (size_t i = 0; i < n;) {
-    size_t j = i + 1;
-    while (j < n && Ar[j] == Ar[i]) j++;
-    TcArena *A = Ar[i];
-    A->Live -= j - i;
-    if (A->Live == 0) ReleaseArena(A);
-    i = j;
-  }
+  for (size_t c = 0; c < chunks; c++) {
+    const AcctChunk &C = Acct_[c];
+    S_.retired += C.retired;
+    S_.timeouts += C.timeouts;
+    S_.cr3 += C.cr3;
+    S_.crashes += C.crashes;
+    for (const std::pair<TcArena *, uint32_t> &E : C.arena) {
+      E.first->Live -= E.second;
+      if (E.first->Live == 0) ReleaseArena(E.first);
+    }
+  }
+  return true;
 }
 
 void FuzzSession::Account(const uint8_t *Tc, size_t Size, const LaneResult &L, bool KnownCrash) {
diff --git a/wtf_amd/host/runner.h b/wtf_amd/host/runner.h
--- a/wtf_amd/host/runner.h
+++ b/wtf_amd/host/runner.h
@@ -45,6 +45,7 @@
 struct StreamResult_t {
   uint64_t tag;
   LaneResult *r;
+  uint64_t icount = 0;
 };
 
 class Executor_t {
@@ -242,7 +243,7 @@
   FILE *Sample_ = nullptr;
   bool StreamStep(bool Done);
   void Account(const uint8_t *Tc, size_t Size, const LaneResult &L, bool KnownCrash = false);
-  void AccountStep(std::vector<StreamResult_t> &Out);
+  bool AccountStep(std::vector<StreamResult_t> &Out);
   void ReleaseArena(TcArena *A);
   std::unique_ptr<TcArena> NewArena();
   std::mutex ArenaPoolMu_;
@@ -269,11 +270,25 @@
   FuzzStats S_;
   std::chrono::steady_clock::time_point t0_;
   bool stream_ = false;
-  std::deque<TcRef> Ready_;
+  struct TcRange {
+    TcArena *A = nullptr;
+    uint32_t B = 0, E = 0;
+  };
+  std::deque<TcRange> Ready_;
+  size_t ReadyCount_ = 0;
   std::unordered_map<TcArena *, std::unique_ptr<TcArena>> Arenas_;
   std::vector<TcRef> Slot_;
   std::vector<uint64_t> FreeSlot_;
   size_t InFlight_ = 0;
+  std::vector<StreamTestcase_t> In_;
+  std::vector<StreamResult_t> Out_;
+  std::vector<std::pair<TcRange, size_t>> Taken_;
+  struct AcctChunk {
+    uint64_t retired = 0, timeouts = 0, cr3 = 0, crashes = 0;
+    std::vector<std::pair<uint32_t, TcRef>> serial;
+    std::vector<std::pair<TcArena *, uint32_t>> arena;
+  };
+  std::vector<AcctChunk> Acct_;
 };
 
 bool ParseRunnerArgs(int argc, char **argv, RunnerOptions &O);
```

Result: faster. 16.06 million (median of 6 runs) (+16.5%).
